# sanweiliti/RoHM

Measured on NVIDIA H100. Metric: denoised motion clips/sec (145-frame, 1000-step PoseNet p_sample_loop), higher is better.
Workload: dtype f32 (fp16 hi/lo error-compensated tensor-core GEMMs)

## Files before the change

include/rohm_b200.h:

```cpp
#ifndef ROHM_B200_H_
#define ROHM_B200_H_

#include <stdint.h>

#ifdef __cplusplus
extern "C" {
#endif

#if defined(__GNUC__)
#define ROHM_API __attribute__((visibility("default")))
#else
#define ROHM_API
#endif

typedef enum {
  ROHM_OK = 0,
  ROHM_ERR_INVALID = -1,
  ROHM_ERR_CUDA = -2,
  ROHM_ERR_NO_DEVICE = -3,
  ROHM_ERR_STATE = -4
} rohm_status;

typedef enum {
  ROHM_PRECISION_TF32X3 = 3,
  ROHM_PRECISION_F16X2 = 2,
  ROHM_PRECISION_TF32 = 1
} rohm_precision;

typedef struct rohm_ctx rohm_ctx;
typedef struct rohm_posenet rohm_posenet;
typedef struct rohm_trajnet rohm_trajnet;
typedef struct rohm_body rohm_body;

ROHM_API int rohm_version(void);
ROHM_API int rohm_ctx_create(int device, rohm_ctx** out);
ROHM_API void rohm_ctx_destroy(rohm_ctx* ctx);
ROHM_API const char* rohm_last_error(const rohm_ctx* ctx);


#define ROHM_DDPM_COEFS 8
ROHM_API int rohm_ddpm_step(rohm_ctx* ctx, const float* x0, const float* x_t, const float* noise, const float* grad0,
                            const float* grad1, int n_grads, float* out, int64_t n_clips, int64_t clip_elems,
                            const float* coef, int64_t coef_clip_stride, void* stream);

ROHM_API int rohm_ddpm_step_philox(rohm_ctx* ctx, const float* x0, const float* x_t, const float* grad0, const float* grad1,
                                   int n_grads, float* out, int64_t n_clips, int64_t clip_elems, const float* coef,
                                   int64_t coef_clip_stride, uint64_t seed, uint64_t offset, uint64_t* offset_increment,
                                   void* stream);

ROHM_API int rohm_q_sample(rohm_ctx* ctx, const float* x_start, const float* noise, float* out, int64_t n, float sqrt_ac,
                  float sqrt_one_minus_ac, void* stream);

ROHM_API int rohm_ddim_step(rohm_ctx* ctx, const float* x0, const float* x_t, const float* noise, float* out, int64_t n,
                   float sqrt_recip_ac, float sqrt_recipm1_ac, float sqrt_ac_prev, float dir_coef, float sigma,
                   void* stream);

typedef struct {
  const float* in_proj_w;
  const float* in_proj_b;
  const float* out_proj_w;
  const float* out_proj_b;
  const float* lin1_w;
  const float* lin1_b;
  const float* lin2_w;
  const float* lin2_b;
  const float* norm1_w;
  const float* norm1_b;
  const float* norm2_w;
  const float* norm2_b;
} rohm_posenet_layer;

typedef struct {
  int d_model;
  int ff_size;
  int num_layers;
  int num_heads;
  int in_feats;
  int out_feats;
  int traj_feats;
  int pe_len;
  const float* in_w;
  const float* in_b;
  const float* cond_w;
  const float* cond_b;
  const float* pe;
  const float* t0_w;
  const float* t0_b;
  const float* t2_w;
  const float* t2_b;
  const float* out_w;
  const float* out_b;
  const rohm_posenet_layer* layers;
} rohm_posenet_weights;

ROHM_API int rohm_posenet_create(rohm_ctx* ctx, const rohm_posenet_weights* w, int max_batch, int max_frames, int precision,
                        rohm_posenet** out);
ROHM_API void rohm_posenet_destroy(rohm_posenet* pn);

ROHM_API int rohm_posenet_set_cond(rohm_posenet* pn, const float* cond, int B, int T, void* stream);

ROHM_API int rohm_posenet_set_lengths(rohm_posenet* pn, const int* lengths_host, int B);

ROHM_API int rohm_posenet_forward(rohm_posenet* pn, const float* x_t, const int64_t* timesteps, float* out, int B, int T,
                         void* stream);

ROHM_API int rohm_posenet_sample_step(rohm_posenet* pn, const float* x_t, const int64_t* timesteps, float* x0_out,
                                      float* x_next, const float* coef_row, uint64_t seed, uint64_t offset,
                                      uint64_t* offset_increment, int B, int T, void* stream);

ROHM_API int rohm_posenet_profile(rohm_posenet* pn, const float* x_t, const int64_t* timesteps, float* out, int B, int T,
                         void* stream, float* ms_by_category, int* launches_by_category);

ROHM_API int rohm_posenet_set_option(rohm_posenet* pn, int option, int value);

ROHM_API int rohm_posenet_launches_per_forward(const rohm_posenet* pn);


ROHM_API int rohm_trajnet_create(rohm_ctx* ctx, int n_params, const char* const* names, const float* const* ptrs,
                                 const int64_t* numels, int time_dim, int cond_dim, int traj_feat_dim, int mid_dim,
                                 int trajcontrol, int control_cond_dim, int max_batch, int frames, int precision,
                                 rohm_trajnet** out);
ROHM_API void rohm_trajnet_destroy(rohm_trajnet* tn);

ROHM_API int rohm_trajnet_set_cond(rohm_trajnet* tn, const float* cond, const float* control_cond, int B, void* stream);

ROHM_API int rohm_trajnet_set_lengths(rohm_trajnet* tn, const int* lengths_host, int B);

ROHM_API int rohm_trajnet_forward(rohm_trajnet* tn, const float* x_t, const int64_t* time, float* out, int B,
                                  void* stream);
ROHM_API int rohm_trajnet_sample_step(rohm_trajnet* tn, const float* x_t, const int64_t* time, float* x0_out, float* x_next,
                                      const float* coef_row, uint64_t seed, uint64_t offset, uint64_t* offset_increment, int B,
                                      void* stream);
ROHM_API int rohm_trajnet_set_option(rohm_trajnet* tn, int option, int value);
ROHM_API int rohm_trajnet_launches_per_forward(const rohm_trajnet* tn);


ROHM_API int rohm_body_create(rohm_ctx* ctx, const float* v_template, const float* shapedirs, int shape_comps,
                              const float* posedirs, const float* J_regressor, const float* lbs_weights,
                              const int* parents_host, int num_verts, int64_t max_frames, int with_vertices,
                              int precision, rohm_body** out);
ROHM_API void rohm_body_destroy(rohm_body* bd);
ROHM_API int rohm_body_uses_fused_lbs(const rohm_body* bd);

ROHM_API int rohm_body_set_vertex_pitch(rohm_body* bd, int64_t pitch_floats);

ROHM_API int rohm_body_forward(rohm_body* bd, const float* global_orient, const float* body_pose, const float* betas,
                               const float* transl, int64_t N, float* joints, int num_joints, float* vertices,
                               void* stream);

ROHM_API int rohm_body_from_repr(rohm_body* bd, const float* x, const float* mean, const float* stdv, int B, int T,
                                 float* joints, int num_joints, float* vertices, void* stream);

ROHM_API int rohm_body_from_repr_layout(rohm_body* bd, const float* x, int channels_last, const float* mean,
                                        const float* stdv, int B, int T, float* joints, int num_joints, float* vertices,
                                        void* stream);


ROHM_API int rohm_body_from_repr_lengths(rohm_body* bd, const float* x, int channels_last, const float* mean,
                                         const float* stdv, int B, int T, const int* lengths, const int* clip_off,
                                         int64_t total_frames, float* joints, int num_joints, float* vertices,
                                         void* stream);

ROHM_API int rohm_skating_guidance(rohm_body* bd, const float* x0, const float* mean, const float* stdv, int B, int T,
                                   float* grad, float* loss_out, void* stream);

ROHM_API int rohm_skating_guidance_lengths(rohm_body* bd, const float* x0, const float* mean, const float* stdv,
                                           const int* lengths, int B, int T, float* grad, float* loss_out, void* stream);

ROHM_API int rohm_skating_guidance_sums(rohm_body* bd, const float* x0, const float* mean, const float* stdv, int B, int T,
                                        float* sums_out, void* stream);
ROHM_API int rohm_skating_guidance_backward(rohm_body* bd, const float* x0, const float* mean, const float* stdv, int B, int T,
                                            const float* sums, float* grad, void* stream);

ROHM_API int rohm_projection_guidance(rohm_body* bd, const float* x0, const float* mean, const float* stdv, int B, int T,
                                      const float* cam_affine, const float* focal, const float* center,
                                      const float* keypoints_2d, int kp_frames, float* grad, float* loss_out,
                                      void* stream);


ROHM_API int rohm_traj_glue(rohm_body* bd, const float* traj_out, int traj_dim, const float* repr_clean,
                            const float* traj_mean, const float* traj_std, const float* pose_mean, const float* pose_std,
                            int B, int T, float* composite_out, float* traj_full_out, void* stream);

ROHM_API int rohm_traj_glue_lengths(rohm_body* bd, const float* traj_out, int traj_dim, const float* repr_clean,
                                    const float* traj_mean, const float* traj_std, const float* pose_mean,
                                    const float* pose_std, int B, int T, const int* lengths, const int* clip_off,
                                    int64_t total_frames, float* composite_out, float* traj_full_out, void* stream);

ROHM_API int rohm_traj_repr_from_joints(rohm_ctx* ctx, const float* joints, const float* global_orient_aa,
                                        const float* transl, const float* mean, const float* stdv, int B, int T,
                                        float* traj_full_out, void* stream);

ROHM_API int rohm_traj_repr_from_joints_lengths(rohm_ctx* ctx, const float* joints, const float* global_orient_aa,
                                                const float* transl, const float* mean, const float* stdv, int B, int T,
                                                const int* lengths, const int* clip_off, float* traj_full_out,
                                                void* stream);

ROHM_API int rohm_pose_to_control_cond(rohm_ctx* ctx, const float* pose_out, int B, int Tp, int T, int traj_feats,
                                       int cond_feats, float* control_cond, void* stream);

ROHM_API int rohm_pose_to_control_cond_lengths(rohm_ctx* ctx, const float* pose_out, int B, int Tp, int T, int traj_feats,
                                               int cond_feats, const int* lengths, float* control_cond, void* stream);

ROHM_API int rohm_build_pose_cond(rohm_ctx* ctx, const float* src, int src_channel_major, int src_T, const float* traj_full,
                                  const unsigned char* chan_keep, const int* frame_lo, const int* frame_hi,
                                  int zero_contact, int B, int Tp, float* cond_out, void* stream);

ROHM_API int rohm_build_pose_cond_lengths(rohm_ctx* ctx, const float* src, int src_channel_major, int src_T,
                                          const float* traj_full, const unsigned char* chan_keep, const int* frame_lo,
                                          const int* frame_hi, int zero_contact, int B, int Tp, const int* lengths,
                                          float* cond_out, void* stream);

ROHM_API int rohm_rot6d_to_aa(rohm_ctx* ctx, const float* rot6d, int64_t n, float* aa, float* rotmat, void* stream);

ROHM_API int rohm_joints_from_traj(rohm_ctx* ctx, const float* x, int channels_last, const float* mean, const float* stdv,
                                   int B, int T, int relative, float* joints, void* stream);

ROHM_API int rohm_joints_from_traj_lengths(rohm_ctx* ctx, const float* x, int channels_last, const float* mean,
                                           const float* stdv, int B, int T, const int* lengths, const int* clip_off,
                                           int64_t total_frames, int relative, float* joints, void* stream);

#ifdef __cplusplus
}
#endif
#endif
```

rohm_b200/_lib.py:

```python
import ctypes as C
import os
import threading

_HERE = os.path.dirname(os.path.abspath(__file__))
LIB_PATH = os.path.join(_HERE, "librohm_b200.so")

ROHM_OK = 0
PRECISION_TF32X3 = 3
PRECISION_F16X2 = 2
PRECISION_TF32 = 1
DDPM_COEFS = 8


class RohmB200Error(RuntimeError):
    pass


class PoseNetLayerW(C.Structure):
    _fields_ = [(n, C.c_void_p) for n in (
        "in_proj_w", "in_proj_b", "out_proj_w", "out_proj_b", "lin1_w", "lin1_b", "lin2_w", "lin2_b",
        "norm1_w", "norm1_b", "norm2_w", "norm2_b")]


class PoseNetW(C.Structure):
    _fields_ = [("d_model", C.c_int), ("ff_size", C.c_int), ("num_layers", C.c_int), ("num_heads", C.c_int),
                ("in_feats", C.c_int), ("out_feats", C.c_int), ("traj_feats", C.c_int), ("pe_len", C.c_int)] + \
               [(n, C.c_void_p) for n in ("in_w", "in_b", "cond_w", "cond_b", "pe", "t0_w", "t0_b", "t2_w", "t2_b",
                                          "out_w", "out_b")] + [("layers", C.POINTER(PoseNetLayerW))]


_p, _i, _i64, _f = C.c_void_p, C.c_int, C.c_int64, C.c_float
SIGNATURES = {
    "rohm_version": (_i, []),
    "rohm_ctx_create": (_i, [_i, C.POINTER(_p)]),
    "rohm_ctx_destroy": (None, [_p]),
    "rohm_last_error": (C.c_char_p, [_p]),
    "rohm_ddpm_step": (_i, [_p, _p, _p, _p, _p, _p, _i, _p, _i64, _i64, _p, _i64, _p]),
    "rohm_ddpm_step_philox": (_i, [_p, _p, _p, _p, _p, _i, _p, _i64, _i64, _p, _i64, C.c_uint64, C.c_uint64,
                                    C.POINTER(C.c_uint64), _p]),
    "rohm_q_sample": (_i, [_p, _p, _p, _p, _i64, _f, _f, _p]),
    "rohm_ddim_step": (_i, [_p, _p, _p, _p, _p, _i64, _f, _f, _f, _f, _f, _p]),
    "rohm_posenet_create": (_i, [_p, C.POINTER(PoseNetW), _i, _i, _i, C.POINTER(_p)]),
    "rohm_posenet_destroy": (None, [_p]),
    "rohm_posenet_set_cond": (_i, [_p, _p, _i, _i, _p]),
    "rohm_posenet_set_lengths": (_i, [_p, C.POINTER(_i), _i]),
    "rohm_posenet_forward": (_i, [_p, _p, _p, _p, _i, _i, _p]),
    "rohm_posenet_sample_step": (_i, [_p, _p, _p, _p, _p, _p, C.c_uint64, C.c_uint64, C.POINTER(C.c_uint64), _i, _i, _p]),
    "rohm_posenet_profile": (_i, [_p, _p, _p, _p, _i, _i, _p, C.POINTER(C.c_float), C.POINTER(C.c_int)]),
    "rohm_posenet_set_option": (_i, [_p, _i, _i]),
    "rohm_posenet_launches_per_forward": (_i, [_p]),
    "rohm_trajnet_create": (_i, [_p, _i, C.POINTER(C.c_char_p), C.POINTER(_p), C.POINTER(_i64), _i, _i, _i, _i, _i, _i,
                                 _i, _i, _i, C.POINTER(_p)]),
    "rohm_trajnet_destroy": (None, [_p]),
    "rohm_trajnet_set_cond": (_i, [_p, _p, _p, _i, _p]),
    "rohm_trajnet_set_lengths": (_i, [_p, C.POINTER(_i), _i]),
    "rohm_trajnet_forward": (_i, [_p, _p, _p, _p, _i, _p]),
    "rohm_trajnet_sample_step": (_i, [_p, _p, _p, _p, _p, _p, C.c_uint64, C.c_uint64, C.POINTER(C.c_uint64), _i, _p]),
    "rohm_trajnet_set_option": (_i, [_p, _i, _i]),
    "rohm_trajnet_launches_per_forward": (_i, [_p]),
    "rohm_body_create": (_i, [_p, _p, _p, _i, _p, _p, _p, C.POINTER(C.c_int), _i, _i64, _i, _i, C.POINTER(_p)]),
    "rohm_body_destroy": (None, [_p]),
    "rohm_body_uses_fused_lbs": (_i, [_p]),
    "rohm_body_set_vertex_pitch": (_i, [_p, _i64]),
    "rohm_body_forward": (_i, [_p, _p, _p, _p, _p, _i64, _p, _i, _p, _p]),
    "rohm_body_from_repr": (_i, [_p, _p, _p, _p, _i, _i, _p, _i, _p, _p]),
    "rohm_body_from_repr_layout": (_i, [_p, _p, _i, _p, _p, _i, _i, _p, _i, _p, _p]),
    "rohm_body_from_repr_lengths": (_i, [_p, _p, _i, _p, _p, _i, _i, _p, _p, _i64, _p, _i, _p, _p]),
    "rohm_skating_guidance": (_i, [_p, _p, _p, _p, _i, _i, _p, _p, _p]),
    "rohm_skating_guidance_lengths": (_i, [_p, _p, _p, _p, _p, _i, _i, _p, _p, _p]),
    "rohm_skating_guidance_sums": (_i, [_p, _p, _p, _p, _i, _i, _p, _p]),
    "rohm_skating_guidance_backward": (_i, [_p, _p, _p, _p, _i, _i, _p, _p, _p]),
    "rohm_projection_guidance": (_i, [_p, _p, _p, _p, _i, _i, _p, _p, _p, _p, _i, _p, _p, _p]),
    "rohm_traj_glue": (_i, [_p, _p, _i, _p, _p, _p, _p, _p, _i, _i, _p, _p, _p]),
    "rohm_traj_glue_lengths": (_i, [_p, _p, _i, _p, _p, _p, _p, _p, _i, _i, _p, _p, _i64, _p, _p, _p]),
    "rohm_traj_repr_from_joints": (_i, [_p, _p, _p, _p, _p, _p, _i, _i, _p, _p]),
    "rohm_traj_repr_from_joints_lengths": (_i, [_p, _p, _p, _p, _p, _p, _i, _i, _p, _p, _p, _p]),
    "rohm_pose_to_control_cond": (_i, [_p, _p, _i, _i, _i, _i, _i, _p, _p]),
    "rohm_pose_to_control_cond_lengths": (_i, [_p, _p, _i, _i, _i, _i, _i, _p, _p, _p]),
    "rohm_build_pose_cond": (_i, [_p, _p, _i, _i, _p, _p, _p, _p, _i, _i, _i, _p, _p]),
    "rohm_build_pose_cond_lengths": (_i, [_p, _p, _i, _i, _p, _p, _p, _p, _i, _i, _i, _p, _p, _p]),
    "rohm_rot6d_to_aa": (_i, [_p, _p, _i64, _p, _p, _p]),
    "rohm_joints_from_traj": (_i, [_p, _p, _i, _p, _p, _i, _i, _i, _p, _p]),
    "rohm_joints_from_traj_lengths": (_i, [_p, _p, _i, _p, _p, _i, _i, _p, _p, _i64, _i, _p, _p]),
}

_lock = threading.Lock()
_lib = None
_ctx = {}


def load():
    global _lib
    if _lib is not None:
        return _lib
    with _lock:
        if _lib is not None:
            return _lib
        if not os.path.exists(LIB_PATH):
            raise RohmB200Error(
                f"{LIB_PATH} not found: build it with `python -c 'import __graft_entry__ as g; g.build()'` "
                "or `make -C rohm_b200/csrc`.  rohm_b200 has no CPU fallback.")
        try:
            lib = C.CDLL(LIB_PATH)
        except OSError as e:
            raise RohmB200Error(f"cannot load {LIB_PATH}: {e}") from e
        for name, (res, args) in SIGNATURES.items():
            fn = getattr(lib, name)
            fn.restype = res
            fn.argtypes = args
        _lib = lib
    return _lib


def ctx(device_index):
    lib = load()
    if device_index in _ctx:
        return _ctx[device_index]
    with _lock:
        if device_index in _ctx:
            return _ctx[device_index]
        out = C.c_void_p()
        rc = lib.rohm_ctx_create(int(device_index), C.byref(out))
        if rc != ROHM_OK:
            raise RohmB200Error(f"rohm_ctx_create(device={device_index}) failed with status {rc}: "
                                "an sm_90 (H100) device is required; there is no CPU fallback")
        _ctx[device_index] = out
    return _ctx[device_index]


def check(rc, c):
    if rc != ROHM_OK:
        msg = load().rohm_last_error(c)
        raise RohmB200Error(f"status {rc}: {msg.decode() if msg else '?'}")
```

rohm_b200/csrc/gemm.cu:

```cuda
#include "gemm.cuh"
#include "ptx.cuh"

#include <cudaTypedefs.h>
#include <cmath>
#include <cstdio>
#include <cstring>
#include <mutex>

namespace rohm {

namespace {

constexpr int kFirstMmaWarp = 4;
constexpr int kMmaWarps = 8;
constexpr int kFirstEpiWarp = kFirstMmaWarp + kMmaWarps;
__host__ __device__ constexpr bool epi_role(int epi) { return epi == 0 || epi == 1 || epi == 3; }
__host__ __device__ constexpr int kernel_threads(int epi) { return 32 * (kFirstEpiWarp + (epi_role(epi) ? 4 : 0)); }
constexpr int kProducerRegs = 40, kEpiRoleRegs = 152, kMmaRegs = 160;
static_assert(kProducerRegs + kEpiRoleRegs + 2 * kMmaRegs <= 512, "register file of one SM");
static_assert(kProducerRegs <= 128 && kEpiRoleRegs >= 128 && kMmaRegs >= 128, "setmaxnreg.dec / .inc direction");
constexpr int kSmemLimit = 227 * 1024;
constexpr int kStaticSmemReserve = 8 * 1024;
constexpr int kEpiTileFloats = 32 * 32;
constexpr int kSkinPitch = 100;
constexpr int kSkinStageBytes = kGemmBlockM * kSkinPitch * 4;

template <int BLOCK_N, int PASSES, bool EPI_ROLE>
struct TileCfg {
  static constexpr int kEpiWarps = EPI_ROLE ? 4 : 8;
  static constexpr int kABytes = kGemmBlockM * kGemmBlockK * 4;
  static constexpr int kBBytes = BLOCK_N * kGemmBlockK * 4;
  static constexpr int kSplit = (PASSES == 3) ? 2 : 1;
  static constexpr int kStageBytes = kSplit * (kABytes + kBBytes);
  static constexpr int kAccPitch = BLOCK_N + 4;
  static constexpr int kAccBytes = kGemmBlockM * kAccPitch * 4;
  static constexpr int kEpiBytes = !EPI_ROLE && BLOCK_N == 96 && kSkinStageBytes > kEpiWarps * kEpiTileFloats * 4
                                       ? kSkinStageBytes
                                       : kEpiWarps * kEpiTileFloats * 4;
  static constexpr int kStagesRaw = (kSmemLimit - kStaticSmemReserve - 1024 - kAccBytes - kEpiBytes) / kStageBytes;
  static constexpr int kStages = kStagesRaw > 10 ? 10 : kStagesRaw;
  static constexpr int kSmemBytes = kStages * kStageBytes + 1024 + kAccBytes + kEpiWarps * kEpiTileFloats * 4;
  static constexpr int kAccRegs = BLOCK_N / 2;
  static_assert(kStages >= 2, "need at least a double buffer");
  static_assert(BLOCK_N % 32 == 0 && BLOCK_N >= 32 && BLOCK_N <= 128, "wgmma N and the epilogue's 32-column chunks");
};

template <int KIND, int R>
__device__ __forceinline__ void mma_step(float (&d)[R], uint64_t a, uint64_t b) {
  if constexpr (KIND == kKindF16) ptx::wgmma_f16(d, a, b);
  else ptx::wgmma_tf32(d, a, b);
}

template <int PITCH, int N>
__device__ __forceinline__ void acc_load(const float* acc, int row, int col, float (&v)[N]) {
  const float4* src = reinterpret_cast<const float4*>(acc + row * PITCH + col);
#pragma unroll
  for (int j = 0; j < N / 4; ++j) {
    const float4 t = src[j];
    v[4 * j] = t.x, v[4 * j + 1] = t.y, v[4 * j + 2] = t.z, v[4 * j + 3] = t.w;
  }
}

__device__ __forceinline__ float apply_act(float x, int act) {
  if (act == kActGelu) {
    return 0.5f * x * (1.0f + erff(x * 0.70710678118654752440f));
  } else if (act == kActSilu) {
    return x / (1.0f + expf(-x));
  } else if (act == kActMish) {
    float sp = x > 20.0f ? x : log1pf(expf(x));
    return x * tanhf(sp);
  }
  return x;
}

__device__ __forceinline__ float gelu_erf(float x) {
  const float u = fminf(fabsf(x), 6.5f);
  float q = -1.657032612e-06f;
  q = fmaf(q, u, 2.461445729e-05f);
  q = fmaf(q, u, -1.118122309e-04f);
  q = fmaf(q, u, -3.311361652e-04f);
  q = fmaf(q, u, 7.346248254e-03f);
  q = fmaf(q, u, -5.272617936e-02f);
  q = fmaf(q, u, -4.591094553e-01f);
  q = fmaf(q, u, -1.151124716e+00f);
  q = fmaf(q, u, -9.999987483e-01f);
  float p;
  asm("ex2.approx.ftz.f32 %0, %1;" : "=f"(p) : "f"(q));
  return fmaf(-fabsf(x), p, fmaxf(x, 0.0f));
}

__device__ __forceinline__ void load_bone_transform(const float* frame_col, int64_t lda, int bone, float4& r0, float4& r1,
                                                    float4& r2) {
  const float* a = frame_col + static_cast<int64_t>(bone) * 12 * lda;
  r0 = make_float4(__ldg(a), __ldg(a + lda), __ldg(a + 2 * lda), __ldg(a + 3 * lda));
  r1 = make_float4(__ldg(a + 4 * lda), __ldg(a + 5 * lda), __ldg(a + 6 * lda), __ldg(a + 7 * lda));
  r2 = make_float4(__ldg(a + 8 * lda), __ldg(a + 9 * lda), __ldg(a + 10 * lda), __ldg(a + 11 * lda));
}

struct EpiParams {
  const float* bias;
  const float* residual;
  const float2* a_stats;
  const float* a_corr;
  const float2* res_stats;
  const float* res_gamma;
  const float* res_beta;
  float2* stats_out;
  float ln_eps;
  float* out;
  void* out_hi;
  void* out_lo;
  float acc_scale;
  int tma_store;
  int bias_per_row;
  int ldr, ldo, lds, act, M, N, out_row_mul, out_row_add, clip_rows, clip_valid;
};

__device__ __forceinline__ float2 combine_row_stats(const float2* row8, float eps) {
  const float4* q4 = reinterpret_cast<const float4*>(row8);
  float4 t[4];
#pragma unroll
  for (int i = 0; i < 4; ++i) t[i] = __ldcg(q4 + i);
  const float mean = ((t[0].x + t[0].z) + (t[1].x + t[1].z) + (t[2].x + t[2].z) + (t[3].x + t[3].z)) * 0.125f;
  float m2 = 0.0f;
#pragma unroll
  for (int i = 0; i < 4; ++i) {
    const float d0 = t[i].x - mean, d1 = t[i].z - mean;
    m2 += fmaf(64.0f * d0, d0, t[i].y) + fmaf(64.0f * d1, d1, t[i].w);
  }
  return make_float2(mean, rsqrtf(m2 * (1.0f / 512.0f) + eps));
}

__device__ __forceinline__ void stage_pair_chunk(const float (&v)[32], uint8_t* tb, int lane, const CUtensorMap* st_hi,
                                                 const CUtensorMap* st_lo, int col0, int row0) {
  if (lane == 0) ptx::bulk_wait_read_all();
  __syncwarp();
#pragma unroll
  for (int c = 0; c < 4; ++c) {
    uint2 h0, l0, h1, l1;
    ptx::split_f16x4(make_float4(v[8 * c], v[8 * c + 1], v[8 * c + 2], v[8 * c + 3]), h0, l0);
    ptx::split_f16x4(make_float4(v[8 * c + 4], v[8 * c + 5], v[8 * c + 6], v[8 * c + 7]), h1, l1);
    const int off = lane * 64 + ((c ^ ((lane >> 1) & 3)) << 4);
    *reinterpret_cast<uint4*>(tb + off) = make_uint4(h0.x, h0.y, h1.x, h1.y);
    *reinterpret_cast<uint4*>(tb + 2048 + off) = make_uint4(l0.x, l0.y, l1.x, l1.y);
  }
  ptx::fence_proxy_async();
  __syncwarp();
  if (lane == 0) {
    ptx::tma_store_2d(st_hi, tb, col0, row0);
    ptx::tma_store_2d(st_lo, tb + 2048, col0, row0);
    ptx::bulk_commit();
  }
}

template <int BLOCK_N, int PASSES, int EPI, int KIND>
__global__ void __launch_bounds__(kernel_threads(EPI), 1) gemm_tile_kernel(const __grid_constant__ GemmParams p) {
  constexpr bool LEAN = EPI != 2 && EPI != 5;
  constexpr bool EPI_ROLE = epi_role(EPI);
  constexpr int kElemK = gemm_block_k(KIND);
  using Cfg = TileCfg<BLOCK_N, PASSES, EPI_ROLE>;
  constexpr int kEpiWarps = Cfg::kEpiWarps;
  extern __shared__ uint8_t smem_raw[];
  __shared__ uint64_t full_bar[Cfg::kStages];
  __shared__ uint64_t empty_bar[Cfg::kStages];
  __shared__ EpiParams epi_s;
  __shared__ __align__(16) float bias_s[BLOCK_N];
  __shared__ __align__(16) float corr_s[BLOCK_N];
  __shared__ __align__(16) float beta_s[EPI == 3 ? BLOCK_N : 4];
  __shared__ uint64_t res_bar[EPI == 3 ? kEpiWarps : 1];
  __shared__ uint64_t acc_full, acc_empty;
  __shared__ __align__(16) float skin_w_s[EPI == 4 ? 2 : 1][EPI == 4 ? kSkinTileBones * 32 : 4];
  __shared__ int skin_bone_s[EPI == 4 ? 2 : 1][EPI == 4 ? kSkinTileBones : 1];
  __shared__ int skin_nb_s[2];

  const uint32_t raw_addr = ptx::smem_u32(smem_raw);
  uint8_t* smem = smem_raw + ((1024u - (raw_addr & 1023u)) & 1023u);
  float* const acc_s = reinterpret_cast<float*>(smem + Cfg::kStages * Cfg::kStageBytes);
  uint8_t* const epi_smem = smem + Cfg::kStages * Cfg::kStageBytes + Cfg::kAccBytes;

  const int warp_idx = threadIdx.x >> 5;
  const int lane = threadIdx.x & 31;
  const int tiles_n = (p.grid_n_cols + BLOCK_N - 1) / BLOCK_N;
  const int tiles_m = (p.grid_m_rows + kGemmBlockM - 1) / kGemmBlockM;
  const int num_tiles = tiles_m * tiles_n;

  int total_iters = 0;
  for (int s = 0; s < p.num_segs; ++s) total_iters += p.seg_kblocks[s];
  const int S = (!LEAN && p.k_splits > 1) ? p.k_splits : 1;
  const int per_split = (total_iters + S - 1) / S;
  const int num_work = num_tiles * S;

  if (warp_idx == 0 && lane == 0) {
    ptx::prefetch_tmap(&p.b_hi);
    if (PASSES == 3) ptx::prefetch_tmap(&p.b_lo);
    for (int s = 0; s < p.num_segs; ++s) {
      ptx::prefetch_tmap(&p.a_hi[s]);
      if (PASSES == 3) ptx::prefetch_tmap(&p.a_lo[s]);
    }
    for (int i = 0; i < Cfg::kStages; ++i) {
      ptx::mbar_init(&full_bar[i], 1);
      ptx::mbar_init(&empty_bar[i], 2);
    }
    if (EPI == 3)
      for (int i = 0; i < kEpiWarps; ++i) ptx::mbar_init(&res_bar[i], 1);
    if (EPI_ROLE) {
      ptx::mbar_init(&acc_full, kMmaWarps);
      ptx::mbar_init(&acc_empty, kEpiWarps);
    }
    ptx::fence_barrier_init();
  }
  int prefetched = 0;
  if (warp_idx == 0 && lane == 0 && static_cast<int>(blockIdx.x) < num_work) {
    const int tile0 = static_cast<int>(blockIdx.x) / S;
    const int it_b = (static_cast<int>(blockIdx.x) - tile0 * S) * per_split;
    const int cnt = (total_iters < it_b + per_split ? total_iters : it_b + per_split) - it_b;
    const int n0 = (tile0 % tiles_n) * BLOCK_N;
    prefetched = cnt < Cfg::kStages ? cnt : Cfg::kStages;
    for (int i = 0; i < prefetched; ++i) {
      uint8_t* st = smem + i * Cfg::kStageBytes;
      ptx::mbar_expect_tx(&full_bar[i], Cfg::kStageBytes);
      ptx::tma_load_2d(st + Cfg::kSplit * Cfg::kABytes, &p.b_hi, &full_bar[i], (it_b + i) * kElemK, n0);
      if (PASSES == 3)
        ptx::tma_load_2d(st + 2 * Cfg::kABytes + Cfg::kBBytes, &p.b_lo, &full_bar[i], (it_b + i) * kElemK, n0);
    }
  }
  if (warp_idx == kFirstMmaWarp && lane == 0) {
    epi_s.bias = p.bias, epi_s.residual = p.residual, epi_s.ldr = p.ldr, epi_s.out = p.out, epi_s.ldo = p.ldo;
    epi_s.out_hi = p.out_hi, epi_s.out_lo = p.out_lo, epi_s.lds = p.lds, epi_s.act = p.act, epi_s.M = p.M, epi_s.N = p.N;
    epi_s.out_row_mul = p.out_row_mul, epi_s.out_row_add = p.out_row_add, epi_s.clip_rows = p.clip_rows;
    epi_s.clip_valid = p.clip_valid;
    epi_s.acc_scale = p.acc_scale == 0.0f ? 1.0f : p.acc_scale;
    epi_s.tma_store = p.tma_store;
    epi_s.bias_per_row = p.bias_per_row;
    epi_s.a_stats = p.a_stats, epi_s.a_corr = p.a_corr, epi_s.res_stats = p.res_stats, epi_s.res_gamma = p.res_gamma;
    epi_s.res_beta = p.res_beta, epi_s.stats_out = p.stats_out, epi_s.ln_eps = p.ln_eps;
    if (p.tma_store) {
      ptx::prefetch_tmap(&p.st_out);
      ptx::prefetch_tmap(&p.st_hi);
      ptx::prefetch_tmap(&p.st_lo);
    }
  }
  __syncthreads();

  ptx::pdl_launch_dependents();
  ptx::pdl_wait_prior_grid();

  if (warp_idx < kFirstMmaWarp) {
    ptx::setmaxnreg_dec<kProducerRegs>();
    if (warp_idx == 0 && lane == 0) {
      int it = 0, stage = 0;
      uint32_t phase = 0;
      for (int w = blockIdx.x; w < num_work; w += gridDim.x) {
        const int tile = w / S;
        const int m0 = (tile / tiles_n) * kGemmBlockM;
        const int n0 = (tile % tiles_n) * BLOCK_N;
        const int it_b = (w - tile * S) * per_split;
        const int it_e = total_iters < it_b + per_split ? total_iters : it_b + per_split;
        int s = 0, kb = it_b;
        while (s + 1 < p.num_segs && kb >= p.seg_kblocks[s]) kb -= p.seg_kblocks[s], ++s;
        int kcol = it_b * kElemK;
        for (int i = it_b; i < it_e; ++i, ++it, kcol += kElemK) {
          {
            const int row = m0 * p.seg_row_mul[s] + p.seg_row_shift[s];
            uint8_t* st = smem + stage * Cfg::kStageBytes;
            if (it < prefetched) {
              ptx::tma_load_2d(st, &p.a_hi[s], &full_bar[stage], kb * kElemK, row);
              if (PASSES == 3) ptx::tma_load_2d(st + Cfg::kABytes, &p.a_lo[s], &full_bar[stage], kb * kElemK, row);
              if (++stage == Cfg::kStages) stage = 0, phase ^= 1;
              if (++kb == p.seg_kblocks[s]) kb = 0, ++s;
              continue;
            }
            ptx::mbar_wait(&empty_bar[stage], phase ^ 1);
            ptx::mbar_expect_tx(&full_bar[stage], Cfg::kStageBytes);
            ptx::tma_load_2d(st, &p.a_hi[s], &full_bar[stage], kb * kElemK, row);
            ptx::tma_load_2d(st + Cfg::kSplit * Cfg::kABytes, &p.b_hi, &full_bar[stage], kcol, n0);
            if (PASSES == 3) {
              ptx::tma_load_2d(st + Cfg::kABytes, &p.a_lo[s], &full_bar[stage], kb * kElemK, row);
              ptx::tma_load_2d(st + 2 * Cfg::kABytes + Cfg::kBBytes, &p.b_lo, &full_bar[stage], kcol, n0);
            }
            if (++stage == Cfg::kStages) stage = 0, phase ^= 1;
            if (++kb == p.seg_kblocks[s]) kb = 0, ++s;
          }
        }
      }
    }
  } else {
    const bool mma_warp = warp_idx < kFirstEpiWarp;
    if constexpr (!EPI_ROLE) ptx::setmaxnreg_inc<232>();
    const int mq = (warp_idx - kFirstMmaWarp) & 3;
    const int mhalf = (warp_idx - kFirstMmaWarp) >> 2;
    const int ew = warp_idx - (EPI_ROLE ? kFirstEpiWarp : kFirstMmaWarp);
    const int q = ew & 3;
    const int half = EPI_ROLE ? 0 : ew >> 2;
    constexpr int kChunkStep = EPI_ROLE ? 32 : 64;
    int mma_stage = 0;
    uint32_t mma_phase = 0;
    auto mma_tile = [&](int w, int tc) {
      float dm[Cfg::kAccRegs];
      float dc[PASSES == 3 ? Cfg::kAccRegs : 1];
#pragma unroll
      for (int i = 0; i < Cfg::kAccRegs; ++i) dm[i] = 0.0f;
#pragma unroll
      for (int i = 0; i < (PASSES == 3 ? Cfg::kAccRegs : 1); ++i) dc[i] = 0.0f;
      const int it_b = (w % S) * per_split;
      const int n_it = (total_iters < it_b + per_split ? total_iters : it_b + per_split) - it_b;
      const bool signaller = (threadIdx.x & 127) == 0;
      auto release = [&](int stg) {
        if (signaller) ptx::mbar_arrive(&empty_bar[stg]);
      };
      int prev = -1;
      for (int ki = 0; ki < n_it; ++ki) {
        ptx::mbar_wait(&full_bar[mma_stage], mma_phase);
        const uint32_t st = ptx::smem_u32(smem + mma_stage * Cfg::kStageBytes);
        const uint32_t a_off = static_cast<uint32_t>(mhalf * (Cfg::kABytes / 2));
        const uint64_t a_hi = ptx::make_desc_kmajor<kGemmBlockK * 4>(st + a_off);
        const uint64_t b_hi = ptx::make_desc_kmajor<kGemmBlockK * 4>(st + Cfg::kSplit * Cfg::kABytes);
        const uint64_t a_lo = ptx::make_desc_kmajor<kGemmBlockK * 4>(st + Cfg::kABytes + a_off);
        const uint64_t b_lo = ptx::make_desc_kmajor<kGemmBlockK * 4>(st + 2 * Cfg::kABytes + Cfg::kBBytes);
        ptx::wgmma_fence_regs(dm);
        if (PASSES == 3) ptx::wgmma_fence_regs(dc);
        ptx::wgmma_fence();
#pragma unroll
        for (int k = 0; k < kGemmBlockK / 8; ++k) {
          const uint64_t koff = static_cast<uint64_t>(k * 2);
          mma_step<KIND>(dm, a_hi + koff, b_hi + koff);
          if constexpr (PASSES == 3) {
            mma_step<KIND>(dc, a_lo + koff, b_hi + koff);
            mma_step<KIND>(dc, a_hi + koff, b_lo + koff);
          }
        }
        ptx::wgmma_commit();
        ptx::wgmma_fence_regs(dm);
        if (PASSES == 3) ptx::wgmma_fence_regs(dc);
        ptx::wgmma_wait<1>();
        if (prev >= 0) release(prev);
        prev = mma_stage;
        if (++mma_stage == Cfg::kStages) mma_stage = 0, mma_phase ^= 1;
      }
      ptx::wgmma_wait<0>();
      ptx::wgmma_fence_regs(dm);
      if (PASSES == 3) ptx::wgmma_fence_regs(dc);
      if (prev >= 0) release(prev);
      if constexpr (EPI_ROLE) ptx::mbar_wait(&acc_empty, static_cast<uint32_t>((tc & 1) ^ 1));
      const int r0 = mhalf * 64 + mq * 16 + (lane >> 2);
      const int cc = 2 * (lane & 3);
#pragma unroll
      for (int j = 0; j < BLOCK_N / 8; ++j) {
        float v0 = dm[4 * j], v1 = dm[4 * j + 1], v2 = dm[4 * j + 2], v3 = dm[4 * j + 3];
        if (PASSES == 3) v0 += dc[4 * j], v1 += dc[4 * j + 1], v2 += dc[4 * j + 2], v3 += dc[4 * j + 3];
        *reinterpret_cast<float2*>(acc_s + r0 * Cfg::kAccPitch + 8 * j + cc) = make_float2(v0, v1);
        *reinterpret_cast<float2*>(acc_s + (r0 + 8) * Cfg::kAccPitch + 8 * j + cc) = make_float2(v2, v3);
      }
      if constexpr (EPI_ROLE) {
        __syncwarp();
        if (lane == 0) ptx::mbar_arrive(&acc_full);
      } else {
        asm volatile("bar.sync 3, %0;" ::"n"(kMmaWarps * 32));
      }
    };
    const bool epi_warp = !EPI_ROLE || !mma_warp;
    if (!epi_warp) {
      ptx::setmaxnreg_inc<kMmaRegs>();
      int tc = 0;
      for (int wi = blockIdx.x; wi < num_work; wi += gridDim.x, ++tc) mma_tile(wi, tc);
    } else if constexpr (EPI_ROLE) {
      ptx::setmaxnreg_inc<kEpiRoleRegs>();
    }
    EpiParams e_regs;
    if constexpr (!EPI_ROLE) e_regs = epi_s;
    const EpiParams& e = EPI_ROLE ? epi_s : e_regs;
    const bool vec_ok = ((e.N & 3) == 0);
    float* tile = reinterpret_cast<float*>(epi_smem) + ew * kEpiTileFloats;
    const int tr = lane >> 3, tc = (lane & 7) * 4;
    int tcount = 0;
    uint32_t res_phase = 0;
    if constexpr (EPI == 4) {
      static_assert(BLOCK_N == 96 && PASSES == 3 && KIND == kKindF16, "skinning epilogue: 32 vertices x 3 per tile, fp16 pairs");
      constexpr int kSkinRegBones = 4;
      const int i = ew * 32 + lane;
      float4 sk[kSkinRegBones][3];
      float* const stg = reinterpret_cast<float*>(epi_smem);
      auto fetch_tables = [&](int tile_n, float& w0, float& w1, int& bone, int& nbv) {
        const float* wsrc = p.skin_w + static_cast<int64_t>(tile_n) * (kSkinTileBones * 32);
        w0 = __ldg(wsrc + i), w1 = __ldg(wsrc + i + 256);
        bone = i < kSkinTileBones ? __ldg(p.skin_bone + tile_n * kSkinTileBones + i) : 0;
        nbv = i == 0 ? __ldg(p.skin_nb + tile_n) : 0;
      };
      auto publish_tables = [&](int buf, float w0, float w1, int bone, int nbv) {
        skin_w_s[buf][i] = w0, skin_w_s[buf][i + 256] = w1;
        if (i < kSkinTileBones) skin_bone_s[buf][i] = bone;
        if (i == 0) skin_nb_s[buf] = nbv;
      };
      auto request_transforms = [&](int buf, int m_first) {
        const int mm = m_first + q * 32 + lane;
        const float* col = p.skin_A + (mm < e.M ? mm : 0);
        const int nbv = skin_nb_s[buf];
#pragma unroll
        for (int b = 0; b < kSkinRegBones; ++b)
          if (b < nbv) load_bone_transform(col, p.skin_lda, skin_bone_s[buf][b], sk[b][0], sk[b][1], sk[b][2]);
      };
      int buf = 0;
      if (static_cast<int>(blockIdx.x) < num_tiles) {
        float w0, w1;
        int bone, nbv;
        fetch_tables(static_cast<int>(blockIdx.x) % tiles_n, w0, w1, bone, nbv);
        publish_tables(0, w0, w1, bone, nbv);
        asm volatile("bar.sync 1, %0;" ::"n"(kEpiWarps * 32));
        request_transforms(0, (static_cast<int>(blockIdx.x) / tiles_n) * kGemmBlockM);
      }
      for (int tile_idx = blockIdx.x; tile_idx < num_tiles; tile_idx += gridDim.x, ++tcount, buf ^= 1) {
        const int m0 = (tile_idx / tiles_n) * kGemmBlockM;
        const int n0 = (tile_idx % tiles_n) * BLOCK_N;
        const int m = m0 + q * 32 + lane;
        const int next = tile_idx + static_cast<int>(gridDim.x);
        const bool has_next = next < num_tiles;
        float nw0 = 0.f, nw1 = 0.f;
        int nbone = 0, nnb = 0;
        if (has_next) fetch_tables(next % tiles_n, nw0, nw1, nbone, nnb);

        mma_tile(tile_idx, tcount);
        float o[48];
#pragma unroll
        for (int j = 0; j < 48; ++j) o[j] = 0.0f;
        const int nb = skin_nb_s[buf];
        const float* col = p.skin_A + (m < e.M ? m : 0);
#pragma unroll
        for (int h2 = 0; h2 < 2; ++h2) {
          float vp[24];
          {
            acc_load<Cfg::kAccPitch>(acc_s, q * 32 + lane, 48 * half + 24 * h2, vp);
#pragma unroll
            for (int j = 0; j < 24; ++j) vp[j] *= e.acc_scale;
          }
          auto apply_bone = [&](const float4& r0, const float4& r1, const float4& r2, const float* wrow) {
#pragma unroll
            for (int g = 0; g < 2; ++g) {
              const float4 w4 = *reinterpret_cast<const float4*>(wrow + 8 * h2 + 4 * g);
              const float wv[4] = {w4.x, w4.y, w4.z, w4.w};
#pragma unroll
              for (int u = 0; u < 4; ++u) {
                const int j = 4 * g + u;
                const float x = vp[3 * j], y = vp[3 * j + 1], z = vp[3 * j + 2];
                float& ox = o[24 * h2 + 3 * j];
                float& oy = o[24 * h2 + 3 * j + 1];
                float& oz = o[24 * h2 + 3 * j + 2];
                ox = fmaf(wv[u], fmaf(r0.x, x, fmaf(r0.y, y, fmaf(r0.z, z, r0.w))), ox);
                oy = fmaf(wv[u], fmaf(r1.x, x, fmaf(r1.y, y, fmaf(r1.z, z, r1.w))), oy);
                oz = fmaf(wv[u], fmaf(r2.x, x, fmaf(r2.y, y, fmaf(r2.z, z, r2.w))), oz);
              }
            }
          };
#pragma unroll
          for (int b = 0; b < kSkinRegBones; ++b)
            if (b < nb) apply_bone(sk[b][0], sk[b][1], sk[b][2], &skin_w_s[buf][b * 32 + 16 * half]);
          if (nb > kSkinRegBones) {
            float4 c0, c1, c2;
            load_bone_transform(col, p.skin_lda, skin_bone_s[buf][kSkinRegBones], c0, c1, c2);
            for (int b = kSkinRegBones; b < nb; ++b) {
              const float4 r0 = c0, r1 = c1, r2 = c2;
              if (b + 1 < nb) load_bone_transform(col, p.skin_lda, skin_bone_s[buf][b + 1], c0, c1, c2);
              apply_bone(r0, r1, r2, &skin_w_s[buf][b * 32 + 16 * half]);
            }
          }
        }
        if (has_next) publish_tables(buf ^ 1, nw0, nw1, nbone, nnb);
        if (e.tma_store && ew == 0 && lane == 0) ptx::bulk_wait_read_all();
        asm volatile("bar.sync 1, %0;" ::"n"(kEpiWarps * 32));
        if (has_next) request_transforms(buf ^ 1, (next / tiles_n) * kGemmBlockM);
        if (e.tma_store) {
          uint8_t* const sb = reinterpret_cast<uint8_t*>(stg);
          const int r = q * 32 + lane;
#pragma unroll
          for (int j = 0; j < 12; ++j) {
            const int cc = 12 * half + j;
            *reinterpret_cast<float4*>(sb + (cc >> 3) * (kGemmBlockM * 128) + r * 128 + (((cc & 7) ^ (r & 7)) << 4)) =
                make_float4(o[4 * j], o[4 * j + 1], o[4 * j + 2], o[4 * j + 3]);
          }
          ptx::fence_proxy_async();
          asm volatile("bar.sync 2, %0;" ::"n"(kEpiWarps * 32));
          if (ew == 0 && lane == 0) {
#pragma unroll
            for (int j = 0; j < 3; ++j)
              if (n0 + 32 * j < e.N) ptx::tma_store_2d(&p.st_out, sb + j * (kGemmBlockM * 128), n0 + 32 * j, m0);
            ptx::bulk_commit();
          }
          continue;
        }
        {
          float4* srow = reinterpret_cast<float4*>(stg + (q * 32 + lane) * kSkinPitch + 48 * half);
#pragma unroll
          for (int j = 0; j < 12; ++j) srow[j] = make_float4(o[4 * j], o[4 * j + 1], o[4 * j + 2], o[4 * j + 3]);
        }
        asm volatile("bar.sync 2, %0;" ::"n"(kEpiWarps * 32));
        {
          const int w8 = ew;
#pragma unroll 4
          for (int rr = 0; rr < kGemmBlockM / kEpiWarps; ++rr) {
            const int r = w8 * (kGemmBlockM / kEpiWarps) + rr;
            const int mr = m0 + r;
            if (mr >= e.M) break;
            float* dst = e.out + static_cast<int64_t>(mr) * e.ldo + n0;
            const float* src = stg + r * kSkinPitch;
#pragma unroll
            for (int c = 0; c < 3; ++c) {
              const int col = lane + 32 * c;
              if (n0 + col < e.N) __stcs(dst + col, src[col]);
            }
          }
        }
      }
    }
    for (int wi = blockIdx.x; EPI != 4 && epi_warp && wi < num_work; wi += gridDim.x, ++tcount) {
      const int tile_idx = wi / S;
      const int split_rows = (wi - tile_idx * S) * (!LEAN ? p.split_row_stride : 0);
      const int m0 = (tile_idx / tiles_n) * kGemmBlockM;
      const int n0 = (tile_idx % tiles_n) * BLOCK_N;
      const int m = m0 + q * 32 + lane;
      const bool row_ok = m < e.M;
      bool row_real = true;
      if constexpr (EPI == 5) row_real = row_ok && __ldg(p.row_mask + m) != 0;
      else if (!LEAN && e.clip_rows > 0) row_real = (m % e.clip_rows) < e.clip_valid;
      const int64_t orow = static_cast<int64_t>(m) * e.out_row_mul + e.out_row_add + split_rows;
      const float bias_row = (e.bias != nullptr && e.bias_per_row && row_ok) ? __ldg(e.bias + m) : 0.0f;

      {
        const int i = ew * 32 + lane;
        asm volatile("bar.sync 1, %0;" ::"n"(kEpiWarps * 32));
        if (i < BLOCK_N) {
          const bool col_ok = n0 + i < e.N;
          bias_s[i] = (e.bias != nullptr && !e.bias_per_row && col_ok) ? __ldg(e.bias + n0 + i) : 0.0f;
          if (EPI == 3) {
            corr_s[i] = e.res_stats != nullptr ? __ldg(e.res_gamma + n0 + i) : 1.0f;
            beta_s[i] = e.res_stats != nullptr ? __ldg(e.res_beta + n0 + i) : 0.0f;
          } else {
            corr_s[i] = (e.a_stats != nullptr && col_ok) ? __ldg(e.a_corr + n0 + i) : 0.0f;
          }
        }
        if (e.residual != nullptr && row_ok) {
          const float* r = e.residual + orow * e.ldr + n0 + half * 32;
#pragma unroll
          for (int c = 0; c < (EPI_ROLE ? BLOCK_N : (BLOCK_N > 64 ? 128 : 64)); c += kChunkStep)
            asm volatile("prefetch.global.L2 [%0];" ::"l"(r + c));
        }
        asm volatile("bar.sync 1, %0;" ::"n"(kEpiWarps * 32));
      }
      float a_mean = 0.0f, a_rstd = 1.0f;
      if (EPI != 3 && LEAN && e.a_stats != nullptr && row_ok) {
        const float2 mr = combine_row_stats(e.a_stats + static_cast<int64_t>(m) * 8, e.ln_eps);
        a_mean = mr.x, a_rstd = mr.y;
      }
      float lnv[EPI == 3 ? 2 : 1][EPI == 3 ? 32 : 1];
      float r_mean = 0.0f, r_rstd = 1.0f;
      auto load_residual = [&](int g) {
        uint8_t* tb = reinterpret_cast<uint8_t*>(tile);
        uint64_t* rb = &res_bar[ew];
#pragma unroll
        for (int h2 = 0; h2 < 2; ++h2) {
          const int c0 = g * 32 + 64 * h2;
          if (lane == 0) {
            ptx::bulk_wait_read_all();
            ptx::mbar_expect_tx(rb, 4096);
            ptx::tma_load_2d(tb, &p.st_hi, rb, n0 + c0, m0 + q * 32);
            ptx::tma_load_2d(tb + 2048, &p.st_lo, rb, n0 + c0, m0 + q * 32);
          }
          ptx::mbar_wait(rb, res_phase);
          res_phase ^= 1;
#pragma unroll
          for (int c = 0; c < 4; ++c) {
            const int off = lane * 64 + ((c ^ ((lane >> 1) & 3)) << 4);
            const uint4 hq = *reinterpret_cast<const uint4*>(tb + off);
            const uint4 lq = *reinterpret_cast<const uint4*>(tb + 2048 + off);
            const uint32_t hw[4] = {hq.x, hq.y, hq.z, hq.w};
            const uint32_t lw[4] = {lq.x, lq.y, lq.z, lq.w};
#pragma unroll
            for (int k = 0; k < 4; ++k) {
              const float2 fh = __half22float2(*reinterpret_cast<const __half2*>(&hw[k]));
              const float2 fl = __half22float2(*reinterpret_cast<const __half2*>(&lw[k]));
              const int j = 8 * c + 2 * k;
              lnv[h2][j] = fmaf(((fh.x + fl.x) - r_mean) * r_rstd, corr_s[c0 + j], beta_s[c0 + j]);
              lnv[h2][j + 1] = fmaf(((fh.y + fl.y) - r_mean) * r_rstd, corr_s[c0 + j + 1], beta_s[c0 + j + 1]);
            }
          }
          ptx::fence_proxy_async();
          __syncwarp();
        }
      };
      if constexpr (EPI == 3) {
        if (e.res_stats != nullptr && row_ok) {
          const float2 mr = combine_row_stats(e.res_stats + static_cast<int64_t>(m) * 8, e.ln_eps);
          r_mean = mr.x, r_rstd = mr.y;
        }
        load_residual(0);
      }
      if constexpr (EPI_ROLE) {
        ptx::mbar_wait(&acc_full, static_cast<uint32_t>(tcount & 1));
      } else {
        mma_tile(wi, tcount);
      }

      if constexpr (EPI == 3) {
        static_assert(BLOCK_N == 128 && PASSES == 3 && KIND == kKindF16, "LayerNorm-folding producer: fp16 pairs, 128-wide tiles");
        static_assert(EPI_ROLE, "one thread per row: both 64-column statistics groups");
        const int tile_n = tile_idx % tiles_n;
        float (&v)[2][32] = lnv;
        uint8_t* tb = reinterpret_cast<uint8_t*>(tile);
        const bool group_full = (m0 + q * 32 + 32 <= e.M);
#pragma unroll 1
        for (int g = 0; g < 2; ++g) {
          if (g == 1) load_residual(1);
#pragma unroll
          for (int h2 = 0; h2 < 2; ++h2) {
            const int c0 = g * 32 + 64 * h2;
            float raw[32];
            acc_load<Cfg::kAccPitch>(acc_s, q * 32 + lane, c0, raw);
#pragma unroll
            for (int j = 0; j < 32; j += 4) {
              const float4 b4 = *reinterpret_cast<const float4*>(&bias_s[c0 + j]);
              v[h2][j] += fmaf(raw[j], e.acc_scale, b4.x);
              v[h2][j + 1] += fmaf(raw[j + 1], e.acc_scale, b4.y);
              v[h2][j + 2] += fmaf(raw[j + 2], e.acc_scale, b4.z);
              v[h2][j + 3] += fmaf(raw[j + 3], e.acc_scale, b4.w);
            }
          }
          if (g == 1) {
            __syncwarp();
            if (lane == 0) ptx::mbar_arrive(&acc_empty);
          }
          auto store_chunk = [&](int h2) {
            const int nb = n0 + g * 32 + 64 * h2;
            if (group_full) {
              stage_pair_chunk(v[h2], tb, lane, &p.st_hi, &p.st_lo, nb, m0 + q * 32);
            } else if (row_ok) {
              __half* oh = static_cast<__half*>(e.out_hi) + static_cast<int64_t>(m) * e.lds + nb;
              __half* ol = static_cast<__half*>(e.out_lo) + static_cast<int64_t>(m) * e.lds + nb;
#pragma unroll
              for (int j = 0; j < 32; ++j) ptx::split_f16(v[h2][j], oh[j], ol[j]);
            }
          };
          store_chunk(0);
          float s1 = 0.0f;
#pragma unroll
          for (int j = 0; j < 32; ++j) s1 += v[0][j] + v[1][j];
          const float mean_i = s1 * (1.0f / 64.0f);
          float m2_i = 0.0f;
#pragma unroll
          for (int j = 0; j < 32; ++j) {
            const float d0 = v[0][j] - mean_i, d1 = v[1][j] - mean_i;
            m2_i = fmaf(d0, d0, fmaf(d1, d1, m2_i));
          }
          if (row_ok) e.stats_out[static_cast<int64_t>(m) * 8 + tile_n * 2 + g] = make_float2(mean_i, m2_i);
          store_chunk(1);
        }
        continue;
      }

#pragma unroll 1
      for (int c0 = half * 32; c0 < BLOCK_N; c0 += kChunkStep) {
        const int nb = n0 + c0;
        const bool full = vec_ok && (nb + 32 <= e.N);
        if (e.tma_store && full && (m0 + q * 32 + 32 <= e.M)) {
          float v[32];
          acc_load<Cfg::kAccPitch>(acc_s, q * 32 + lane, c0, v);
          if (KIND == kKindF16) {
#pragma unroll
            for (int j = 0; j < 32; ++j) v[j] *= e.acc_scale;
          }
          if (LEAN && e.a_stats != nullptr) {
#pragma unroll
            for (int j = 0; j < 32; j += 4) {
              const float4 c4 = *reinterpret_cast<const float4*>(&corr_s[c0 + j]);
              v[j] = a_rstd * fmaf(-a_mean, c4.x, v[j]), v[j + 1] = a_rstd * fmaf(-a_mean, c4.y, v[j + 1]);
              v[j + 2] = a_rstd * fmaf(-a_mean, c4.z, v[j + 2]), v[j + 3] = a_rstd * fmaf(-a_mean, c4.w, v[j + 3]);
            }
          }
          if (e.bias != nullptr) {
#pragma unroll
            for (int j = 0; j < 32; j += 4) {
              const float4 b4 = *reinterpret_cast<const float4*>(&bias_s[c0 + j]);
              v[j] += b4.x, v[j + 1] += b4.y, v[j + 2] += b4.z, v[j + 3] += b4.w;
            }
            if (e.bias_per_row) {
#pragma unroll
              for (int j = 0; j < 32; ++j) v[j] += bias_row;
            }
          }
          if (EPI == 1) {
#pragma unroll
            for (int j = 0; j < 32; ++j) v[j] = gelu_erf(v[j]);
          }
          if (!LEAN) {
            if (e.act == kActGelu) {
#pragma unroll
              for (int j = 0; j < 32; ++j) v[j] = gelu_erf(v[j]);
            } else if (e.act == kActSilu) {
#pragma unroll
              for (int j = 0; j < 32; ++j) v[j] = v[j] / (1.0f + expf(-v[j]));
            } else if (e.act == kActMish) {
#pragma unroll
              for (int j = 0; j < 32; ++j) v[j] = apply_act(v[j], kActMish);
            }
            if (!row_real) {
#pragma unroll
              for (int j = 0; j < 32; ++j) v[j] = 0.0f;
            }
          }
          if (lane == 0) ptx::bulk_wait_read_all();
          __syncwarp();
          uint8_t* tb = reinterpret_cast<uint8_t*>(tile);
          if (e.out != nullptr) {
#pragma unroll
            for (int c = 0; c < 8; ++c)
              *reinterpret_cast<float4*>(tb + lane * 128 + ((c ^ (lane & 7)) << 4)) =
                  make_float4(v[4 * c], v[4 * c + 1], v[4 * c + 2], v[4 * c + 3]);
          } else {
#pragma unroll
            for (int c = 0; c < 4; ++c) {
              uint2 h0, l0, h1, l1;
              ptx::split_f16x4(make_float4(v[8 * c], v[8 * c + 1], v[8 * c + 2], v[8 * c + 3]), h0, l0);
              ptx::split_f16x4(make_float4(v[8 * c + 4], v[8 * c + 5], v[8 * c + 6], v[8 * c + 7]), h1, l1);
              const int off = lane * 64 + ((c ^ ((lane >> 1) & 3)) << 4);
              *reinterpret_cast<uint4*>(tb + off) = make_uint4(h0.x, h0.y, h1.x, h1.y);
              *reinterpret_cast<uint4*>(tb + 2048 + off) = make_uint4(l0.x, l0.y, l1.x, l1.y);
            }
          }
          ptx::fence_proxy_async();
          __syncwarp();
          if (lane == 0) {
            if (e.out != nullptr) {
              ptx::tma_store_2d(&p.st_out, tb, nb, m0 + q * 32 + split_rows);
            } else {
              ptx::tma_store_2d(&p.st_hi, tb, nb, m0 + q * 32 + split_rows);
              ptx::tma_store_2d(&p.st_lo, tb + 2048, nb, m0 + q * 32 + split_rows);
            }
            ptx::bulk_commit();
          }
          continue;
        }
        float4 res[8];
        const bool use_res = e.residual != nullptr && full;
        if (use_res) {
#pragma unroll
          for (int rr = 0; rr < 8; ++rr) {
            const int mr = m0 + q * 32 + rr * 4 + tr;
            res[rr] = make_float4(0.f, 0.f, 0.f, 0.f);
            if (mr < e.M)
              res[rr] = *reinterpret_cast<const float4*>(
                  e.residual + (static_cast<int64_t>(mr) * e.out_row_mul + e.out_row_add) * e.ldr + nb + tc);
          }
        }
        float v[32];
        acc_load<Cfg::kAccPitch>(acc_s, q * 32 + lane, c0, v);
        if (KIND == kKindF16) {
#pragma unroll
          for (int j = 0; j < 32; ++j) v[j] *= e.acc_scale;
        }
        if (nb >= e.N) continue;

        if (row_ok) {
          if (LEAN && e.a_stats != nullptr) {
#pragma unroll
            for (int j = 0; j < 32; ++j) v[j] = a_rstd * fmaf(-a_mean, corr_s[c0 + j], v[j]);
          }
          if (e.bias != nullptr) {
#pragma unroll
            for (int j = 0; j < 32; ++j) v[j] += bias_s[c0 + j];
            if (e.bias_per_row) {
#pragma unroll
              for (int j = 0; j < 32; ++j) v[j] += bias_row;
            }
          }
          if (EPI == 0) {
          } else if (EPI == 1 || e.act == kActGelu) {
#pragma unroll
            for (int j = 0; j < 32; ++j) v[j] = gelu_erf(v[j]);
          } else if (e.act == kActSilu) {
#pragma unroll
            for (int j = 0; j < 32; ++j) v[j] = v[j] / (1.0f + expf(-v[j]));
          } else if (e.act == kActMish) {
#pragma unroll
            for (int j = 0; j < 32; ++j) v[j] = apply_act(v[j], kActMish);
          }
          if (e.residual != nullptr && !full) {
            const float* r = e.residual + orow * e.ldr + nb;
#pragma unroll
            for (int j = 0; j < 32; ++j)
              if (nb + j < e.N) v[j] += r[j];
          }
          if (!LEAN && !row_real) {
#pragma unroll
            for (int j = 0; j < 32; ++j) v[j] = 0.0f;
          }
        }

        if (full) {
          if (e.tma_store) {
            if (lane == 0) ptx::bulk_wait_read_all();
            __syncwarp();
          }
#pragma unroll
          for (int j = 0; j < 32; ++j) tile[lane * 32 + (j ^ lane)] = v[j];
          __syncwarp();
#pragma unroll
          for (int rr = 0; rr < 8; ++rr) {
            const int r = rr * 4 + tr;
            const int mr = m0 + q * 32 + r;
            float4 w;
            w.x = tile[r * 32 + (tc ^ r)], w.y = tile[r * 32 + ((tc + 1) ^ r)];
            w.z = tile[r * 32 + ((tc + 2) ^ r)], w.w = tile[r * 32 + ((tc + 3) ^ r)];
            if (mr < e.M) {
              if (use_res) {
                bool real = true;
                if constexpr (EPI == 5) real = __ldg(p.row_mask + mr) != 0;
                else if (!LEAN && e.clip_rows > 0) real = (mr % e.clip_rows) < e.clip_valid;
                if (real) w.x += res[rr].x, w.y += res[rr].y, w.z += res[rr].z, w.w += res[rr].w;
              }
              const int64_t orr = static_cast<int64_t>(mr) * e.out_row_mul + e.out_row_add + split_rows;
              if (e.out != nullptr) *reinterpret_cast<float4*>(e.out + orr * e.ldo + nb + tc) = w;
              if (e.out_hi != nullptr) {
                if (KIND == kKindF16) {
                  uint2 h, l;
                  ptx::split_f16x4(w, h, l);
                  *reinterpret_cast<uint2*>(static_cast<__half*>(e.out_hi) + orr * e.lds + nb + tc) = h;
                  *reinterpret_cast<uint2*>(static_cast<__half*>(e.out_lo) + orr * e.lds + nb + tc) = l;
                } else {
                  float4 h, l;
                  h.x = ptx::to_tf32(w.x), h.y = ptx::to_tf32(w.y), h.z = ptx::to_tf32(w.z), h.w = ptx::to_tf32(w.w);
                  l.x = w.x - h.x, l.y = w.y - h.y, l.z = w.z - h.z, l.w = w.w - h.w;
                  *reinterpret_cast<float4*>(static_cast<float*>(e.out_hi) + orr * e.lds + nb + tc) = h;
                  *reinterpret_cast<float4*>(static_cast<float*>(e.out_lo) + orr * e.lds + nb + tc) = l;
                }
              }
            }
          }
          __syncwarp();
        } else if (row_ok) {
          if (e.out != nullptr) {
            float* o = e.out + orow * e.ldo + nb;
#pragma unroll
            for (int j = 0; j < 32; ++j)
              if (nb + j < e.N) o[j] = v[j];
          }
          if (e.out_hi != nullptr && KIND == kKindF16) {
            __half* oh = static_cast<__half*>(e.out_hi) + orow * e.lds + nb;
            __half* ol = static_cast<__half*>(e.out_lo) + orow * e.lds + nb;
#pragma unroll
            for (int j = 0; j < 32; ++j)
              if (nb + j < e.N) ptx::split_f16(v[j], oh[j], ol[j]);
          } else if (e.out_hi != nullptr) {
            float* oh = static_cast<float*>(e.out_hi) + orow * e.lds + nb;
            float* ol = static_cast<float*>(e.out_lo) + orow * e.lds + nb;
#pragma unroll
            for (int j = 0; j < 32; ++j)
              if (nb + j < e.N) {
                const float h = ptx::to_tf32(v[j]);
                oh[j] = h;
                ol[j] = v[j] - h;
              }
          }
        }
      }
      if constexpr (EPI_ROLE) {
        __syncwarp();
        if (lane == 0) ptx::mbar_arrive(&acc_empty);
      }
    }
    if (lane == 0) ptx::bulk_wait_read_all();
  }

  __syncthreads();
}

__global__ void split_tf32_kernel(const float* __restrict__ x, float* __restrict__ hi, float* __restrict__ lo,
                                  int64_t n) {
  int64_t i = static_cast<int64_t>(blockIdx.x) * blockDim.x + threadIdx.x;
  const int64_t stride = static_cast<int64_t>(gridDim.x) * blockDim.x;
  for (; i < n; i += stride) {
    const float v = x[i];
    const float h = ptx::to_tf32(v);
    hi[i] = h;
    lo[i] = v - h;
  }
}

__global__ void split_f16_kernel(const float* __restrict__ x, __half* __restrict__ hi, __half* __restrict__ lo, int64_t n,
                                 float scale) {
  int64_t i = static_cast<int64_t>(blockIdx.x) * blockDim.x + threadIdx.x;
  const int64_t stride = static_cast<int64_t>(gridDim.x) * blockDim.x;
  for (; i < n; i += stride) ptx::split_f16(x[i] * scale, hi[i], lo[i]);
}

__global__ void absmax_kernel(const float* __restrict__ w, int64_t n, unsigned int* __restrict__ out) {
  float m = 0.0f;
  for (int64_t i = static_cast<int64_t>(blockIdx.x) * blockDim.x + threadIdx.x; i < n;
       i += static_cast<int64_t>(gridDim.x) * blockDim.x) {
    const float a = fabsf(w[i]);
    m = (a <= 3.0e38f && a > m) ? a : m;
  }
#pragma unroll
  for (int off = 16; off > 0; off >>= 1) m = fmaxf(m, __shfl_xor_sync(0xffffffffu, m, off));
  if ((threadIdx.x & 31) == 0) atomicMax(out, __float_as_uint(m));
}

PFN_cuTensorMapEncodeTiled_v12000 get_encode_fn() {
  static PFN_cuTensorMapEncodeTiled_v12000 fn = nullptr;
  static std::once_flag once;
  std::call_once(once, [] {
    void* ptr = nullptr;
    cudaDriverEntryPointQueryResult qres;
    cudaError_t e = cudaGetDriverEntryPoint("cuTensorMapEncodeTiled", &ptr, cudaEnableDefault, &qres);
    if (e == cudaSuccess && qres == cudaDriverEntryPointSuccess) fn = reinterpret_cast<PFN_cuTensorMapEncodeTiled_v12000>(ptr);
  });
  return fn;
}

template <int BLOCK_N, int PASSES, int KIND>
static cudaError_t set_attr() {
  constexpr int kRoleSmem = TileCfg<BLOCK_N, PASSES, true>::kSmemBytes;
  cudaError_t e = cudaFuncSetAttribute(gemm_tile_kernel<BLOCK_N, PASSES, 0, KIND>,
                                       cudaFuncAttributeMaxDynamicSharedMemorySize, kRoleSmem);
  if (e != cudaSuccess) return e;
  e = cudaFuncSetAttribute(gemm_tile_kernel<BLOCK_N, PASSES, 1, KIND>, cudaFuncAttributeMaxDynamicSharedMemorySize, kRoleSmem);
  if (e != cudaSuccess) return e;
  e = cudaFuncSetAttribute(gemm_tile_kernel<BLOCK_N, PASSES, 2, KIND>, cudaFuncAttributeMaxDynamicSharedMemorySize,
                           TileCfg<BLOCK_N, PASSES, false>::kSmemBytes);
  if (e != cudaSuccess) return e;
  e = cudaFuncSetAttribute(gemm_tile_kernel<BLOCK_N, PASSES, 5, KIND>, cudaFuncAttributeMaxDynamicSharedMemorySize,
                           TileCfg<BLOCK_N, PASSES, false>::kSmemBytes);
  if (e != cudaSuccess) return e;
  if constexpr (BLOCK_N == 128 && PASSES == 3 && KIND == kKindF16)
    e = cudaFuncSetAttribute(gemm_tile_kernel<BLOCK_N, PASSES, 3, KIND>, cudaFuncAttributeMaxDynamicSharedMemorySize, kRoleSmem);
  return e;
}

template <int BLOCK_N, int PASSES, int KIND>
cudaError_t launch_cfg(const GemmParams& p, int m_rows, int n_cols, cudaStream_t stream, bool pdl) {
  using Cfg = TileCfg<BLOCK_N, PASSES, false>;
  const bool plain = p.clip_rows == 0;
  const int epi = (plain && p.act == kActNone) ? 0 : (plain && p.act == kActGelu) ? 1 : p.row_mask != nullptr ? 5 : 2;
  auto kern = epi == 0   ? gemm_tile_kernel<BLOCK_N, PASSES, 0, KIND>
              : epi == 1 ? gemm_tile_kernel<BLOCK_N, PASSES, 1, KIND>
              : epi == 2 ? gemm_tile_kernel<BLOCK_N, PASSES, 2, KIND>
                         : gemm_tile_kernel<BLOCK_N, PASSES, 5, KIND>;
  int threads = kernel_threads(epi);
  int smem_bytes = epi_role(epi) ? TileCfg<BLOCK_N, PASSES, true>::kSmemBytes : Cfg::kSmemBytes;
  if (p.a_stats != nullptr && (!plain || p.a_corr == nullptr)) return cudaErrorInvalidValue;
  if (p.row_mask != nullptr && plain) return cudaErrorInvalidValue;
  if (p.stats_out != nullptr) {
    if constexpr (BLOCK_N == 128 && PASSES == 3 && KIND == kKindF16) {
      if (!plain || p.act != kActNone || n_cols != 4 * BLOCK_N || p.N != n_cols || !p.tma_store || p.out != nullptr ||
          p.out_hi == nullptr || p.a_stats != nullptr || (p.res_stats != nullptr && (p.res_gamma == nullptr || p.res_beta == nullptr)))
        return cudaErrorInvalidValue;
      kern = gemm_tile_kernel<BLOCK_N, PASSES, 3, KIND>;
      threads = kernel_threads(3);
      smem_bytes = TileCfg<BLOCK_N, PASSES, true>::kSmemBytes;
    } else {
      return cudaErrorInvalidValue;
    }
  }
  if (p.skin_A != nullptr) {
    if constexpr (BLOCK_N == 96 && PASSES == 3 && KIND == kKindF16) {
      if (!plain || p.act != kActNone || p.out == nullptr || p.skin_nb == nullptr || p.skin_bone == nullptr || p.skin_w == nullptr ||
          p.bias != nullptr || p.residual != nullptr || p.a_stats != nullptr || p.stats_out != nullptr)
        return cudaErrorInvalidValue;
      kern = gemm_tile_kernel<BLOCK_N, PASSES, 4, KIND>;
      threads = kernel_threads(4);
      smem_bytes = Cfg::kStages * Cfg::kStageBytes + 1024 + Cfg::kAccBytes + kSkinStageBytes;
      static bool skin_attr_set = false;
      if (!skin_attr_set) {
        cudaError_t e = cudaFuncSetAttribute(kern, cudaFuncAttributeMaxDynamicSharedMemorySize, smem_bytes);
        if (e != cudaSuccess) return e;
        skin_attr_set = true;
      }
    } else {
      return cudaErrorInvalidValue;
    }
  }
  static bool attr_set = false;
  if (!attr_set) {
    cudaError_t e = set_attr<BLOCK_N, PASSES, KIND>();
    if (e != cudaSuccess) return e;
    attr_set = true;
  }
  static int num_sms = 0;
  if (num_sms == 0) {
    int dev = 0;
    cudaGetDevice(&dev);
    if (cudaDeviceGetAttribute(&num_sms, cudaDevAttrMultiProcessorCount, dev) != cudaSuccess || num_sms <= 0) num_sms = 132;
  }
  GemmParams q = p;
  q.grid_m_rows = m_rows;
  q.grid_n_cols = n_cols;
  int tiles = ((n_cols + BLOCK_N - 1) / BLOCK_N) * ((m_rows + kGemmBlockM - 1) / kGemmBlockM);
  if (q.k_splits > 1) {
    int iters = 0;
    for (int s = 0; s < q.num_segs; ++s) iters += q.seg_kblocks[s];
    const int per = (iters + q.k_splits - 1) / q.k_splits;
    if (plain || q.out == nullptr || q.out_hi != nullptr || q.bias != nullptr || q.residual != nullptr ||
        q.act != kActNone || q.out_row_mul != 1 || q.out_row_add != 0 || (q.k_splits - 1) * per >= iters ||
        q.split_row_stride < m_rows)
      return cudaErrorInvalidValue;
    tiles *= q.k_splits;
  }
  cudaLaunchConfig_t cfg{};
  int grid = tiles < num_sms ? tiles : num_sms;
  if (p.stats_out != nullptr) grid -= grid % 4;
  cfg.gridDim = dim3(grid, 1, 1);
  cfg.blockDim = dim3(threads, 1, 1);
  cfg.dynamicSmemBytes = smem_bytes;
  cfg.stream = stream;
  cudaLaunchAttribute attr[1];
  int na = 0;
  if (pdl) {
    attr[na].id = cudaLaunchAttributeProgrammaticStreamSerialization;
    attr[na].val.programmaticStreamSerializationAllowed = 1;
    ++na;
  }
  cfg.attrs = attr;
  cfg.numAttrs = na;
  return cudaLaunchKernelEx(&cfg, kern, q);
}

}

int make_tmap_2d(CUtensorMap* map, const void* base, int64_t rows, int64_t cols, int64_t ld, int box_rows,
                 int row_elem_stride, int kind) {
  auto fn = get_encode_fn();
  if (fn == nullptr) return -1;
  cuuint64_t gdim[2] = {static_cast<cuuint64_t>(cols), static_cast<cuuint64_t>(rows)};
  cuuint64_t gstride[1] = {static_cast<cuuint64_t>(ld) * gemm_elem_bytes(kind)};
  cuuint32_t box[2] = {static_cast<cuuint32_t>(gemm_block_k(kind)), static_cast<cuuint32_t>(box_rows * row_elem_stride)};
  cuuint32_t estride[2] = {1u, static_cast<cuuint32_t>(row_elem_stride)};
  CUresult r = fn(map, kind == kKindF16 ? CU_TENSOR_MAP_DATA_TYPE_FLOAT16 : CU_TENSOR_MAP_DATA_TYPE_FLOAT32, 2,
                  const_cast<void*>(base), gdim, gstride, box, estride,
                  CU_TENSOR_MAP_INTERLEAVE_NONE, CU_TENSOR_MAP_SWIZZLE_64B, CU_TENSOR_MAP_L2_PROMOTION_L2_256B,
                  CU_TENSOR_MAP_FLOAT_OOB_FILL_NONE);
  return static_cast<int>(r);
}

static int encode_store_map(CUtensorMap* map, const void* base, int64_t rows, int64_t cols, int64_t ld, bool half,
                            int box_rows = 32) {
  auto fn = get_encode_fn();
  if (fn == nullptr) return -1;
  const int eb = half ? 2 : 4;
  cuuint64_t gdim[2] = {static_cast<cuuint64_t>(cols), static_cast<cuuint64_t>(rows)};
  cuuint64_t gstride[1] = {static_cast<cuuint64_t>(ld) * eb};
  cuuint32_t box[2] = {32u, static_cast<cuuint32_t>(box_rows)};
  cuuint32_t estride[2] = {1u, 1u};
  return static_cast<int>(fn(map, half ? CU_TENSOR_MAP_DATA_TYPE_FLOAT16 : CU_TENSOR_MAP_DATA_TYPE_FLOAT32, 2,
                             const_cast<void*>(base), gdim, gstride, box, estride, CU_TENSOR_MAP_INTERLEAVE_NONE,
                             half ? CU_TENSOR_MAP_SWIZZLE_64B : CU_TENSOR_MAP_SWIZZLE_128B, CU_TENSOR_MAP_L2_PROMOTION_NONE,
                             CU_TENSOR_MAP_FLOAT_OOB_FILL_NONE));
}

int make_store_tmap(CUtensorMap* map, const void* base, int64_t rows, int64_t cols, int64_t ld, bool half, int box_rows) {
  return encode_store_map(map, base, rows, cols, ld, half, box_rows);
}

int make_tile_tmap_f16_sw128(CUtensorMap* map, const void* base, int64_t rows, int64_t cols, int64_t ld, int box_rows) {
  auto fn = get_encode_fn();
  if (fn == nullptr) return -1;
  cuuint64_t gdim[2] = {static_cast<cuuint64_t>(cols), static_cast<cuuint64_t>(rows)};
  cuuint64_t gstride[1] = {static_cast<cuuint64_t>(ld) * 2};
  cuuint32_t box[2] = {64u, static_cast<cuuint32_t>(box_rows)};
  cuuint32_t estride[2] = {1u, 1u};
  return static_cast<int>(fn(map, CU_TENSOR_MAP_DATA_TYPE_FLOAT16, 2, const_cast<void*>(base), gdim, gstride, box, estride,
                             CU_TENSOR_MAP_INTERLEAVE_NONE, CU_TENSOR_MAP_SWIZZLE_128B, CU_TENSOR_MAP_L2_PROMOTION_L2_256B,
                             CU_TENSOR_MAP_FLOAT_OOB_FILL_NONE));
}

int gemm_enable_tma_store(GemmParams* p, int64_t rows_total, int kind) {
  p->tma_store = 0;
  const bool plain = p->residual == nullptr && p->out_row_mul == 1 && p->out_row_add == 0;
  const bool only_out = p->out != nullptr && p->out_hi == nullptr;
  const bool only_pair = p->out == nullptr && p->out_hi != nullptr && kind == kKindF16;
  if (!plain || !(only_out || only_pair)) return 0;
  int rc = 0;
  if (only_out) {
    if ((p->ldo * 4) % 16 != 0 || (reinterpret_cast<uintptr_t>(p->out) & 15) != 0) return 0;
    rc = encode_store_map(&p->st_out, p->out, rows_total, p->N, p->ldo, false);
    p->st_hi = p->st_out, p->st_lo = p->st_out;
  } else {
    if ((p->lds * 2) % 16 != 0 || (reinterpret_cast<uintptr_t>(p->out_hi) & 15) != 0 ||
        (reinterpret_cast<uintptr_t>(p->out_lo) & 15) != 0)
      return 0;
    rc = encode_store_map(&p->st_hi, p->out_hi, rows_total, p->N, p->lds, true);
    if (rc == 0) rc = encode_store_map(&p->st_lo, p->out_lo, rows_total, p->N, p->lds, true);
    p->st_out = p->st_hi;
  }
  if (rc != 0) return rc;
  p->tma_store = 1;
  return 0;
}

cudaError_t launch_gemm(const GemmParams& p, int m_rows, int n_cols, int block_n, int passes, cudaStream_t stream,
                        bool pdl, int kind) {
  if (kind == kKindF16 && passes != 3) return cudaErrorInvalidValue;
#define ROHM_GEMM_CASE(BN)                                                                       \
  case BN:                                                                                       \
    if (kind == kKindF16) return launch_cfg<BN, 3, kKindF16>(p, m_rows, n_cols, stream, pdl);    \
    return passes == 3 ? launch_cfg<BN, 3, kKindTf32>(p, m_rows, n_cols, stream, pdl)            \
                       : launch_cfg<BN, 1, kKindTf32>(p, m_rows, n_cols, stream, pdl);
  switch (block_n) {
    ROHM_GEMM_CASE(32)
    ROHM_GEMM_CASE(64)
    ROHM_GEMM_CASE(96)
    ROHM_GEMM_CASE(128)
    default:
      return cudaErrorInvalidValue;
  }
#undef ROHM_GEMM_CASE
}

cudaError_t gemm_init_attributes() {
  cudaError_t e;
  if ((e = set_attr<32, 1, kKindTf32>()) != cudaSuccess) return e;
  if ((e = set_attr<32, 3, kKindTf32>()) != cudaSuccess) return e;
  if ((e = set_attr<64, 1, kKindTf32>()) != cudaSuccess) return e;
  if ((e = set_attr<64, 3, kKindTf32>()) != cudaSuccess) return e;
  if ((e = set_attr<96, 1, kKindTf32>()) != cudaSuccess) return e;
  if ((e = set_attr<96, 3, kKindTf32>()) != cudaSuccess) return e;
  if ((e = set_attr<128, 1, kKindTf32>()) != cudaSuccess) return e;
  if ((e = set_attr<128, 3, kKindTf32>()) != cudaSuccess) return e;
  if ((e = set_attr<32, 3, kKindF16>()) != cudaSuccess) return e;
  if ((e = set_attr<64, 3, kKindF16>()) != cudaSuccess) return e;
  if ((e = set_attr<96, 3, kKindF16>()) != cudaSuccess) return e;
  if ((e = set_attr<128, 3, kKindF16>()) != cudaSuccess) return e;
  return cudaSuccess;
}

cudaError_t f16_weight_scale(const float* w_dev, int64_t n, float* scale_out) {
  *scale_out = 1.0f;
  if (n <= 0) return cudaSuccess;
  unsigned int* d_max = nullptr;
  cudaError_t e = cudaMalloc(&d_max, sizeof(unsigned int));
  if (e != cudaSuccess) return e;
  unsigned int bits = 0;
  e = cudaMemset(d_max, 0, sizeof(unsigned int));
  if (e == cudaSuccess) {
    absmax_kernel<<<132, 256>>>(w_dev, n, d_max);
    e = cudaGetLastError();
  }
  if (e == cudaSuccess) e = cudaMemcpy(&bits, d_max, sizeof bits, cudaMemcpyDeviceToHost);
  cudaFree(d_max);
  if (e != cudaSuccess) return e;
  float wmax;
  memcpy(&wmax, &bits, sizeof wmax);
  if (wmax > 0.0f) {
    int e2 = 0;
    frexpf(wmax, &e2);
    int sh = 14 - e2;
    sh = sh > 100 ? 100 : (sh < -100 ? -100 : sh);
    *scale_out = ldexpf(1.0f, sh);
  }
  return cudaSuccess;
}

cudaError_t launch_split_f16(const float* x, void* hi, void* lo, int64_t n, float scale, cudaStream_t stream) {
  if (n <= 0) return cudaSuccess;
  const int threads = 256;
  int64_t blocks = (n + threads - 1) / threads;
  if (blocks > 132 * 16) blocks = 132 * 16;
  split_f16_kernel<<<static_cast<unsigned>(blocks), threads, 0, stream>>>(x, static_cast<__half*>(hi), static_cast<__half*>(lo),
                                                                          n, scale);
  return cudaGetLastError();
}

cudaError_t launch_split_tf32(const float* x, float* hi, float* lo, int64_t n, cudaStream_t stream) {
  if (n <= 0) return cudaSuccess;
  const int threads = 256;
  int64_t blocks = (n + threads - 1) / threads;
  if (blocks > 132 * 16) blocks = 132 * 16;
  split_tf32_kernel<<<static_cast<unsigned>(blocks), threads, 0, stream>>>(x, hi, lo, n);
  return cudaGetLastError();
}

}
```

rohm_b200/csrc/gemm.cuh:

```cuda
#pragma once
#include <cstdint>
#include <cuda.h>
#include <cuda_runtime.h>

namespace rohm {

constexpr int kSkinTileBones = 16;
constexpr int kGemmBlockM = 128;
constexpr int kGemmBlockK = 16;
constexpr int kMaxSegs = 10;

enum GemmKind : int { kKindTf32 = 0, kKindF16 = 1 };
__host__ __device__ constexpr int gemm_block_k(int kind) { return kind == kKindF16 ? 2 * kGemmBlockK : kGemmBlockK; }
__host__ __device__ constexpr int gemm_elem_bytes(int kind) { return kind == kKindF16 ? 2 : 4; }

enum GemmAct : int { kActNone = 0, kActGelu = 1, kActSilu = 2, kActMish = 3 };

struct alignas(64) GemmParams {
  CUtensorMap a_hi[kMaxSegs];
  CUtensorMap a_lo[kMaxSegs];
  CUtensorMap b_hi;
  CUtensorMap b_lo;
  int seg_kblocks[kMaxSegs];
  int seg_row_shift[kMaxSegs];
  int seg_row_mul[kMaxSegs];
  int num_segs;
  const float* bias;
  int bias_per_row;
  const float* residual;
  int ldr;
  float* out;
  int ldo;
  void* out_hi;
  void* out_lo;
  int lds;
  float acc_scale;
  int act;
  int M;
  int N;
  int out_row_mul;
  int out_row_add;
  int clip_rows;
  int clip_valid;
  const unsigned char* row_mask;
  CUtensorMap st_out;
  CUtensorMap st_hi;
  CUtensorMap st_lo;
  int tma_store;
  const float2* a_stats;
  const float* a_corr;
  const float2* res_stats;
  const float* res_gamma;
  const float* res_beta;
  float2* stats_out;
  float ln_eps;
  const float* skin_A;
  int64_t skin_lda;
  const int* skin_nb;
  const int* skin_bone;
  const float* skin_w;
  int k_splits;
  int split_row_stride;
  int grid_m_rows;
  int grid_n_cols;
};

int make_tmap_2d(CUtensorMap* map, const void* base, int64_t rows, int64_t cols, int64_t ld, int box_rows,
                 int row_elem_stride = 1, int kind = kKindTf32);

int gemm_enable_tma_store(GemmParams* p, int64_t rows_total, int kind);

int make_store_tmap(CUtensorMap* map, const void* base, int64_t rows, int64_t cols, int64_t ld, bool half, int box_rows = 32);

int make_tile_tmap_f16_sw128(CUtensorMap* map, const void* base, int64_t rows, int64_t cols, int64_t ld, int box_rows);

cudaError_t launch_gemm(const GemmParams& p, int m_rows, int n_cols, int block_n, int passes, cudaStream_t stream,
                        bool pdl = false, int kind = kKindTf32);

cudaError_t gemm_init_attributes();

cudaError_t launch_split_tf32(const float* x, float* hi, float* lo, int64_t n, cudaStream_t stream);
cudaError_t f16_weight_scale(const float* w_dev, int64_t n, float* scale_out);

cudaError_t launch_split_f16(const float* x, void* hi, void* lo, int64_t n, float scale, cudaStream_t stream);

}
```

rohm_b200/csrc/posenet.cu:

```cuda
#include <cmath>
#include <cstdlib>
#include <cstring>
#include <new>

#include "attention.cuh"
#include "common.h"
#include "gemm.cuh"
#include "graph.cuh"
#include "ptx.cuh"

namespace rohm {
namespace {


__device__ __forceinline__ void clip_rows(const int* clip_off, int b, int S, int T, int64_t& row0, int& frames) {
  if (clip_off != nullptr) {
    row0 = clip_off[b];
    frames = clip_off[b + 1] - clip_off[b] - 1;
  } else {
    row0 = static_cast<int64_t>(b) * S;
    frames = T;
  }
}

__global__ void pack_tokens_kernel(const float* __restrict__ x, float* __restrict__ hi, float* __restrict__ lo, int C,
                                   int T, int S, int ld, int f16, const int* __restrict__ clip_off) {
  __shared__ float tile[32][33];
  ptx::pdl_launch_dependents();
  ptx::pdl_wait_prior_grid();
  const int b = blockIdx.z;
  const int t0 = blockIdx.x * 32, c0 = blockIdx.y * 32;
  const int tx = threadIdx.x, ty = threadIdx.y;
  int64_t row0;
  int len;
  clip_rows(clip_off, b, S, T, row0, len);
  for (int j = ty; j < 32; j += 8) {
    const int c = c0 + j, t = t0 + tx;
    tile[j][tx] = (c < C && t < len) ? x[(static_cast<int64_t>(b) * C + c) * T + t] : 0.0f;
  }
  __syncthreads();
  for (int j = ty; j < 32; j += 8) {
    const int t = t0 + j, c = c0 + tx;
    if (t < len && c < C) {
      const float v = tile[tx][j];
      const int64_t o = (row0 + 1 + t) * ld + c;
      if (f16) {
        ptx::split_f16(v, reinterpret_cast<__half*>(hi)[o], reinterpret_cast<__half*>(lo)[o]);
      } else {
        const float h = ptx::to_tf32(v);
        hi[o] = h;
        lo[o] = v - h;
      }
    }
  }
}
constexpr size_t kPackTokensX = 0;

__global__ void unpack_tokens_kernel(const float* __restrict__ tok, const float* __restrict__ cond_traj,
                                     float* __restrict__ out, int C, int Cout, int traj, int T, int S, int ldt,
                                     const int* __restrict__ clip_off) {
  __shared__ float tile[32][33];
  ptx::pdl_launch_dependents();
  ptx::pdl_wait_prior_grid();
  const int b = blockIdx.z;
  const int t0 = blockIdx.x * 32, c0 = blockIdx.y * 32;
  const int tx = threadIdx.x, ty = threadIdx.y;
  int64_t row0;
  int len;
  clip_rows(clip_off, b, S, T, row0, len);
  for (int j = ty; j < 32; j += 8) {
    const int t = t0 + j, c = c0 + tx;
    tile[j][tx] = (t < len && c < Cout) ? tok[(row0 + 1 + t) * ldt + c] : 0.0f;
  }
  __syncthreads();
  for (int j = ty; j < 32; j += 8) {
    const int c = c0 + j, t = t0 + tx;
    if (c < Cout && t < T) out[(static_cast<int64_t>(b) * C + traj + c) * T + t] = tile[tx][j];
  }
  if (blockIdx.y == 0) {
    for (int c = ty; c < traj; c += 8) {
      const int t = t0 + tx;
      if (t < T) out[(static_cast<int64_t>(b) * C + c) * T + t] = t < len ? cond_traj[(static_cast<int64_t>(b) * traj + c) * T + t] : 0.0f;
    }
  }
}
constexpr size_t kUnpackTokensOut = 2;

__global__ void pe_rows_kernel(const float* __restrict__ pe, float* __restrict__ rows, int T, int S, int D,
                               const int* __restrict__ clip_off) {
  int64_t row0;
  int len;
  clip_rows(clip_off, blockIdx.y, S, T, row0, len);
  const int d4 = D / 4;
  const int64_t i = static_cast<int64_t>(blockIdx.x) * blockDim.x + threadIdx.x;
  if (i >= static_cast<int64_t>(len + 1) * d4) return;
  const int s = static_cast<int>(i / d4);
  const int c = static_cast<int>(i - static_cast<int64_t>(s) * d4);
  reinterpret_cast<float4*>(rows)[row0 * d4 + i] = reinterpret_cast<const float4*>(pe)[static_cast<int64_t>(s) * d4 + c];
}

__global__ void time_token_gather_kernel(const int64_t* __restrict__ timesteps, const float* __restrict__ table,
                                         int table_rows, float* __restrict__ X, float* __restrict__ Xh,
                                         float* __restrict__ Xl, int S, int D, int f16, const int* __restrict__ clip_off) {
  ptx::pdl_launch_dependents();
  ptx::pdl_wait_prior_grid();
  const int b = blockIdx.x;
  int64_t t = timesteps[b];
  const bool bad = t < 0 || t >= table_rows;
  t = bad ? 0 : t;
  const float4* src = reinterpret_cast<const float4*>(table + t * D);
  const int64_t o = (clip_off != nullptr ? static_cast<int64_t>(clip_off[b]) : static_cast<int64_t>(b) * S) * D;
  const float nan = __int_as_float(0x7fc00000);
  for (int i = threadIdx.x; i < D / 4; i += blockDim.x) {
    const float4 v = bad ? make_float4(nan, nan, nan, nan) : src[i];
    reinterpret_cast<float4*>(X + o)[i] = v;
    if (f16) {
      uint2 h, l;
      ptx::split_f16x4(v, h, l);
      reinterpret_cast<uint2*>(reinterpret_cast<__half*>(Xh) + o)[i] = h;
      reinterpret_cast<uint2*>(reinterpret_cast<__half*>(Xl) + o)[i] = l;
    } else {
      float4 h, l;
      h.x = ptx::to_tf32(v.x), h.y = ptx::to_tf32(v.y), h.z = ptx::to_tf32(v.z), h.w = ptx::to_tf32(v.w);
      l.x = v.x - h.x, l.y = v.y - h.y, l.z = v.z - h.z, l.w = v.w - h.w;
      reinterpret_cast<float4*>(Xh + o)[i] = h;
      reinterpret_cast<float4*>(Xl + o)[i] = l;
    }
  }
}
constexpr size_t kTimeTokenTimesteps = 0;

__global__ void add_vec_kernel(const float* __restrict__ a, const float* __restrict__ b, float* __restrict__ out, int n) {
  const int i = blockIdx.x * blockDim.x + threadIdx.x;
  if (i < n) out[i] = a[i] + b[i];
}

template <int D>
__global__ void __launch_bounds__(256) layernorm_kernel(const float* __restrict__ in, const float* res,
                                                        const float* __restrict__ gamma,
                                                        const float* __restrict__ beta, float* out,
                                                        float* __restrict__ out_hi, float* __restrict__ out_lo,
                                                        int rows, int f16) {
  static_assert(D % 128 == 0, "row must be a multiple of 32 lanes x float4");
  ptx::pdl_launch_dependents();
  ptx::pdl_wait_prior_grid();
  constexpr int V = D / 128;
  const int row = blockIdx.x * (blockDim.x >> 5) + (threadIdx.x >> 5);
  const int lane = threadIdx.x & 31;
  if (row >= rows) return;
  const float4* src = reinterpret_cast<const float4*>(in + static_cast<int64_t>(row) * D);
  float4 x[V];
#pragma unroll
  for (int i = 0; i < V; ++i) x[i] = src[lane + 32 * i];
  if (res != nullptr) {
    const float4* rs = reinterpret_cast<const float4*>(res + static_cast<int64_t>(row) * D);
#pragma unroll
    for (int i = 0; i < V; ++i) {
      const float4 r = rs[lane + 32 * i];
      x[i].x += r.x, x[i].y += r.y, x[i].z += r.z, x[i].w += r.w;
    }
  }
  float sum = 0.0f;
#pragma unroll
  for (int i = 0; i < V; ++i) sum += (x[i].x + x[i].y) + (x[i].z + x[i].w);
#pragma unroll
  for (int off = 16; off > 0; off >>= 1) sum += __shfl_xor_sync(0xffffffffu, sum, off);
  const float mean = sum * (1.0f / D);
  float sq = 0.0f;
#pragma unroll
  for (int i = 0; i < V; ++i) {
    const float a = x[i].x - mean, b = x[i].y - mean, c = x[i].z - mean, d = x[i].w - mean;
    sq += (a * a + b * b) + (c * c + d * d);
  }
#pragma unroll
  for (int off = 16; off > 0; off >>= 1) sq += __shfl_xor_sync(0xffffffffu, sq, off);
  const float rstd = rsqrtf(sq * (1.0f / D) + 1e-5f);
  const float4* g4 = reinterpret_cast<const float4*>(gamma);
  const float4* b4 = reinterpret_cast<const float4*>(beta);
  float4* o = reinterpret_cast<float4*>(out + static_cast<int64_t>(row) * D);
  float4* oh = reinterpret_cast<float4*>(out_hi + static_cast<int64_t>(row) * D);
  float4* ol = reinterpret_cast<float4*>(out_lo + static_cast<int64_t>(row) * D);
  uint2* oh16 = reinterpret_cast<uint2*>(reinterpret_cast<__half*>(out_hi) + static_cast<int64_t>(row) * D);
  uint2* ol16 = reinterpret_cast<uint2*>(reinterpret_cast<__half*>(out_lo) + static_cast<int64_t>(row) * D);
#pragma unroll
  for (int i = 0; i < V; ++i) {
    const float4 g = g4[lane + 32 * i], bb = b4[lane + 32 * i];
    float4 y;
    y.x = (x[i].x - mean) * rstd * g.x + bb.x;
    y.y = (x[i].y - mean) * rstd * g.y + bb.y;
    y.z = (x[i].z - mean) * rstd * g.z + bb.z;
    y.w = (x[i].w - mean) * rstd * g.w + bb.w;
    o[lane + 32 * i] = y;
    if (f16) {
      uint2 h, l;
      ptx::split_f16x4(y, h, l);
      oh16[lane + 32 * i] = h;
      ol16[lane + 32 * i] = l;
    } else {
      float4 h, l;
      h.x = ptx::to_tf32(y.x), h.y = ptx::to_tf32(y.y), h.z = ptx::to_tf32(y.z), h.w = ptx::to_tf32(y.w);
      l.x = y.x - h.x, l.y = y.y - h.y, l.z = y.z - h.z, l.w = y.w - h.w;
      oh[lane + 32 * i] = h;
      ol[lane + 32 * i] = l;
    }
  }
}

}

struct PoseNetLayerDev {
  PackedWeight qkv, proj, ff1, ff2;
  float *qkv_b, *proj_b, *ff1_b, *ff2_b, *n1_w, *n1_b, *n2_w, *n2_b;
  float *qkv_c = nullptr, *qkv_d = nullptr, *ff1_c = nullptr, *ff1_d = nullptr;
};

}

using namespace rohm;

struct rohm_posenet {
  rohm_ctx* ctx = nullptr;
  DevicePool pool;
  int D = 0, F = 0, L = 0, H = 0, C = 0, Cout = 0, traj = 0, pe_len = 0, passes = 3;
  int kind = kKindTf32;
  int max_batch = 0, max_frames = 0;
  int64_t max_rows = 0;
  int Kin_p = 0;
  PackedWeight w_in, w_cond, w_out;
  float *in_b = nullptr, *cond_b = nullptr, *out_b = nullptr, *pe = nullptr;
  float* time_table = nullptr;
  std::vector<PoseNetLayerDev> layers;
  float *Ain_h = nullptr, *Ain_l = nullptr;
  float *X = nullptr, *Xh = nullptr, *Xl = nullptr, *Y = nullptr, *QKV = nullptr, *CTXh = nullptr, *CTXl = nullptr;
  float *Hh = nullptr, *Hl = nullptr, *condpe = nullptr, *OUT = nullptr;
  float* cond_traj = nullptr;
  int cond_B = -1, cond_T = -1;
  std::vector<int> lengths;
  std::vector<int> cond_lengths;
  int* clip_off = nullptr;
  int* clip_ids = nullptr;
  int packed_rows = 0, n_short = 0, short_tokens = 0, long_tokens = 0;
  int launches = 0;
  ForwardGraphs graphs;
  bool use_pdl = true;
  bool tc_attention = false;
  bool attn_maps = false;
  AttnWgmmaMaps attn_wg{};
  AttnArgs attn{};
  bool fused_ln = false;
  float2* stats1 = nullptr;
  float2* stats2 = nullptr;
  float *out_c = nullptr, *out_d = nullptr;
  bool profiling = false;
  std::vector<cudaEvent_t> prof_events;
  std::vector<int> prof_cat;
  GemmParams g_in{}, g_cond{}, g_out{};
  std::vector<GemmParams> g_qkv, g_proj, g_ff1, g_ff2;
};

enum ProfCat { kCatGemm = 0, kCatAttention = 1, kCatLayerNorm = 2, kCatOther = 3, kNumCats = 4 };

static void prof_begin(rohm_posenet* pn, int cat, cudaStream_t st) {
  if (!pn->profiling) return;
  cudaEvent_t a, b;
  cudaEventCreate(&a);
  cudaEventCreate(&b);
  pn->prof_events.push_back(a);
  pn->prof_events.push_back(b);
  pn->prof_cat.push_back(cat);
  cudaEventRecord(a, st);
}
static void prof_end(rohm_posenet* pn, cudaStream_t st) {
  if (!pn->profiling) return;
  cudaEventRecord(pn->prof_events.back(), st);
}

static int pick_block_n(int N) {
  if (N % 128 == 0) return 128;
  if (N % 96 == 0) return 96;
  if (N % 64 == 0) return 64;
  if (N <= 32) return 32;
  int best = 128, waste = static_cast<int>(round_up(N, 128)) - N;
  for (int bn : {96, 64}) {
    const int w = static_cast<int>(round_up(N, bn)) - N;
    if (w < waste) best = bn, waste = w;
  }
  return best;
}

static __global__ void pack_weight_kernel(const float* __restrict__ w, float* __restrict__ hi, float* __restrict__ lo, int N,
                                   int K, int Kp, int f16, float scale) {
  const int64_t i = static_cast<int64_t>(blockIdx.x) * blockDim.x + threadIdx.x;
  if (i >= static_cast<int64_t>(N) * K) return;
  const int n = static_cast<int>(i / K), k = static_cast<int>(i % K);
  const float v = w[i];
  const int64_t o = static_cast<int64_t>(n) * Kp + k;
  if (f16) {
    ptx::split_f16(v * scale, reinterpret_cast<__half*>(hi)[o], reinterpret_cast<__half*>(lo)[o]);
  } else {
    const float h = ptx::to_tf32(v);
    hi[o] = h;
    lo[o] = v - h;
  }
}

static __global__ void fold_ln_kernel(const float* __restrict__ W, const float* __restrict__ gamma,
                                      const float* __restrict__ beta, const float* __restrict__ bias, int K,
                                      float* __restrict__ Wf, float* __restrict__ c, float* __restrict__ d) {
  const int n = blockIdx.x;
  double sc = 0.0, sd = 0.0;
  for (int k = threadIdx.x; k < K; k += blockDim.x) {
    const float w = W[static_cast<int64_t>(n) * K + k];
    const float wf = gamma[k] * w;
    Wf[static_cast<int64_t>(n) * K + k] = wf;
    sc += static_cast<double>(wf);
    sd += static_cast<double>(beta[k]) * static_cast<double>(w);
  }
  __shared__ double rc[256], rd[256];
  rc[threadIdx.x] = sc, rd[threadIdx.x] = sd;
  __syncthreads();
  for (int s = blockDim.x / 2; s > 0; s >>= 1) {
    if (threadIdx.x < s) rc[threadIdx.x] += rc[threadIdx.x + s], rd[threadIdx.x] += rd[threadIdx.x + s];
    __syncthreads();
  }
  if (threadIdx.x == 0) {
    c[n] = static_cast<float>(rc[0]);
    d[n] = static_cast<float>(static_cast<double>(bias[n]) + rd[0]);
  }
}

static int pack_weight(rohm_posenet* pn, const float* w, int N, int K, PackedWeight* out, int kind);

static int pack_folded(rohm_posenet* pn, const float* w, const float* bias, const float* gamma, const float* beta, int N, int K,
                       PackedWeight* out, float** c, float** d) {
  float* wf = nullptr;
  if (cudaMalloc(&wf, static_cast<size_t>(N) * K * sizeof(float)) != cudaSuccess)
    return fail(pn->ctx, ROHM_ERR_CUDA, "folded weight scratch alloc failed");
  *c = pn->pool.floats(N), *d = pn->pool.floats(N);
  int rc = ROHM_OK;
  if (*c == nullptr || *d == nullptr) {
    rc = fail(pn->ctx, ROHM_ERR_CUDA, "alloc failed: %s", cudaGetErrorString(pn->pool.last_error()));
  } else {
    fold_ln_kernel<<<N, 256>>>(w, gamma, beta, bias, K, wf, *c, *d);
    if (cudaGetLastError() != cudaSuccess) rc = fail(pn->ctx, ROHM_ERR_CUDA, "fold_ln_kernel launch failed");
    if (rc == ROHM_OK) rc = pack_weight(pn, wf, N, K, out, pn->kind);
    if (rc == ROHM_OK && cudaDeviceSynchronize() != cudaSuccess) rc = fail(pn->ctx, ROHM_ERR_CUDA, "weight folding failed");
  }
  cudaFree(wf);
  return rc;
}

static int pack_weight(rohm_posenet* pn, const float* w, int N, int K, PackedWeight* out, int kind) {
  out->N = N, out->K = K;
  out->block_n = pick_block_n(N);
  out->Np = static_cast<int>(round_up(N, out->block_n));
  out->Kp = static_cast<int>(round_up(K, gemm_block_k(kind)));
  out->kind = kind;
  out->scale = 1.0f;
  const int64_t bytes = static_cast<int64_t>(out->Np) * out->Kp * gemm_elem_bytes(kind);
  out->hi = static_cast<float*>(pn->pool.bytes(bytes));
  out->lo = static_cast<float*>(pn->pool.bytes(bytes));
  if (out->hi == nullptr || out->lo == nullptr)
    return fail(pn->ctx, ROHM_ERR_CUDA, "weight alloc failed: %s", cudaGetErrorString(pn->pool.last_error()));
  const int64_t n = static_cast<int64_t>(N) * K;
  if (kind == kKindF16) ROHM_CUDA(pn->ctx, f16_weight_scale(w, n, &out->scale));
  pack_weight_kernel<<<static_cast<unsigned>((n + 255) / 256), 256>>>(w, out->hi, out->lo, N, K, out->Kp,
                                                                     kind == kKindF16 ? 1 : 0, out->scale);
  ROHM_CUDA(pn->ctx, cudaGetLastError());
  return ROHM_OK;
}

static int copy_vec(rohm_posenet* pn, const float* src, int64_t n, float** dst) {
  *dst = pn->pool.floats(n);
  if (*dst == nullptr) return fail(pn->ctx, ROHM_ERR_CUDA, "alloc failed: %s", cudaGetErrorString(pn->pool.last_error()));
  ROHM_CUDA(pn->ctx, cudaMemcpy(*dst, src, static_cast<size_t>(n) * sizeof(float), cudaMemcpyDeviceToDevice));
  return ROHM_OK;
}

static int setup_linear(rohm_posenet* pn, GemmParams* g, const float* a_hi, const float* a_lo, int64_t rows, int K, int lda,
                 const PackedWeight& w, const float* bias) {
  *g = GemmParams{};
  int rc = make_tmap_2d(&g->a_hi[0], a_hi, rows, K, lda, kGemmBlockM, 1, w.kind);
  rc |= make_tmap_2d(&g->a_lo[0], a_lo, rows, K, lda, kGemmBlockM, 1, w.kind);
  rc |= make_tmap_2d(&g->b_hi, w.hi, w.Np, w.Kp, w.Kp, w.block_n, 1, w.kind);
  rc |= make_tmap_2d(&g->b_lo, w.lo, w.Np, w.Kp, w.Kp, w.block_n, 1, w.kind);
  if (rc != 0) return fail(pn->ctx, ROHM_ERR_CUDA, "cuTensorMapEncodeTiled failed (%d)", rc);
  g->num_segs = 1;
  g->seg_kblocks[0] = w.Kp / gemm_block_k(w.kind);
  g->acc_scale = 1.0f / w.scale;
  g->seg_row_shift[0] = 0;
  g->seg_row_mul[0] = 1;
  g->bias = bias;
  g->N = w.N;
  g->out_row_mul = 1;
  g->out_row_add = 0;
  return ROHM_OK;
}

static int run_gemm(rohm_posenet* pn, GemmParams& g, const PackedWeight& w, int rows, cudaStream_t st) {
  g.M = rows;
  prof_begin(pn, kCatGemm, st);
  ROHM_CUDA(pn->ctx, launch_gemm(g, rows, w.N, w.block_n, pn->passes, st, pn->use_pdl && !pn->profiling, w.kind));
  prof_end(pn, st);
  pn->launches++;
  return ROHM_OK;
}

template <int D>
static void launch_ln(const float* in, const float* res, const float* g, const float* b, float* out, float* oh, float* ol,
               int rows, cudaStream_t st, int f16, bool pdl) {
  launch_chain(layernorm_kernel<D>, dim3((rows + 7) / 8), dim3(256), 0, st, pdl, in, res, g, b, out, oh, ol, rows, f16);
}

static int run_ln(rohm_posenet* pn, const float* in, const float* res, const float* g, const float* b, float* out, float* oh,
           float* ol, int rows, cudaStream_t st) {
  prof_begin(pn, kCatLayerNorm, st);
  const int f16 = pn->kind == kKindF16 ? 1 : 0;
  const bool pdl = pn->use_pdl && !pn->profiling;
  switch (pn->D) {
    case 128: launch_ln<128>(in, res, g, b, out, oh, ol, rows, st, f16, pdl); break;
    case 256: launch_ln<256>(in, res, g, b, out, oh, ol, rows, st, f16, pdl); break;
    case 512: launch_ln<512>(in, res, g, b, out, oh, ol, rows, st, f16, pdl); break;
    case 1024: launch_ln<1024>(in, res, g, b, out, oh, ol, rows, st, f16, pdl); break;
    default: return fail(pn->ctx, ROHM_ERR_INVALID, "unsupported d_model %d for LayerNorm", pn->D);
  }
  prof_end(pn, st);
  ROHM_CUDA(pn->ctx, cudaGetLastError());
  pn->launches++;
  return ROHM_OK;
}

static int run_attention(rohm_posenet* pn, int B, int S, cudaStream_t st) {
  if (!pn->lengths.empty()) {
    const int n_long = B - pn->n_short;
    for (int k = 0; k < 2; ++k) {
      AttnArgs a = pn->attn;
      a.clip_off = pn->clip_off;
      a.clip_ids = pn->clip_ids + (k == 0 ? 0 : pn->n_short);
      a.B = k == 0 ? pn->n_short : n_long;
      a.S = k == 0 ? pn->short_tokens : pn->long_tokens;
      if (a.B == 0) continue;
      prof_begin(pn, kCatAttention, st);
      const cudaError_t e = launch_attention(a, k == 0 ? kAttnWgmma : kAttnWgmmaStream, &pn->attn_wg, st,
                                             pn->use_pdl && !pn->profiling);
      prof_end(pn, st);
      ROHM_CUDA(pn->ctx, e);
      pn->launches++;
    }
    return ROHM_OK;
  }
  AttnArgs a = pn->attn;
  a.B = B, a.S = S;
  const bool maps = pn->attn_maps && (pn->tc_attention || S > kAttnWgmmaMaxTokens);
  prof_begin(pn, kCatAttention, st);
  const cudaError_t e = launch_attention(a, kAttnAuto, maps ? &pn->attn_wg : nullptr, st, pn->use_pdl && !pn->profiling);
  prof_end(pn, st);
  ROHM_CUDA(pn->ctx, e);
  pn->launches++;
  return ROHM_OK;
}

static int build_time_table(rohm_posenet* pn, const rohm_posenet_weights* w) {
  const int D = pn->D, R = pn->pe_len;
  const int64_t n = static_cast<int64_t>(R) * D;
  pn->time_table = pn->pool.floats(n);
  if (pn->time_table == nullptr) return fail(pn->ctx, ROHM_ERR_CUDA, "time table alloc failed");
  DevicePool tmp;
  PackedWeight w0, w2;
  float* pe_h = tmp.floats(n);
  float* pe_l = tmp.floats(n);
  float* h_h = tmp.floats(n);
  float* h_l = tmp.floats(n);
  float* bias2 = tmp.floats(D);
  if (!pe_h || !pe_l || !h_h || !h_l || !bias2) return fail(pn->ctx, ROHM_ERR_CUDA, "time table scratch alloc failed");
  int rc;
  if ((rc = pack_weight(pn, w->t0_w, D, D, &w0, kKindTf32)) != ROHM_OK) return rc;
  if ((rc = pack_weight(pn, w->t2_w, D, D, &w2, kKindTf32)) != ROHM_OK) return rc;
  ROHM_CUDA(pn->ctx, launch_split_tf32(pn->pe, pe_h, pe_l, n, 0));
  add_vec_kernel<<<(D + 255) / 256, 256>>>(w->t2_b, pn->pe, bias2, D);
  ROHM_CUDA(pn->ctx, cudaGetLastError());
  GemmParams g1{}, g2{};
  if ((rc = setup_linear(pn, &g1, pe_h, pe_l, R, D, D, w0, w->t0_b)) != ROHM_OK) return rc;
  g1.act = kActSilu;
  g1.out_hi = h_h, g1.out_lo = h_l, g1.lds = D;
  g1.M = R;
  ROHM_CUDA(pn->ctx, launch_gemm(g1, R, D, w0.block_n, 3, 0));
  if ((rc = setup_linear(pn, &g2, h_h, h_l, R, D, D, w2, bias2)) != ROHM_OK) return rc;
  g2.out = pn->time_table, g2.ldo = D;
  g2.M = R;
  ROHM_CUDA(pn->ctx, launch_gemm(g2, R, D, w2.block_n, 3, 0));
  ROHM_CUDA(pn->ctx, cudaDeviceSynchronize());
  return ROHM_OK;
}

extern "C" int rohm_posenet_create(rohm_ctx* ctx, const rohm_posenet_weights* w, int max_batch, int max_frames,
                                   int precision, rohm_posenet** out) {
  if (ctx == nullptr) return ROHM_ERR_INVALID;
  rohm::DeviceGuard device_guard__(ctx);
  if (w == nullptr || out == nullptr || max_batch <= 0 || max_frames <= 0)
    return fail(ctx, ROHM_ERR_INVALID, "rohm_posenet_create: bad arguments");
  if (precision != ROHM_PRECISION_TF32X3 && precision != ROHM_PRECISION_TF32 && precision != ROHM_PRECISION_F16X2)
    return fail(ctx, ROHM_ERR_INVALID, "rohm_posenet_create: precision must be 3 (TF32x3), 2 (F16x2) or 1 (TF32)");
  if (w->d_model % 128 != 0 || w->d_model % w->num_heads != 0 || w->ff_size % 64 != 0)
    return fail(ctx, ROHM_ERR_INVALID, "rohm_posenet_create: d_model must be a multiple of 128, ff_size of 64");
  const int dh = w->d_model / w->num_heads;
  if (dh != 64 && dh != 128) return fail(ctx, ROHM_ERR_INVALID, "rohm_posenet_create: head dim must be 64 or 128");
  if (max_frames + 1 > w->pe_len)
    return fail(ctx, ROHM_ERR_INVALID, "rohm_posenet_create: %d frames need %d rows of the positional table, which has %d",
                max_frames, max_frames + 1, w->pe_len);
  if (!(precision == ROHM_PRECISION_F16X2 && dh == 128)) {
    int simt_frames = kAttnSimtMaxTokens - 1;
    while (attention_smem_bytes(simt_frames + 1, dh) > kAttnSmemLimit) --simt_frames;
    if (max_frames > simt_frames)
      return fail(ctx, ROHM_ERR_INVALID,
                  "rohm_posenet_create: %d frames per clip: precision f16x2 with head dim 128 reaches pe_len - 1 = %d "
                  "frames; the tf32x3 / tf32 precisions and head dim 64 reach %d frames at head dim %d",
                  max_frames, w->pe_len - 1, simt_frames, dh);
  }

  rohm_posenet* pn = new (std::nothrow) rohm_posenet();
  if (pn == nullptr) return fail(ctx, ROHM_ERR_INVALID, "out of host memory");
  pn->ctx = ctx;
  pn->D = w->d_model, pn->F = w->ff_size, pn->L = w->num_layers, pn->H = w->num_heads;
  pn->C = w->in_feats, pn->Cout = w->out_feats, pn->traj = w->traj_feats, pn->pe_len = w->pe_len;
  pn->kind = precision == ROHM_PRECISION_F16X2 ? kKindF16 : kKindTf32;
  pn->passes = precision == ROHM_PRECISION_TF32 ? 1 : 3;
  pn->max_batch = max_batch, pn->max_frames = max_frames;
  pn->max_rows = static_cast<int64_t>(max_batch) * (max_frames + 1);
  pn->Kin_p = static_cast<int>(round_up(pn->C, gemm_block_k(pn->kind)));
  {
    const char* env = getenv("ROHM_B200_TC_ATTENTION");
    pn->tc_attention = pn->kind == kKindF16 && dh == 128 && (env == nullptr || env[0] != '0');
  }
  const int D = pn->D, F = pn->F;
  const int64_t R = pn->max_rows;
  {
    const char* env = getenv("ROHM_B200_FUSED_LN");
    pn->fused_ln = pn->kind == kKindF16 && D == 512 && (env == nullptr || env[0] != '0');
    if (pn->fused_ln) {
      pn->stats1 = static_cast<float2*>(pn->pool.bytes(R * 8 * static_cast<int64_t>(sizeof(float2))));
      pn->stats2 = static_cast<float2*>(pn->pool.bytes(R * 8 * static_cast<int64_t>(sizeof(float2))));
      if (pn->stats1 == nullptr || pn->stats2 == nullptr) {
        const int rc = fail(ctx, ROHM_ERR_CUDA, "LayerNorm statistics buffers: %s", cudaGetErrorString(pn->pool.last_error()));
        delete pn;
        return rc;
      }
    }
  }

#define TRY(expr)            \
  do {                       \
    int rc__ = (expr);       \
    if (rc__ != ROHM_OK) {   \
      delete pn;             \
      return rc__;           \
    }                        \
  } while (0)

  TRY(pack_weight(pn, w->in_w, D, pn->C, &pn->w_in, pn->kind));
  TRY(pack_weight(pn, w->cond_w, D, pn->C, &pn->w_cond, pn->kind));
  if (pn->fused_ln && pn->L > 0) {
    const rohm_posenet_layer& last = w->layers[pn->L - 1];
    TRY(pack_folded(pn, w->out_w, w->out_b, last.norm2_w, last.norm2_b, pn->Cout, D, &pn->w_out, &pn->out_c, &pn->out_d));
  } else {
    TRY(pack_weight(pn, w->out_w, pn->Cout, D, &pn->w_out, pn->kind));
  }
  TRY(copy_vec(pn, w->in_b, D, &pn->in_b));
  TRY(copy_vec(pn, w->cond_b, D, &pn->cond_b));
  TRY(copy_vec(pn, w->out_b, pn->Cout, &pn->out_b));
  TRY(copy_vec(pn, w->pe, static_cast<int64_t>(pn->pe_len) * D, &pn->pe));
  TRY(build_time_table(pn, w));
  pn->layers.resize(pn->L);
  for (int l = 0; l < pn->L; ++l) {
    const rohm_posenet_layer& s = w->layers[l];
    PoseNetLayerDev& d = pn->layers[l];
    if (pn->fused_ln && l > 0) {
      const rohm_posenet_layer& prev = w->layers[l - 1];
      TRY(pack_folded(pn, s.in_proj_w, s.in_proj_b, prev.norm2_w, prev.norm2_b, 3 * D, D, &d.qkv, &d.qkv_c, &d.qkv_d));
    } else {
      TRY(pack_weight(pn, s.in_proj_w, 3 * D, D, &d.qkv, pn->kind));
    }
    TRY(pack_weight(pn, s.out_proj_w, D, D, &d.proj, pn->kind));
    if (pn->fused_ln) {
      TRY(pack_folded(pn, s.lin1_w, s.lin1_b, s.norm1_w, s.norm1_b, F, D, &d.ff1, &d.ff1_c, &d.ff1_d));
    } else {
      TRY(pack_weight(pn, s.lin1_w, F, D, &d.ff1, pn->kind));
    }
    TRY(pack_weight(pn, s.lin2_w, D, F, &d.ff2, pn->kind));
    TRY(copy_vec(pn, s.in_proj_b, 3 * D, &d.qkv_b));
    TRY(copy_vec(pn, s.out_proj_b, D, &d.proj_b));
    TRY(copy_vec(pn, s.lin1_b, F, &d.ff1_b));
    TRY(copy_vec(pn, s.lin2_b, D, &d.ff2_b));
    TRY(copy_vec(pn, s.norm1_w, D, &d.n1_w));
    TRY(copy_vec(pn, s.norm1_b, D, &d.n1_b));
    TRY(copy_vec(pn, s.norm2_w, D, &d.n2_w));
    TRY(copy_vec(pn, s.norm2_b, D, &d.n2_b));
  }

  struct {
    float** p;
    int64_t n;
  } bufs[] = {{&pn->Ain_h, R * pn->Kin_p}, {&pn->Ain_l, R * pn->Kin_p}, {&pn->X, R * D},     {&pn->Xh, R * D},
              {&pn->Xl, R * D},           {&pn->Y, R * D},             {&pn->QKV, R * 3 * D}, {&pn->CTXh, R * D},
              {&pn->CTXl, R * D},         {&pn->Hh, R * F},            {&pn->Hl, R * F},      {&pn->condpe, R * D},
              {&pn->OUT, R * pn->Cout},
              {&pn->cond_traj, static_cast<int64_t>(max_batch) * (pn->traj > 0 ? pn->traj : 1) * max_frames}};
  for (auto& b : bufs) {
    *b.p = pn->pool.floats(b.n);
    if (*b.p == nullptr) {
      const int rc = fail(ctx, ROHM_ERR_CUDA, "workspace alloc failed: %s", cudaGetErrorString(pn->pool.last_error()));
      delete pn;
      return rc;
    }
  }

  pn->clip_off = static_cast<int*>(pn->pool.bytes(static_cast<int64_t>(max_batch + 1) * sizeof(int)));
  pn->clip_ids = static_cast<int*>(pn->pool.bytes(static_cast<int64_t>(max_batch) * sizeof(int)));
  if (pn->clip_off == nullptr || pn->clip_ids == nullptr) {
    const int rc = fail(ctx, ROHM_ERR_CUDA, "clip table alloc failed: %s", cudaGetErrorString(pn->pool.last_error()));
    delete pn;
    return rc;
  }

  TRY(setup_linear(pn, &pn->g_in, pn->Ain_h, pn->Ain_l, R, pn->C, pn->Kin_p, pn->w_in, pn->in_b));
  pn->g_in.residual = pn->condpe, pn->g_in.ldr = D;
  pn->g_in.out = pn->X, pn->g_in.ldo = D;
  pn->g_in.out_hi = pn->Xh, pn->g_in.out_lo = pn->Xl, pn->g_in.lds = D;
  TRY(setup_linear(pn, &pn->g_cond, pn->Ain_h, pn->Ain_l, R, pn->C, pn->Kin_p, pn->w_cond, pn->cond_b));
  pn->g_cond.residual = pn->condpe, pn->g_cond.ldr = D;
  pn->g_cond.out = pn->condpe, pn->g_cond.ldo = D;
  TRY(setup_linear(pn, &pn->g_out, pn->Xh, pn->Xl, R, D, D, pn->w_out, pn->out_b));
  pn->g_out.out = pn->OUT, pn->g_out.ldo = pn->Cout;
  if (pn->fused_ln && pn->L > 0)
    pn->g_out.a_stats = pn->stats2, pn->g_out.a_corr = pn->out_c, pn->g_out.bias = pn->out_d, pn->g_out.ln_eps = 1e-5f;
  pn->g_qkv.resize(pn->L), pn->g_proj.resize(pn->L), pn->g_ff1.resize(pn->L), pn->g_ff2.resize(pn->L);
  for (int l = 0; l < pn->L; ++l) {
    PoseNetLayerDev& d = pn->layers[l];
    TRY(setup_linear(pn, &pn->g_qkv[l], pn->Xh, pn->Xl, R, D, D, d.qkv, d.qkv_b));
    if (pn->kind == kKindF16) {
      pn->g_qkv[l].out_hi = pn->QKV;
      pn->g_qkv[l].out_lo = reinterpret_cast<__half*>(pn->QKV) + R * 3 * D;
      pn->g_qkv[l].lds = 3 * D;
    } else {
      pn->g_qkv[l].out = pn->QKV, pn->g_qkv[l].ldo = 3 * D;
    }
    TRY(setup_linear(pn, &pn->g_proj[l], pn->CTXh, pn->CTXl, R, D, D, d.proj, d.proj_b));
    pn->g_proj[l].out = pn->Y, pn->g_proj[l].ldo = D;
    auto producer = [&](GemmParams& g, float2* stats_out, const float2* res_stats, const float* res_gamma, const float* res_beta) {
      g.out = nullptr, g.ldo = 0;
      g.out_hi = pn->Xh, g.out_lo = pn->Xl, g.lds = D;
      g.stats_out = stats_out, g.res_stats = res_stats, g.res_gamma = res_gamma, g.res_beta = res_beta, g.ln_eps = 1e-5f;
    };
    auto consumer = [&](GemmParams& g, const float2* a_stats, const float* c, const float* dvec) {
      g.a_stats = a_stats, g.a_corr = c, g.bias = dvec, g.ln_eps = 1e-5f;
    };
    if (pn->fused_ln) {
      if (l > 0) consumer(pn->g_qkv[l], pn->stats2, d.qkv_c, d.qkv_d);
      producer(pn->g_proj[l], pn->stats1, l > 0 ? pn->stats2 : nullptr, l > 0 ? pn->layers[l - 1].n2_w : nullptr,
               l > 0 ? pn->layers[l - 1].n2_b : nullptr);
    }
    TRY(setup_linear(pn, &pn->g_ff1[l], pn->Xh, pn->Xl, R, D, D, d.ff1, d.ff1_b));
    pn->g_ff1[l].act = kActGelu;
    pn->g_ff1[l].out_hi = pn->Hh, pn->g_ff1[l].out_lo = pn->Hl, pn->g_ff1[l].lds = F;
    TRY(setup_linear(pn, &pn->g_ff2[l], pn->Hh, pn->Hl, R, F, F, d.ff2, d.ff2_b));
    pn->g_ff2[l].out = pn->Y, pn->g_ff2[l].ldo = D;
    if (pn->fused_ln) {
      consumer(pn->g_ff1[l], pn->stats1, d.ff1_c, d.ff1_d);
      producer(pn->g_ff2[l], pn->stats2, pn->stats1, d.n1_w, d.n1_b);
    }
    for (GemmParams* g : {&pn->g_qkv[l], &pn->g_proj[l], &pn->g_ff1[l], &pn->g_ff2[l]}) {
      if (gemm_enable_tma_store(g, R, pn->kind) != 0) {
        const int rc__ = fail(ctx, ROHM_ERR_CUDA, "cuTensorMapEncodeTiled (store map) failed");
        delete pn;
        return rc__;
      }
    }
  }
  if (gemm_enable_tma_store(&pn->g_out, R, pn->kind) != 0) {
    const int rc__ = fail(ctx, ROHM_ERR_CUDA, "cuTensorMapEncodeTiled (store map) failed");
    delete pn;
    return rc__;
  }
#undef TRY

  {
    cudaError_t ea = gemm_init_attributes();
    if (ea == cudaSuccess) ea = attention_init_attributes(max_frames + 1, dh);
    if (ea != cudaSuccess) {
      delete pn;
      return fail(ctx, ROHM_ERR_CUDA, "kernel attribute setup failed: %s", cudaGetErrorString(ea));
    }
  }
  pn->attn.qkv_hi = pn->QKV;
  pn->attn.qkv_lo = reinterpret_cast<const __half*>(pn->QKV) + R * 3 * D;
  pn->attn.rows = R;
  pn->attn.ctx_hi = pn->CTXh, pn->attn.ctx_lo = pn->CTXl;
  pn->attn.D = D, pn->attn.H = pn->H;
  pn->attn.scale = 1.0f / sqrtf(static_cast<float>(dh));
  pn->attn.kind = pn->kind;
  pn->attn_maps = pn->kind == kKindF16 && dh == 128;
  if (pn->attn_maps) {
    const int rcm = attention_wgmma_maps(&pn->attn_wg, pn->attn);
    if (rcm != 0) {
      delete pn;
      return fail(ctx, ROHM_ERR_CUDA, "cuTensorMapEncodeTiled (attention tiles) failed (%d)", rcm);
    }
  }
  const cudaError_t e = cudaDeviceSynchronize();
  if (e != cudaSuccess) {
    delete pn;
    return fail(ctx, ROHM_ERR_CUDA, "weight packing failed: %s", cudaGetErrorString(e));
  }
  *out = pn;
  return ROHM_OK;
}

extern "C" void rohm_posenet_destroy(rohm_posenet* pn) { delete pn; }

extern "C" int rohm_posenet_launches_per_forward(const rohm_posenet* pn) { return pn ? pn->launches : 0; }

static int check_lengths(rohm_posenet* pn, int B, int T, const char* fn) {
  if (pn->lengths.empty()) return ROHM_OK;
  if (static_cast<int>(pn->lengths.size()) != B)
    return fail(pn->ctx, ROHM_ERR_INVALID, "%s: lengths were set for %d clips, the call has B=%d", fn,
                static_cast<int>(pn->lengths.size()), B);
  for (int b = 0; b < B; ++b)
    if (pn->lengths[b] > T)
      return fail(pn->ctx, ROHM_ERR_INVALID, "%s: lengths[%d] = %d exceeds T=%d", fn, b, pn->lengths[b], T);
  return ROHM_OK;
}

extern "C" int rohm_posenet_set_cond(rohm_posenet* pn, const float* cond, int B, int T, void* stream) {
  if (pn == nullptr) return ROHM_ERR_INVALID;
  rohm_ctx* ctx = pn->ctx;
  rohm::DeviceGuard device_guard__(ctx);
  if (cond == nullptr || B <= 0 || T <= 0 || B > pn->max_batch || T > pn->max_frames)
    return fail(ctx, ROHM_ERR_INVALID, "rohm_posenet_set_cond: B=%d T=%d outside the created capacity (%d, %d)", B, T,
                pn->max_batch, pn->max_frames);
  int rc = check_lengths(pn, B, T, "rohm_posenet_set_cond");
  if (rc != ROHM_OK) return rc;
  cudaStream_t st = static_cast<cudaStream_t>(stream);
  const int S = T + 1, D = pn->D;
  const bool packed = !pn->lengths.empty();
  const int* off = packed ? pn->clip_off : nullptr;
  const int rows = packed ? pn->packed_rows : B * S;
  dim3 grid((T + 31) / 32, (pn->C + 31) / 32, B);
  pack_tokens_kernel<<<grid, dim3(32, 8), 0, st>>>(cond, pn->Ain_h, pn->Ain_l, pn->C, T, S, pn->Kin_p,
                                                   pn->kind == kKindF16 ? 1 : 0, off);
  ROHM_CUDA(ctx, cudaGetLastError());
  const int64_t clip4 = static_cast<int64_t>(S) * D / 4;
  pe_rows_kernel<<<dim3(static_cast<unsigned>((clip4 + 255) / 256), B), 256, 0, st>>>(pn->pe, pn->condpe, T, S, D, off);
  ROHM_CUDA(ctx, cudaGetLastError());
  const int saved = pn->launches;
  rc = run_gemm(pn, pn->g_cond, pn->w_cond, rows, st);
  pn->launches = saved;
  if (rc != ROHM_OK) return rc;
  if (pn->traj > 0) {
    const size_t width = static_cast<size_t>(pn->traj) * T * sizeof(float);
    ROHM_CUDA(ctx, cudaMemcpy2DAsync(pn->cond_traj, width, cond, static_cast<size_t>(pn->C) * T * sizeof(float), width,
                                     B, cudaMemcpyDeviceToDevice, st));
  }
  pn->cond_B = B, pn->cond_T = T;
  pn->cond_lengths = pn->lengths;
  return ROHM_OK;
}

extern "C" int rohm_posenet_set_lengths(rohm_posenet* pn, const int* lengths, int B) {
  if (pn == nullptr) return ROHM_ERR_INVALID;
  rohm_ctx* ctx = pn->ctx;
  rohm::DeviceGuard device_guard__(ctx);
  if (lengths == nullptr) {
    pn->lengths.clear();
    return ROHM_OK;
  }
  if (!pn->attn_maps || !pn->tc_attention)
    return fail(ctx, ROHM_ERR_INVALID,
                "rohm_posenet_set_lengths: per-clip lengths run on the wgmma attention kernels: precision f16x2 with head "
                "dim 128 only (the tf32x3 / tf32 precisions, head dim 64 and ROHM_B200_TC_ATTENTION=0 are not supported)");
  if (B <= 0 || B > pn->max_batch)
    return fail(ctx, ROHM_ERR_INVALID, "rohm_posenet_set_lengths: B=%d outside the created capacity %d", B, pn->max_batch);
  for (int b = 0; b < B; ++b)
    if (lengths[b] < 1 || lengths[b] > pn->max_frames)
      return fail(ctx, ROHM_ERR_INVALID, "rohm_posenet_set_lengths: lengths[%d] = %d outside [1, %d]", b, lengths[b],
                  pn->max_frames);
  std::vector<int> v(lengths, lengths + B);
  if (v == pn->lengths) return ROHM_OK;
  std::vector<int> off(B + 1), ids;
  int n_short = 0, short_tokens = 0, long_tokens = 0;
  off[0] = 0;
  for (int b = 0; b < B; ++b) off[b + 1] = off[b] + v[b] + 1;
  for (int pass = 0; pass < 2; ++pass)
    for (int b = 0; b < B; ++b) {
      const int S = v[b] + 1;
      const bool is_short = S <= kAttnWgmmaMaxTokens;
      if (is_short != (pass == 0)) continue;
      ids.push_back(b);
      if (is_short) ++n_short, short_tokens = S > short_tokens ? S : short_tokens;
      else long_tokens = S > long_tokens ? S : long_tokens;
    }
  ROHM_CUDA(ctx, cudaDeviceSynchronize());
  ROHM_CUDA(ctx, cudaMemcpy(pn->clip_off, off.data(), (B + 1) * sizeof(int), cudaMemcpyHostToDevice));
  ROHM_CUDA(ctx, cudaMemcpy(pn->clip_ids, ids.data(), B * sizeof(int), cudaMemcpyHostToDevice));
  pn->lengths = std::move(v);
  pn->packed_rows = off[B];
  pn->n_short = n_short, pn->short_tokens = short_tokens, pn->long_tokens = long_tokens;
  return ROHM_OK;
}

static int forward_launches(rohm_posenet* pn, const float* x_t, const int64_t* timesteps, float* out, int B, int T,
                            cudaStream_t st) {
  rohm_ctx* ctx = pn->ctx;
  rohm::DeviceGuard device_guard__(ctx);
  const int S = T + 1, D = pn->D;
  const bool packed = !pn->lengths.empty();
  const int* off = packed ? pn->clip_off : nullptr;
  const int rows = packed ? pn->packed_rows : B * S;
  pn->launches = 0;
  int rc;

  dim3 grid((T + 31) / 32, (pn->C + 31) / 32, B);
  prof_begin(pn, kCatOther, st);
  const bool pdl = pn->use_pdl && !pn->profiling;
  ROHM_CUDA(ctx, launch_chain(pack_tokens_kernel, grid, dim3(32, 8), 0, st, pdl, x_t, pn->Ain_h, pn->Ain_l, pn->C, T, S, pn->Kin_p,
                              pn->kind == kKindF16 ? 1 : 0, off));
  prof_end(pn, st);
  ROHM_CUDA(ctx, cudaGetLastError());
  pn->launches++;
  if ((rc = run_gemm(pn, pn->g_in, pn->w_in, rows, st)) != ROHM_OK) return rc;
  prof_begin(pn, kCatOther, st);
  ROHM_CUDA(ctx, launch_chain(time_token_gather_kernel, dim3(B), dim3(128), 0, st, pdl, timesteps, pn->time_table, pn->pe_len,
                              pn->X, pn->Xh, pn->Xl, S, D, pn->kind == kKindF16 ? 1 : 0, off));
  prof_end(pn, st);
  ROHM_CUDA(ctx, cudaGetLastError());
  pn->launches++;

  for (int l = 0; l < pn->L; ++l) {
    PoseNetLayerDev& d = pn->layers[l];
    if ((rc = run_gemm(pn, pn->g_qkv[l], d.qkv, rows, st)) != ROHM_OK) return rc;
    if ((rc = run_attention(pn, B, S, st)) != ROHM_OK) return rc;
    if ((rc = run_gemm(pn, pn->g_proj[l], d.proj, rows, st)) != ROHM_OK) return rc;
    if (!pn->fused_ln && (rc = run_ln(pn, pn->Y, pn->X, d.n1_w, d.n1_b, pn->X, pn->Xh, pn->Xl, rows, st)) != ROHM_OK) return rc;
    if ((rc = run_gemm(pn, pn->g_ff1[l], d.ff1, rows, st)) != ROHM_OK) return rc;
    if ((rc = run_gemm(pn, pn->g_ff2[l], d.ff2, rows, st)) != ROHM_OK) return rc;
    if (!pn->fused_ln && (rc = run_ln(pn, pn->Y, pn->X, d.n2_w, d.n2_b, pn->X, pn->Xh, pn->Xl, rows, st)) != ROHM_OK) return rc;
  }
  if ((rc = run_gemm(pn, pn->g_out, pn->w_out, rows, st)) != ROHM_OK) return rc;
  dim3 grid_o((T + 31) / 32, (pn->Cout + 31) / 32, B);
  prof_begin(pn, kCatOther, st);
  ROHM_CUDA(ctx, launch_chain(unpack_tokens_kernel, grid_o, dim3(32, 8), 0, st, pdl, pn->OUT, pn->cond_traj, out, pn->C, pn->Cout,
                              pn->traj, T, S, pn->Cout, off));
  prof_end(pn, st);
  ROHM_CUDA(ctx, cudaGetLastError());
  pn->launches++;
  return ROHM_OK;
}

extern "C" int rohm_posenet_forward(rohm_posenet* pn, const float* x_t, const int64_t* timesteps, float* out, int B,
                                    int T, void* stream);

extern "C" int rohm_posenet_profile(rohm_posenet* pn, const float* x_t, const int64_t* timesteps, float* out, int B,
                                    int T, void* stream, float* ms_by_category, int* launches_by_category) {
  if (pn == nullptr) return ROHM_ERR_INVALID;
  if (ms_by_category == nullptr || launches_by_category == nullptr)
    return fail(pn->ctx, ROHM_ERR_INVALID, "rohm_posenet_profile: null output");
  pn->profiling = true;
  pn->prof_events.clear();
  pn->prof_cat.clear();
  int rc = rohm_posenet_forward(pn, x_t, timesteps, out, B, T, stream);
  pn->profiling = false;
  cudaError_t e = cudaStreamSynchronize(static_cast<cudaStream_t>(stream));
  for (int c = 0; c < kNumCats; ++c) ms_by_category[c] = 0.0f, launches_by_category[c] = 0;
  for (size_t i = 0; i < pn->prof_cat.size(); ++i) {
    float ms = 0.0f;
    if (rc == ROHM_OK && e == cudaSuccess) cudaEventElapsedTime(&ms, pn->prof_events[2 * i], pn->prof_events[2 * i + 1]);
    ms_by_category[pn->prof_cat[i]] += ms;
    launches_by_category[pn->prof_cat[i]]++;
  }
  for (cudaEvent_t ev : pn->prof_events) cudaEventDestroy(ev);
  pn->prof_events.clear();
  pn->prof_cat.clear();
  if (rc != ROHM_OK) return rc;
  ROHM_CUDA(pn->ctx, e);
  return ROHM_OK;
}

static int forward_or_step(rohm_posenet* pn, const float* x_t, const int64_t* timesteps, float* out, int B, int T,
                           void* stream, const DdpmStep* step) {
  if (pn == nullptr) return ROHM_ERR_INVALID;
  rohm_ctx* ctx = pn->ctx;
  rohm::DeviceGuard device_guard__(ctx);
  if (x_t == nullptr || timesteps == nullptr || out == nullptr)
    return fail(ctx, ROHM_ERR_INVALID, "rohm_posenet_forward: null pointer");
  if (B != pn->cond_B || T != pn->cond_T)
    return fail(ctx, ROHM_ERR_STATE, "rohm_posenet_forward: B=%d T=%d but set_cond was called with B=%d T=%d", B, T,
                pn->cond_B, pn->cond_T);
  if (pn->lengths != pn->cond_lengths)
    return fail(ctx, ROHM_ERR_STATE, "rohm_posenet_forward: the clip lengths differ from those set_cond was called with");
  auto launches = [&](cudaStream_t st) {
    const int rc = forward_launches(pn, x_t, timesteps, out, B, T, st);
    if (rc != ROHM_OK || step == nullptr) return rc;
    pn->launches++;
    return launch_ddpm_step(ctx, *step, st, pn->use_pdl && !pn->profiling);
  };
  std::vector<KernelPatch> patches = {{pack_tokens_kernel, arg<kPackTokensX>(x_t)},
                                      {time_token_gather_kernel, arg<kTimeTokenTimesteps>(timesteps)},
                                      {unpack_tokens_kernel, arg<kUnpackTokensOut>(out)}};
  if (step != nullptr) patches.push_back(ddpm_step_patch(*step));
  return pn->graphs.run(ctx, B, T, step != nullptr, pn->profiling, static_cast<cudaStream_t>(stream), launches, patches,
                        pn->lengths);
}

extern "C" int rohm_posenet_forward(rohm_posenet* pn, const float* x_t, const int64_t* timesteps, float* out, int B,
                                    int T, void* stream) {
  return forward_or_step(pn, x_t, timesteps, out, B, T, stream, nullptr);
}

extern "C" int rohm_posenet_sample_step(rohm_posenet* pn, const float* x_t, const int64_t* timesteps, float* x0_out,
                                        float* x_next, const float* coef_row, uint64_t seed, uint64_t offset,
                                        uint64_t* offset_increment, int B, int T, void* stream) {
  if (pn == nullptr) return ROHM_ERR_INVALID;
  if (x_next == nullptr || coef_row == nullptr)
    return fail(pn->ctx, ROHM_ERR_INVALID, "rohm_posenet_sample_step: null pointer");
  const int64_t clip_elems = static_cast<int64_t>(pn->C) * T;
  DdpmStep step{x0_out, x_t, x_next, clip_elems * B, clip_elems, coef_row, seed, offset};
  const int rc = ddpm_step_plan(pn->ctx, &step, offset_increment);
  if (rc != ROHM_OK) return rc;
  return forward_or_step(pn, x_t, timesteps, x0_out, B, T, stream, &step);
}

extern "C" int rohm_posenet_set_option(rohm_posenet* pn, int option, int value) {
  if (pn == nullptr) return ROHM_ERR_INVALID;
  if (option == 0) {
    pn->graphs.enabled = value != 0;
    return ROHM_OK;
  }
  if (option == 1) {
    if (pn->use_pdl != (value != 0)) pn->graphs.clear();
    pn->use_pdl = value != 0;
    return ROHM_OK;
  }
  return fail(pn->ctx, ROHM_ERR_INVALID, "rohm_posenet_set_option: unknown option %d", option);
}
```

rohm_b200/csrc/ptx.cuh:

```cuda
#pragma once
#include <cstdint>
#include <cuda.h>
#include <cuda_fp16.h>
#include <cuda_runtime.h>

namespace rohm {
namespace ptx {

__device__ __forceinline__ uint32_t smem_u32(const void* p) {
  return static_cast<uint32_t>(__cvta_generic_to_shared(p));
}

__device__ __forceinline__ bool elect_one() {
  uint32_t pred = 0;
  asm volatile(
      "{\n\t"
      ".reg .pred P;\n\t"
      "elect.sync _|P, 0xffffffff;\n\t"
      "selp.u32 %0, 1, 0, P;\n\t"
      "}\n"
      : "=r"(pred));
  return pred != 0;
}

__device__ __forceinline__ void mbar_init(uint64_t* bar, uint32_t count) {
  asm volatile("mbarrier.init.shared::cta.b64 [%0], %1;" ::"r"(smem_u32(bar)), "r"(count));
}
__device__ __forceinline__ void fence_barrier_init() {
  asm volatile("fence.mbarrier_init.release.cluster;" ::: "memory");
}
__device__ __forceinline__ void fence_proxy_async() {
  asm volatile("fence.proxy.async.shared::cta;" ::: "memory");
}
__device__ __forceinline__ void mbar_expect_tx(uint64_t* bar, uint32_t bytes) {
  asm volatile("mbarrier.arrive.expect_tx.shared::cta.b64 _, [%0], %1;" ::"r"(smem_u32(bar)), "r"(bytes)
               : "memory");
}
__device__ __forceinline__ void mbar_arrive(uint64_t* bar) {
  asm volatile("mbarrier.arrive.shared::cta.b64 _, [%0];" ::"r"(smem_u32(bar)) : "memory");
}
__device__ __forceinline__ bool mbar_try_wait(uint64_t* bar, uint32_t parity) {
  uint32_t ok;
  asm volatile(
      "{\n\t"
      ".reg .pred P;\n\t"
      "mbarrier.try_wait.parity.shared::cta.b64 P, [%1], %2;\n\t"
      "selp.u32 %0, 1, 0, P;\n\t"
      "}\n"
      : "=r"(ok)
      : "r"(smem_u32(bar)), "r"(parity)
      : "memory");
  return ok != 0;
}
__device__ __forceinline__ void mbar_wait(uint64_t* bar, uint32_t parity) {
  while (!mbar_try_wait(bar, parity)) {
  }
}

__device__ __forceinline__ void prefetch_tmap(const CUtensorMap* m) {
  asm volatile("prefetch.tensormap [%0];" ::"l"(reinterpret_cast<uint64_t>(m)) : "memory");
}
__device__ __forceinline__ void tma_load_2d(void* smem_dst, const CUtensorMap* m, uint64_t* bar, int32_t c0,
                                            int32_t c1) {
  asm volatile(
      "cp.async.bulk.tensor.2d.shared::cluster.global.tile.mbarrier::complete_tx::bytes [%0], [%1, {%3, %4}], [%2];"
      ::"r"(smem_u32(smem_dst)),
      "l"(reinterpret_cast<uint64_t>(m)), "r"(smem_u32(bar)), "r"(c0), "r"(c1)
      : "memory");
}
__device__ __forceinline__ void tma_load_3d(void* smem_dst, const CUtensorMap* m, uint64_t* bar, int32_t c0,
                                            int32_t c1, int32_t c2) {
  asm volatile(
      "cp.async.bulk.tensor.3d.shared::cluster.global.tile.mbarrier::complete_tx::bytes [%0], [%1, {%3, %4, %5}], "
      "[%2];" ::"r"(smem_u32(smem_dst)),
      "l"(reinterpret_cast<uint64_t>(m)), "r"(smem_u32(bar)), "r"(c0), "r"(c1), "r"(c2)
      : "memory");
}

__device__ __forceinline__ void tma_store_2d(const CUtensorMap* m, const void* smem_src, int32_t c0, int32_t c1) {
  asm volatile("cp.async.bulk.tensor.2d.global.shared::cta.bulk_group [%0, {%2, %3}], [%1];" ::"l"(
                   reinterpret_cast<uint64_t>(m)),
               "r"(smem_u32(smem_src)), "r"(c0), "r"(c1)
               : "memory");
}
__device__ __forceinline__ void bulk_load_1d(void* smem_dst, const void* gsrc, uint32_t bytes, uint64_t* bar) {
  asm volatile("cp.async.bulk.shared::cluster.global.mbarrier::complete_tx::bytes [%0], [%1], %2, [%3];" ::"r"(smem_u32(smem_dst)),
               "l"(gsrc), "r"(bytes), "r"(smem_u32(bar))
               : "memory");
}
__device__ __forceinline__ void bulk_commit() { asm volatile("cp.async.bulk.commit_group;" ::: "memory"); }
__device__ __forceinline__ void bulk_wait_read_all() { asm volatile("cp.async.bulk.wait_group.read 0;" ::: "memory"); }
__device__ __forceinline__ void bulk_wait_all() { asm volatile("cp.async.bulk.wait_group 0;" ::: "memory"); }

__device__ __forceinline__ void wgmma_fence() { asm volatile("wgmma.fence.sync.aligned;" ::: "memory"); }
__device__ __forceinline__ void wgmma_commit() { asm volatile("wgmma.commit_group.sync.aligned;" ::: "memory"); }
template <int N>
__device__ __forceinline__ void wgmma_wait() {
  asm volatile("wgmma.wait_group.sync.aligned %0;" ::"n"(N) : "memory");
}
template <int R>
__device__ __forceinline__ void wgmma_fence_regs(float (&d)[R]) {
#pragma unroll
  for (int i = 0; i < R; ++i) asm volatile("" : "+f"(d[i])::"memory");
}
template <int R>
__device__ __forceinline__ void setmaxnreg_dec() {
  asm volatile("setmaxnreg.dec.sync.aligned.u32 %0;" ::"n"(R));
}
template <int R>
__device__ __forceinline__ void setmaxnreg_inc() {
  asm volatile("setmaxnreg.inc.sync.aligned.u32 %0;" ::"n"(R));
}
template <int kRowBytes>
__device__ __forceinline__ uint64_t make_desc_kmajor(uint32_t smem_addr) {
  static_assert(kRowBytes == 128 || kRowBytes == 64, "row = one swizzle span");
  uint64_t d = 0;
  d |= static_cast<uint64_t>((smem_addr & 0x3FFFFu) >> 4);
  d |= static_cast<uint64_t>(1) << 16;
  d |= static_cast<uint64_t>((8 * kRowBytes) >> 4) << 32;
  d |= static_cast<uint64_t>(kRowBytes == 128 ? 1 : 2) << 62;
  return d;
}

__device__ __forceinline__ uint64_t make_desc_mnmajor_sw128(uint32_t smem_addr, uint32_t lbo_bytes, uint32_t sbo_bytes) {
  uint64_t d = 0;
  d |= static_cast<uint64_t>((smem_addr & 0x3FFFFu) >> 4);
  d |= static_cast<uint64_t>((lbo_bytes >> 4) & 0x3FFFu) << 16;
  d |= static_cast<uint64_t>((sbo_bytes >> 4) & 0x3FFFu) << 32;
  d |= static_cast<uint64_t>(1) << 62;
  return d;
}

#define ROHM_R16_0 "%0, %1, %2, %3, %4, %5, %6, %7, %8, %9, %10, %11, %12, %13, %14, %15"
#define ROHM_R16_1 "%16, %17, %18, %19, %20, %21, %22, %23, %24, %25, %26, %27, %28, %29, %30, %31"
#define ROHM_R16_2 "%32, %33, %34, %35, %36, %37, %38, %39, %40, %41, %42, %43, %44, %45, %46, %47"
#define ROHM_R16_3 "%48, %49, %50, %51, %52, %53, %54, %55, %56, %57, %58, %59, %60, %61, %62, %63"
#define ROHM_R16_4 "%64, %65, %66, %67, %68, %69, %70, %71, %72, %73, %74, %75, %76, %77, %78, %79"
#define ROHM_F4(i) "+f"(d[i]), "+f"(d[i + 1]), "+f"(d[i + 2]), "+f"(d[i + 3])
#define ROHM_F16(i) ROHM_F4(i), ROHM_F4(i + 4), ROHM_F4(i + 8), ROHM_F4(i + 12)
#define ROHM_PRED(n) "{\n\t.reg .pred p;\n\tsetp.ne.b32 p, %" #n ", 0;\n\t"

#define ROHM_WGMMA_SS(KIND, INSTR, R, REGS, A, B, P, IMM, ...)                                                       \
  __device__ __forceinline__ void wgmma_##KIND(float (&d)[R], uint64_t desc_a, uint64_t desc_b) {                 \
    asm volatile(ROHM_PRED(P) INSTR " {" REGS "}, %" #A ", %" #B ", p" IMM ";\n\t}\n"                           \
                 : __VA_ARGS__                                                                                    \
                 : "l"(desc_a), "l"(desc_b), "r"(1));                                                             \
  }
ROHM_WGMMA_SS(f16, "wgmma.mma_async.sync.aligned.m64n32k16.f32.f16.f16", 16, ROHM_R16_0, 16, 17, 18, ", 1, 1, 0, 0",
              ROHM_F16(0))
ROHM_WGMMA_SS(f16, "wgmma.mma_async.sync.aligned.m64n64k16.f32.f16.f16", 32, ROHM_R16_0 ", " ROHM_R16_1, 32, 33, 34,
              ", 1, 1, 0, 0", ROHM_F16(0), ROHM_F16(16))
ROHM_WGMMA_SS(f16, "wgmma.mma_async.sync.aligned.m64n96k16.f32.f16.f16", 48,
              ROHM_R16_0 ", " ROHM_R16_1 ", " ROHM_R16_2, 48, 49, 50, ", 1, 1, 0, 0", ROHM_F16(0), ROHM_F16(16), ROHM_F16(32))
ROHM_WGMMA_SS(f16, "wgmma.mma_async.sync.aligned.m64n128k16.f32.f16.f16", 64,
              ROHM_R16_0 ", " ROHM_R16_1 ", " ROHM_R16_2 ", " ROHM_R16_3, 64, 65, 66, ", 1, 1, 0, 0", ROHM_F16(0),
              ROHM_F16(16), ROHM_F16(32), ROHM_F16(48))
ROHM_WGMMA_SS(f16, "wgmma.mma_async.sync.aligned.m64n160k16.f32.f16.f16", 80,
              ROHM_R16_0 ", " ROHM_R16_1 ", " ROHM_R16_2 ", " ROHM_R16_3 ", " ROHM_R16_4, 80, 81, 82, ", 1, 1, 0, 0",
              ROHM_F16(0), ROHM_F16(16), ROHM_F16(32), ROHM_F16(48), ROHM_F16(64))
ROHM_WGMMA_SS(tf32, "wgmma.mma_async.sync.aligned.m64n32k8.f32.tf32.tf32", 16, ROHM_R16_0, 16, 17, 18, ", 1, 1", ROHM_F16(0))
ROHM_WGMMA_SS(tf32, "wgmma.mma_async.sync.aligned.m64n64k8.f32.tf32.tf32", 32, ROHM_R16_0 ", " ROHM_R16_1, 32, 33, 34,
              ", 1, 1", ROHM_F16(0), ROHM_F16(16))
ROHM_WGMMA_SS(tf32, "wgmma.mma_async.sync.aligned.m64n96k8.f32.tf32.tf32", 48, ROHM_R16_0 ", " ROHM_R16_1 ", " ROHM_R16_2,
              48, 49, 50, ", 1, 1", ROHM_F16(0), ROHM_F16(16), ROHM_F16(32))
ROHM_WGMMA_SS(tf32, "wgmma.mma_async.sync.aligned.m64n128k8.f32.tf32.tf32", 64,
              ROHM_R16_0 ", " ROHM_R16_1 ", " ROHM_R16_2 ", " ROHM_R16_3, 64, 65, 66, ", 1, 1", ROHM_F16(0), ROHM_F16(16),
              ROHM_F16(32), ROHM_F16(48))

__device__ __forceinline__ void wgmma_f16_rs_tb(float (&d)[64], const uint32_t (&a)[4], uint64_t desc_b) {
  asm volatile(ROHM_PRED(69) "wgmma.mma_async.sync.aligned.m64n128k16.f32.f16.f16 {" ROHM_R16_0 ", " ROHM_R16_1 ", " ROHM_R16_2
               ", " ROHM_R16_3 "}, {%64, %65, %66, %67}, %68, p, 1, 1, 1;\n\t}\n"
               : ROHM_F16(0), ROHM_F16(16), ROHM_F16(32), ROHM_F16(48)
               : "r"(a[0]), "r"(a[1]), "r"(a[2]), "r"(a[3]), "l"(desc_b), "r"(1));
}

__device__ __forceinline__ float to_tf32(float x) {
  uint32_t r;
  asm("cvt.rna.tf32.f32 %0, %1;" : "=r"(r) : "f"(x));
  return __uint_as_float(r);
}

__device__ __forceinline__ void split_f16(float x, __half& hi, __half& lo) {
  const float c = fminf(fmaxf(x, -65504.0f), 65504.0f);
  hi = __float2half_rn(c);
  lo = __float2half_rn(x - __half2float(hi));
}
__device__ __forceinline__ void split_f16x2(float x, float y, uint32_t& hi, uint32_t& lo) {
  asm("cvt.rn.satfinite.f16x2.f32 %0, %1, %2;" : "=r"(hi) : "f"(y), "f"(x));
  const float2 hf = __half22float2(*reinterpret_cast<const __half2*>(&hi));
  const float lx = x - hf.x, ly = y - hf.y;
  asm("cvt.rn.satfinite.f16x2.f32 %0, %1, %2;" : "=r"(lo) : "f"(ly), "f"(lx));
}
__device__ __forceinline__ void split_f16x4(const float4& v, uint2& hi, uint2& lo) {
  split_f16x2(v.x, v.y, hi.x, lo.x);
  split_f16x2(v.z, v.w, hi.y, lo.y);
}

__device__ __forceinline__ void pdl_wait_prior_grid() { asm volatile("griddepcontrol.wait;" ::: "memory"); }
__device__ __forceinline__ void pdl_launch_dependents() { asm volatile("griddepcontrol.launch_dependents;" ::: "memory"); }

}
}
```

Baseline: 19.97.

## Chain per-layer proj/FF1/FF2/next-QKV GEMMs into one persistent dataflow kernel

Adds a chained GEMM launch that runs up to four dependent GEMMs (attention projection, FF1, FF2, next layer's QKV) in a single persistent kernel. CTAs take work items from a global atomic counter, and each stage's row-block waits on per-row-block completion counters from the previous stage before issuing TMA loads. The aim is to cut kernel launch count and the tail gaps between dependent GEMMs so stages overlap across row blocks. In exchange it adds spin-wait synchronisation with a timeout status flag and a per-forward memset of the counters, and the chained stages cannot carry a residual input.

```diff
diff --git a/include/rohm_b200.h b/include/rohm_b200.h
--- a/include/rohm_b200.h
+++ b/include/rohm_b200.h
@@ -113,6 +113,8 @@
 
 ROHM_API int rohm_posenet_set_option(rohm_posenet* pn, int option, int value);
 
+ROHM_API int rohm_posenet_chain_status(const rohm_posenet* pn, int* status);
+
 ROHM_API int rohm_posenet_launches_per_forward(const rohm_posenet* pn);
 
 
diff --git a/rohm_b200/_lib.py b/rohm_b200/_lib.py
--- a/rohm_b200/_lib.py
+++ b/rohm_b200/_lib.py
@@ -49,6 +49,7 @@
     "rohm_posenet_profile": (_i, [_p, _p, _p, _p, _i, _i, _p, C.POINTER(C.c_float), C.POINTER(C.c_int)]),
     "rohm_posenet_set_option": (_i, [_p, _i, _i]),
     "rohm_posenet_launches_per_forward": (_i, [_p]),
+    "rohm_posenet_chain_status": (_i, [_p, _p]),
     "rohm_trajnet_create": (_i, [_p, _i, C.POINTER(C.c_char_p), C.POINTER(_p), C.POINTER(_i64), _i, _i, _i, _i, _i, _i,
                                  _i, _i, _i, C.POINTER(_p)]),
     "rohm_trajnet_destroy": (None, [_p]),
diff --git a/rohm_b200/csrc/gemm.cu b/rohm_b200/csrc/gemm.cu
--- a/rohm_b200/csrc/gemm.cu
+++ b/rohm_b200/csrc/gemm.cu
@@ -6,6 +6,7 @@
 #include <cstdio>
 #include <cstring>
 #include <mutex>
+#include <type_traits>
 
 namespace rohm {
 
@@ -116,6 +117,41 @@
   int ldr, ldo, lds, act, M, N, out_row_mul, out_row_add, clip_rows, clip_valid;
 };
 
+struct ChainStage {
+  CUtensorMap a_hi, a_lo, b_hi, b_lo, st_hi, st_lo;
+  EpiParams epi;
+  int kblocks, row_shift, row_mul;
+  int tiles_n;
+  int first_item;
+  int kind;
+};
+struct GemmChainParams {
+  ChainStage stage[kMaxChainStages];
+  unsigned int* words;
+  int* status;
+  int num_stages, num_items, tiles_m;
+};
+static_assert(sizeof(GemmChainParams) <= 4096, "lean kernel parameter block: 4 KB");
+template <int EPI>
+using KernelParams = std::conditional_t<epi_role(EPI), GemmChainParams, GemmParams>;
+
+__device__ __forceinline__ int chain_stage_of(const GemmChainParams& c, int t) {
+  int s = 0;
+  while (s + 1 < c.num_stages && t >= c.stage[s + 1].first_item) ++s;
+  return s;
+}
+
+constexpr unsigned int kChainSpinLimit = 1u << 20;
+__device__ __forceinline__ void chain_wait(const unsigned int* counter, unsigned int target, int* status) {
+  for (unsigned int i = 0; ptx::ld_acquire_gpu(counter) < target; ++i) {
+    if (i >= kChainSpinLimit || ((i & 255) == 255 && *reinterpret_cast<volatile int*>(status) != kChainOk)) {
+      atomicExch(status, kChainErrWaitExpired);
+      return;
+    }
+    __nanosleep(64);
+  }
+}
+
 __device__ __forceinline__ float2 combine_row_stats(const float2* row8, float eps) {
   const float4* q4 = reinterpret_cast<const float4*>(row8);
   float4 t[4];
@@ -154,21 +190,26 @@
 }
 
 template <int BLOCK_N, int PASSES, int EPI, int KIND>
-__global__ void __launch_bounds__(kernel_threads(EPI), 1) gemm_tile_kernel(const __grid_constant__ GemmParams p) {
+__global__ void __launch_bounds__(kernel_threads(EPI), 1) gemm_tile_kernel(const __grid_constant__ KernelParams<EPI> p) {
   constexpr bool LEAN = EPI != 2 && EPI != 5;
   constexpr bool EPI_ROLE = epi_role(EPI);
+  constexpr bool kLnEpi = EPI == 0 && BLOCK_N == 128 && PASSES == 3 && KIND == kKindF16;
+  constexpr bool kResidual = !EPI_ROLE || EPI == 1;
   constexpr int kElemK = gemm_block_k(KIND);
   using Cfg = TileCfg<BLOCK_N, PASSES, EPI_ROLE>;
   constexpr int kEpiWarps = Cfg::kEpiWarps;
+  constexpr int kItemQ = 4;
   extern __shared__ uint8_t smem_raw[];
   __shared__ uint64_t full_bar[Cfg::kStages];
   __shared__ uint64_t empty_bar[Cfg::kStages];
-  __shared__ EpiParams epi_s;
+  __shared__ EpiParams epi_s[EPI_ROLE ? kMaxChainStages : 1];
   __shared__ __align__(16) float bias_s[BLOCK_N];
   __shared__ __align__(16) float corr_s[BLOCK_N];
-  __shared__ __align__(16) float beta_s[EPI == 3 ? BLOCK_N : 4];
-  __shared__ uint64_t res_bar[EPI == 3 ? kEpiWarps : 1];
+  __shared__ __align__(16) float beta_s[kLnEpi ? BLOCK_N : 4];
+  __shared__ uint64_t res_bar[kLnEpi ? kEpiWarps : 1];
   __shared__ uint64_t acc_full, acc_empty;
+  __shared__ int item_q[EPI_ROLE ? kItemQ : 1];
+  __shared__ uint64_t q_full[EPI_ROLE ? kItemQ : 1], q_empty[EPI_ROLE ? kItemQ : 1];
   __shared__ __align__(16) float skin_w_s[EPI == 4 ? 2 : 1][EPI == 4 ? kSkinTileBones * 32 : 4];
   __shared__ int skin_bone_s[EPI == 4 ? 2 : 1][EPI == 4 ? kSkinTileBones : 1];
   __shared__ int skin_nb_s[2];
@@ -180,28 +221,47 @@
 
   const int warp_idx = threadIdx.x >> 5;
   const int lane = threadIdx.x & 31;
-  const int tiles_n = (p.grid_n_cols + BLOCK_N - 1) / BLOCK_N;
-  const int tiles_m = (p.grid_m_rows + kGemmBlockM - 1) / kGemmBlockM;
-  const int num_tiles = tiles_m * tiles_n;
-
-  int total_iters = 0;
-  for (int s = 0; s < p.num_segs; ++s) total_iters += p.seg_kblocks[s];
-  const int S = (!LEAN && p.k_splits > 1) ? p.k_splits : 1;
-  const int per_split = (total_iters + S - 1) / S;
-  const int num_work = num_tiles * S;
+  int tiles_n = 0, num_tiles = 0, total_iters = 0, S = 1, per_split = 0, num_work = 0;
+  if constexpr (EPI_ROLE) {
+    num_work = p.num_items;
+  } else {
+    tiles_n = (p.grid_n_cols + BLOCK_N - 1) / BLOCK_N;
+    num_tiles = ((p.grid_m_rows + kGemmBlockM - 1) / kGemmBlockM) * tiles_n;
+    for (int s = 0; s < p.num_segs; ++s) total_iters += p.seg_kblocks[s];
+    S = (!LEAN && p.k_splits > 1) ? p.k_splits : 1;
+    per_split = (total_iters + S - 1) / S;
+    num_work = num_tiles * S;
+  }
+  auto item_iters = [&](int w) {
+    const int it_b = (w % S) * per_split;
+    return (total_iters < it_b + per_split ? total_iters : it_b + per_split) - it_b;
+  };
 
   if (warp_idx == 0 && lane == 0) {
-    ptx::prefetch_tmap(&p.b_hi);
-    if (PASSES == 3) ptx::prefetch_tmap(&p.b_lo);
-    for (int s = 0; s < p.num_segs; ++s) {
-      ptx::prefetch_tmap(&p.a_hi[s]);
-      if (PASSES == 3) ptx::prefetch_tmap(&p.a_lo[s]);
+    if constexpr (EPI_ROLE) {
+      for (int s = 0; s < p.num_stages; ++s) {
+        ptx::prefetch_tmap(&p.stage[s].b_hi);
+        if (PASSES == 3) ptx::prefetch_tmap(&p.stage[s].b_lo);
+        ptx::prefetch_tmap(&p.stage[s].a_hi);
+        if (PASSES == 3) ptx::prefetch_tmap(&p.stage[s].a_lo);
+      }
+      for (int i = 0; i < kItemQ; ++i) {
+        ptx::mbar_init(&q_full[i], 1);
+        ptx::mbar_init(&q_empty[i], kMmaWarps + kEpiWarps);
+      }
+    } else {
+      ptx::prefetch_tmap(&p.b_hi);
+      if (PASSES == 3) ptx::prefetch_tmap(&p.b_lo);
+      for (int s = 0; s < p.num_segs; ++s) {
+        ptx::prefetch_tmap(&p.a_hi[s]);
+        if (PASSES == 3) ptx::prefetch_tmap(&p.a_lo[s]);
+      }
     }
     for (int i = 0; i < Cfg::kStages; ++i) {
       ptx::mbar_init(&full_bar[i], 1);
       ptx::mbar_init(&empty_bar[i], 2);
     }
-    if (EPI == 3)
+    if (kLnEpi)
       for (int i = 0; i < kEpiWarps; ++i) ptx::mbar_init(&res_bar[i], 1);
     if (EPI_ROLE) {
       ptx::mbar_init(&acc_full, kMmaWarps);
@@ -210,10 +270,26 @@
     ptx::fence_barrier_init();
   }
   int prefetched = 0;
-  if (warp_idx == 0 && lane == 0 && static_cast<int>(blockIdx.x) < num_work) {
+  int first_item = static_cast<int>(blockIdx.x);
+  if constexpr (EPI_ROLE) {
+    if (warp_idx == 0 && lane == 0) {
+      if (p.words != nullptr) first_item = static_cast<int>(atomicAdd(p.words, 1u));
+      if (first_item < num_work) {
+        const ChainStage& cs = p.stage[chain_stage_of(p, first_item)];
+        const int n0 = ((first_item - cs.first_item) % cs.tiles_n) * BLOCK_N;
+        prefetched = cs.kblocks < Cfg::kStages ? cs.kblocks : Cfg::kStages;
+        for (int i = 0; i < prefetched; ++i) {
+          uint8_t* st = smem + i * Cfg::kStageBytes;
+          ptx::mbar_expect_tx(&full_bar[i], Cfg::kStageBytes);
+          ptx::tma_load_2d(st + Cfg::kSplit * Cfg::kABytes, &cs.b_hi, &full_bar[i], i * kElemK, n0);
+          if (PASSES == 3) ptx::tma_load_2d(st + 2 * Cfg::kABytes + Cfg::kBBytes, &cs.b_lo, &full_bar[i], i * kElemK, n0);
+        }
+      }
+    }
+  } else if (warp_idx == 0 && lane == 0 && static_cast<int>(blockIdx.x) < num_work) {
     const int tile0 = static_cast<int>(blockIdx.x) / S;
     const int it_b = (static_cast<int>(blockIdx.x) - tile0 * S) * per_split;
-    const int cnt = (total_iters < it_b + per_split ? total_iters : it_b + per_split) - it_b;
+    const int cnt = item_iters(static_cast<int>(blockIdx.x));
     const int n0 = (tile0 % tiles_n) * BLOCK_N;
     prefetched = cnt < Cfg::kStages ? cnt : Cfg::kStages;
     for (int i = 0; i < prefetched; ++i) {
@@ -225,19 +301,30 @@
     }
   }
   if (warp_idx == kFirstMmaWarp && lane == 0) {
-    epi_s.bias = p.bias, epi_s.residual = p.residual, epi_s.ldr = p.ldr, epi_s.out = p.out, epi_s.ldo = p.ldo;
-    epi_s.out_hi = p.out_hi, epi_s.out_lo = p.out_lo, epi_s.lds = p.lds, epi_s.act = p.act, epi_s.M = p.M, epi_s.N = p.N;
-    epi_s.out_row_mul = p.out_row_mul, epi_s.out_row_add = p.out_row_add, epi_s.clip_rows = p.clip_rows;
-    epi_s.clip_valid = p.clip_valid;
-    epi_s.acc_scale = p.acc_scale == 0.0f ? 1.0f : p.acc_scale;
-    epi_s.tma_store = p.tma_store;
-    epi_s.bias_per_row = p.bias_per_row;
-    epi_s.a_stats = p.a_stats, epi_s.a_corr = p.a_corr, epi_s.res_stats = p.res_stats, epi_s.res_gamma = p.res_gamma;
-    epi_s.res_beta = p.res_beta, epi_s.stats_out = p.stats_out, epi_s.ln_eps = p.ln_eps;
-    if (p.tma_store) {
-      ptx::prefetch_tmap(&p.st_out);
-      ptx::prefetch_tmap(&p.st_hi);
-      ptx::prefetch_tmap(&p.st_lo);
+    if constexpr (EPI_ROLE) {
+      for (int s = 0; s < p.num_stages; ++s) {
+        epi_s[s] = p.stage[s].epi;
+        if (p.stage[s].epi.tma_store) {
+          ptx::prefetch_tmap(&p.stage[s].st_hi);
+          ptx::prefetch_tmap(&p.stage[s].st_lo);
+        }
+      }
+    } else {
+      EpiParams& es = epi_s[0];
+      es.bias = p.bias, es.residual = p.residual, es.ldr = p.ldr, es.out = p.out, es.ldo = p.ldo;
+      es.out_hi = p.out_hi, es.out_lo = p.out_lo, es.lds = p.lds, es.act = p.act, es.M = p.M, es.N = p.N;
+      es.out_row_mul = p.out_row_mul, es.out_row_add = p.out_row_add, es.clip_rows = p.clip_rows;
+      es.clip_valid = p.clip_valid;
+      es.acc_scale = p.acc_scale == 0.0f ? 1.0f : p.acc_scale;
+      es.tma_store = p.tma_store;
+      es.bias_per_row = p.bias_per_row;
+      es.a_stats = p.a_stats, es.a_corr = p.a_corr, es.res_stats = p.res_stats, es.res_gamma = p.res_gamma;
+      es.res_beta = p.res_beta, es.stats_out = p.stats_out, es.ln_eps = p.ln_eps;
+      if (p.tma_store) {
+        ptx::prefetch_tmap(&p.st_out);
+        ptx::prefetch_tmap(&p.st_hi);
+        ptx::prefetch_tmap(&p.st_lo);
+      }
     }
   }
   __syncthreads();
@@ -247,7 +334,45 @@
 
   if (warp_idx < kFirstMmaWarp) {
     ptx::setmaxnreg_dec<kProducerRegs>();
-    if (warp_idx == 0 && lane == 0) {
+    if constexpr (EPI_ROLE) {
+      if (warp_idx == 0 && lane == 0) {
+        int it = 0, stage = 0;
+        uint32_t phase = 0;
+        for (int k = 0;; ++k) {
+          int t = first_item;
+          if (k > 0)
+            t = p.words != nullptr ? static_cast<int>(atomicAdd(p.words, 1u)) : static_cast<int>(blockIdx.x + k * gridDim.x);
+          const int slot = k % kItemQ;
+          ptx::mbar_wait(&q_empty[slot], static_cast<uint32_t>(((k / kItemQ) & 1) ^ 1));
+          item_q[slot] = t;
+          ptx::mbar_arrive(&q_full[slot]);
+          if (t >= num_work) break;
+          const int s = chain_stage_of(p, t);
+          const ChainStage& cs = p.stage[s];
+          const int tile = t - cs.first_item;
+          const int m0 = (tile / cs.tiles_n) * kGemmBlockM;
+          const int n0 = (tile % cs.tiles_n) * BLOCK_N;
+          if (s > 0) {
+            chain_wait(p.words + 1 + (s - 1) * p.tiles_m + m0 / kGemmBlockM, static_cast<unsigned int>(p.stage[s - 1].tiles_n),
+                       p.status);
+            ptx::fence_proxy_async_global();
+          }
+          const int row = m0 * cs.row_mul + cs.row_shift;
+          for (int kb = 0; kb < cs.kblocks; ++kb, ++it) {
+            uint8_t* st = smem + stage * Cfg::kStageBytes;
+            if (it >= prefetched) {
+              ptx::mbar_wait(&empty_bar[stage], phase ^ 1);
+              ptx::mbar_expect_tx(&full_bar[stage], Cfg::kStageBytes);
+              ptx::tma_load_2d(st + Cfg::kSplit * Cfg::kABytes, &cs.b_hi, &full_bar[stage], kb * kElemK, n0);
+              if (PASSES == 3) ptx::tma_load_2d(st + 2 * Cfg::kABytes + Cfg::kBBytes, &cs.b_lo, &full_bar[stage], kb * kElemK, n0);
+            }
+            ptx::tma_load_2d(st, &cs.a_hi, &full_bar[stage], kb * kElemK, row);
+            if (PASSES == 3) ptx::tma_load_2d(st + Cfg::kABytes, &cs.a_lo, &full_bar[stage], kb * kElemK, row);
+            if (++stage == Cfg::kStages) stage = 0, phase ^= 1;
+          }
+        }
+      }
+    } else if (warp_idx == 0 && lane == 0) {
       int it = 0, stage = 0;
       uint32_t phase = 0;
       for (int w = blockIdx.x; w < num_work; w += gridDim.x) {
@@ -295,15 +420,13 @@
     constexpr int kChunkStep = EPI_ROLE ? 32 : 64;
     int mma_stage = 0;
     uint32_t mma_phase = 0;
-    auto mma_tile = [&](int w, int tc) {
+    auto mma_tile = [&](int n_it, int tc) {
       float dm[Cfg::kAccRegs];
       float dc[PASSES == 3 ? Cfg::kAccRegs : 1];
 #pragma unroll
       for (int i = 0; i < Cfg::kAccRegs; ++i) dm[i] = 0.0f;
 #pragma unroll
       for (int i = 0; i < (PASSES == 3 ? Cfg::kAccRegs : 1); ++i) dc[i] = 0.0f;
-      const int it_b = (w % S) * per_split;
-      const int n_it = (total_iters < it_b + per_split ? total_iters : it_b + per_split) - it_b;
       const bool signaller = (threadIdx.x & 127) == 0;
       auto release = [&](int stg) {
         if (signaller) ptx::mbar_arrive(&empty_bar[stg]);
@@ -358,24 +481,36 @@
         asm volatile("bar.sync 3, %0;" ::"n"(kMmaWarps * 32));
       }
     };
+    auto pop_item = [&](int k) {
+      const int slot = k % kItemQ;
+      ptx::mbar_wait(&q_full[slot], static_cast<uint32_t>((k / kItemQ) & 1));
+      const int t = item_q[slot];
+      __syncwarp();
+      if (lane == 0) ptx::mbar_arrive(&q_empty[slot]);
+      return t;
+    };
     const bool epi_warp = !EPI_ROLE || !mma_warp;
     if (!epi_warp) {
       ptx::setmaxnreg_inc<kMmaRegs>();
-      int tc = 0;
-      for (int wi = blockIdx.x; wi < num_work; wi += gridDim.x, ++tc) mma_tile(wi, tc);
+      if constexpr (EPI_ROLE) {
+        for (int k = 0;; ++k) {
+          const int t = pop_item(k);
+          if (t >= num_work) break;
+          mma_tile(p.stage[chain_stage_of(p, t)].kblocks, k);
+        }
+      }
     } else if constexpr (EPI_ROLE) {
       ptx::setmaxnreg_inc<kEpiRoleRegs>();
     }
     EpiParams e_regs;
-    if constexpr (!EPI_ROLE) e_regs = epi_s;
-    const EpiParams& e = EPI_ROLE ? epi_s : e_regs;
-    const bool vec_ok = ((e.N & 3) == 0);
+    if constexpr (!EPI_ROLE) e_regs = epi_s[0];
     float* tile = reinterpret_cast<float*>(epi_smem) + ew * kEpiTileFloats;
     const int tr = lane >> 3, tc = (lane & 7) * 4;
     int tcount = 0;
     uint32_t res_phase = 0;
     if constexpr (EPI == 4) {
       static_assert(BLOCK_N == 96 && PASSES == 3 && KIND == kKindF16, "skinning epilogue: 32 vertices x 3 per tile, fp16 pairs");
+      const EpiParams& e = e_regs;
       constexpr int kSkinRegBones = 4;
       const int i = ew * 32 + lane;
       float4 sk[kSkinRegBones][3];
@@ -418,7 +553,7 @@
         int nbone = 0, nnb = 0;
         if (has_next) fetch_tables(next % tiles_n, nw0, nw1, nbone, nnb);
 
-        mma_tile(tile_idx, tcount);
+        mma_tile(item_iters(tile_idx), tcount);
         float o[48];
 #pragma unroll
         for (int j = 0; j < 48; ++j) o[j] = 0.0f;
@@ -510,11 +645,57 @@
         }
       }
     }
-    for (int wi = blockIdx.x; EPI != 4 && epi_warp && wi < num_work; wi += gridDim.x, ++tcount) {
-      const int tile_idx = wi / S;
-      const int split_rows = (wi - tile_idx * S) * (!LEAN ? p.split_row_stride : 0);
-      const int m0 = (tile_idx / tiles_n) * kGemmBlockM;
-      const int n0 = (tile_idx % tiles_n) * BLOCK_N;
+    for (int k = 0; EPI != 4 && epi_warp; ++k, ++tcount) {
+      int wi, stage = 0, tile_idx, tiles_n_s = tiles_n, split_rows = 0, epi_k = EPI;
+      if constexpr (EPI_ROLE) {
+        wi = pop_item(k);
+        if (wi >= num_work) break;
+        stage = chain_stage_of(p, wi);
+        const ChainStage& cs = p.stage[stage];
+        tile_idx = wi - cs.first_item;
+        tiles_n_s = cs.tiles_n;
+        epi_k = cs.kind;
+      } else {
+        wi = static_cast<int>(blockIdx.x) + k * static_cast<int>(gridDim.x);
+        if (wi >= num_work) break;
+        tile_idx = wi / S;
+        if constexpr (!LEAN) split_rows = (wi - tile_idx * S) * p.split_row_stride;
+      }
+      auto map_out = [&]() -> const CUtensorMap* {
+        if constexpr (EPI_ROLE) return &p.stage[stage].st_hi;
+        else return &p.st_out;
+      };
+      auto map_hi = [&]() -> const CUtensorMap* {
+        if constexpr (EPI_ROLE) return &p.stage[stage].st_hi;
+        else return &p.st_hi;
+      };
+      auto map_lo = [&]() -> const CUtensorMap* {
+        if constexpr (EPI_ROLE) return &p.stage[stage].st_lo;
+        else return &p.st_lo;
+      };
+      const EpiParams& e = EPI_ROLE ? epi_s[stage] : e_regs;
+      const bool vec_ok = ((e.N & 3) == 0);
+      const int m0 = (tile_idx / tiles_n_s) * kGemmBlockM;
+      const int n0 = (tile_idx % tiles_n_s) * BLOCK_N;
+      if constexpr (EPI_ROLE) {
+        if (stage > 0) {
+          chain_wait(p.words + 1 + (stage - 1) * p.tiles_m + m0 / kGemmBlockM,
+                     static_cast<unsigned int>(p.stage[stage - 1].tiles_n), p.status);
+          ptx::fence_proxy_async_global();
+        }
+      }
+      auto publish = [&]() {
+        if constexpr (EPI_ROLE) {
+          if (stage + 1 < p.num_stages) {
+            if (lane == 0) ptx::bulk_wait_all();
+            asm volatile("bar.sync 4, %0;" ::"n"(kEpiWarps * 32));
+            if (ew == 0 && lane == 0) {
+              ptx::fence_proxy_async_global();
+              ptx::red_release_gpu_add(p.words + 1 + stage * p.tiles_m + m0 / kGemmBlockM, 1u);
+            }
+          }
+        }
+      };
       const int m = m0 + q * 32 + lane;
       const bool row_ok = m < e.M;
       bool row_real = true;
@@ -529,14 +710,14 @@
         if (i < BLOCK_N) {
           const bool col_ok = n0 + i < e.N;
           bias_s[i] = (e.bias != nullptr && !e.bias_per_row && col_ok) ? __ldg(e.bias + n0 + i) : 0.0f;
-          if (EPI == 3) {
+          if (kLnEpi && epi_k == 3) {
             corr_s[i] = e.res_stats != nullptr ? __ldg(e.res_gamma + n0 + i) : 1.0f;
             beta_s[i] = e.res_stats != nullptr ? __ldg(e.res_beta + n0 + i) : 0.0f;
           } else {
             corr_s[i] = (e.a_stats != nullptr && col_ok) ? __ldg(e.a_corr + n0 + i) : 0.0f;
           }
         }
-        if (e.residual != nullptr && row_ok) {
+        if (kResidual && e.residual != nullptr && row_ok) {
           const float* r = e.residual + orow * e.ldr + n0 + half * 32;
 #pragma unroll
           for (int c = 0; c < (EPI_ROLE ? BLOCK_N : (BLOCK_N > 64 ? 128 : 64)); c += kChunkStep)
@@ -545,11 +726,11 @@
         asm volatile("bar.sync 1, %0;" ::"n"(kEpiWarps * 32));
       }
       float a_mean = 0.0f, a_rstd = 1.0f;
-      if (EPI != 3 && LEAN && e.a_stats != nullptr && row_ok) {
+      if (epi_k != 3 && LEAN && e.a_stats != nullptr && row_ok) {
         const float2 mr = combine_row_stats(e.a_stats + static_cast<int64_t>(m) * 8, e.ln_eps);
         a_mean = mr.x, a_rstd = mr.y;
       }
-      float lnv[EPI == 3 ? 2 : 1][EPI == 3 ? 32 : 1];
+      float lnv[kLnEpi ? 2 : 1][kLnEpi ? 32 : 1];
       float r_mean = 0.0f, r_rstd = 1.0f;
       auto load_residual = [&](int g) {
         uint8_t* tb = reinterpret_cast<uint8_t*>(tile);
@@ -560,8 +741,8 @@
           if (lane == 0) {
             ptx::bulk_wait_read_all();
             ptx::mbar_expect_tx(rb, 4096);
-            ptx::tma_load_2d(tb, &p.st_hi, rb, n0 + c0, m0 + q * 32);
-            ptx::tma_load_2d(tb + 2048, &p.st_lo, rb, n0 + c0, m0 + q * 32);
+            ptx::tma_load_2d(tb, map_hi(), rb, n0 + c0, m0 + q * 32);
+            ptx::tma_load_2d(tb + 2048, map_lo(), rb, n0 + c0, m0 + q * 32);
           }
           ptx::mbar_wait(rb, res_phase);
           res_phase ^= 1;
@@ -585,23 +766,23 @@
           __syncwarp();
         }
       };
-      if constexpr (EPI == 3) {
-        if (e.res_stats != nullptr && row_ok) {
-          const float2 mr = combine_row_stats(e.res_stats + static_cast<int64_t>(m) * 8, e.ln_eps);
-          r_mean = mr.x, r_rstd = mr.y;
-        }
-        load_residual(0);
+      if constexpr (kLnEpi) {
+        if (epi_k == 3) {
+          if (e.res_stats != nullptr && row_ok) {
+            const float2 mr = combine_row_stats(e.res_stats + static_cast<int64_t>(m) * 8, e.ln_eps);
+            r_mean = mr.x, r_rstd = mr.y;
+          }
+          load_residual(0);
+        }
       }
       if constexpr (EPI_ROLE) {
         ptx::mbar_wait(&acc_full, static_cast<uint32_t>(tcount & 1));
       } else {
-        mma_tile(wi, tcount);
-      }
-
-      if constexpr (EPI == 3) {
-        static_assert(BLOCK_N == 128 && PASSES == 3 && KIND == kKindF16, "LayerNorm-folding producer: fp16 pairs, 128-wide tiles");
-        static_assert(EPI_ROLE, "one thread per row: both 64-column statistics groups");
-        const int tile_n = tile_idx % tiles_n;
+        mma_tile(item_iters(wi), tcount);
+      }
+
+      if constexpr (kLnEpi) if (epi_k == 3) {
+        const int tile_n = tile_idx % tiles_n_s;
         float (&v)[2][32] = lnv;
         uint8_t* tb = reinterpret_cast<uint8_t*>(tile);
         const bool group_full = (m0 + q * 32 + 32 <= e.M);
@@ -629,7 +810,7 @@
           auto store_chunk = [&](int h2) {
             const int nb = n0 + g * 32 + 64 * h2;
             if (group_full) {
-              stage_pair_chunk(v[h2], tb, lane, &p.st_hi, &p.st_lo, nb, m0 + q * 32);
+              stage_pair_chunk(v[h2], tb, lane, map_hi(), map_lo(), nb, m0 + q * 32);
             } else if (row_ok) {
               __half* oh = static_cast<__half*>(e.out_hi) + static_cast<int64_t>(m) * e.lds + nb;
               __half* ol = static_cast<__half*>(e.out_lo) + static_cast<int64_t>(m) * e.lds + nb;
@@ -651,6 +832,7 @@
           if (row_ok) e.stats_out[static_cast<int64_t>(m) * 8 + tile_n * 2 + g] = make_float2(mean_i, m2_i);
           store_chunk(1);
         }
+        publish();
         continue;
       }
 
@@ -684,7 +866,7 @@
               for (int j = 0; j < 32; ++j) v[j] += bias_row;
             }
           }
-          if (EPI == 1) {
+          if (LEAN && epi_k == 1) {
 #pragma unroll
             for (int j = 0; j < 32; ++j) v[j] = gelu_erf(v[j]);
           }
@@ -727,17 +909,17 @@
           __syncwarp();
           if (lane == 0) {
             if (e.out != nullptr) {
-              ptx::tma_store_2d(&p.st_out, tb, nb, m0 + q * 32 + split_rows);
+              ptx::tma_store_2d(map_out(), tb, nb, m0 + q * 32 + split_rows);
             } else {
-              ptx::tma_store_2d(&p.st_hi, tb, nb, m0 + q * 32 + split_rows);
-              ptx::tma_store_2d(&p.st_lo, tb + 2048, nb, m0 + q * 32 + split_rows);
+              ptx::tma_store_2d(map_hi(), tb, nb, m0 + q * 32 + split_rows);
+              ptx::tma_store_2d(map_lo(), tb + 2048, nb, m0 + q * 32 + split_rows);
             }
             ptx::bulk_commit();
           }
           continue;
         }
         float4 res[8];
-        const bool use_res = e.residual != nullptr && full;
+        const bool use_res = kResidual && e.residual != nullptr && full;
         if (use_res) {
 #pragma unroll
           for (int rr = 0; rr < 8; ++rr) {
@@ -769,18 +951,18 @@
               for (int j = 0; j < 32; ++j) v[j] += bias_row;
             }
           }
-          if (EPI == 0) {
-          } else if (EPI == 1 || e.act == kActGelu) {
+          if (LEAN && epi_k == 0) {
+          } else if (epi_k == 1 || e.act == kActGelu) {
 #pragma unroll
             for (int j = 0; j < 32; ++j) v[j] = gelu_erf(v[j]);
-          } else if (e.act == kActSilu) {
+          } else if (!LEAN && e.act == kActSilu) {
 #pragma unroll
             for (int j = 0; j < 32; ++j) v[j] = v[j] / (1.0f + expf(-v[j]));
-          } else if (e.act == kActMish) {
+          } else if (!LEAN && e.act == kActMish) {
 #pragma unroll
             for (int j = 0; j < 32; ++j) v[j] = apply_act(v[j], kActMish);
           }
-          if (e.residual != nullptr && !full) {
+          if (kResidual && e.residual != nullptr && !full) {
             const float* r = e.residual + orow * e.ldr + nb;
 #pragma unroll
             for (int j = 0; j < 32; ++j)
@@ -863,6 +1045,7 @@
         __syncwarp();
         if (lane == 0) ptx::mbar_arrive(&acc_empty);
       }
+      publish();
     }
     if (lane == 0) ptx::bulk_wait_read_all();
   }
@@ -915,95 +1098,32 @@
 
 template <int BLOCK_N, int PASSES, int KIND>
 static cudaError_t set_attr() {
-  constexpr int kRoleSmem = TileCfg<BLOCK_N, PASSES, true>::kSmemBytes;
-  cudaError_t e = cudaFuncSetAttribute(gemm_tile_kernel<BLOCK_N, PASSES, 0, KIND>,
-                                       cudaFuncAttributeMaxDynamicSharedMemorySize, kRoleSmem);
+  cudaError_t e = cudaFuncSetAttribute(gemm_tile_kernel<BLOCK_N, PASSES, 0, KIND>, cudaFuncAttributeMaxDynamicSharedMemorySize,
+                                       TileCfg<BLOCK_N, PASSES, true>::kSmemBytes);
   if (e != cudaSuccess) return e;
-  e = cudaFuncSetAttribute(gemm_tile_kernel<BLOCK_N, PASSES, 1, KIND>, cudaFuncAttributeMaxDynamicSharedMemorySize, kRoleSmem);
+  e = cudaFuncSetAttribute(gemm_tile_kernel<BLOCK_N, PASSES, 1, KIND>, cudaFuncAttributeMaxDynamicSharedMemorySize,
+                           TileCfg<BLOCK_N, PASSES, true>::kSmemBytes);
   if (e != cudaSuccess) return e;
   e = cudaFuncSetAttribute(gemm_tile_kernel<BLOCK_N, PASSES, 2, KIND>, cudaFuncAttributeMaxDynamicSharedMemorySize,
                            TileCfg<BLOCK_N, PASSES, false>::kSmemBytes);
   if (e != cudaSuccess) return e;
-  e = cudaFuncSetAttribute(gemm_tile_kernel<BLOCK_N, PASSES, 5, KIND>, cudaFuncAttributeMaxDynamicSharedMemorySize,
-                           TileCfg<BLOCK_N, PASSES, false>::kSmemBytes);
-  if (e != cudaSuccess) return e;
-  if constexpr (BLOCK_N == 128 && PASSES == 3 && KIND == kKindF16)
-    e = cudaFuncSetAttribute(gemm_tile_kernel<BLOCK_N, PASSES, 3, KIND>, cudaFuncAttributeMaxDynamicSharedMemorySize, kRoleSmem);
-  return e;
-}
-
-template <int BLOCK_N, int PASSES, int KIND>
-cudaError_t launch_cfg(const GemmParams& p, int m_rows, int n_cols, cudaStream_t stream, bool pdl) {
-  using Cfg = TileCfg<BLOCK_N, PASSES, false>;
-  const bool plain = p.clip_rows == 0;
-  const int epi = (plain && p.act == kActNone) ? 0 : (plain && p.act == kActGelu) ? 1 : p.row_mask != nullptr ? 5 : 2;
-  auto kern = epi == 0   ? gemm_tile_kernel<BLOCK_N, PASSES, 0, KIND>
-              : epi == 1 ? gemm_tile_kernel<BLOCK_N, PASSES, 1, KIND>
-              : epi == 2 ? gemm_tile_kernel<BLOCK_N, PASSES, 2, KIND>
-                         : gemm_tile_kernel<BLOCK_N, PASSES, 5, KIND>;
-  int threads = kernel_threads(epi);
-  int smem_bytes = epi_role(epi) ? TileCfg<BLOCK_N, PASSES, true>::kSmemBytes : Cfg::kSmemBytes;
-  if (p.a_stats != nullptr && (!plain || p.a_corr == nullptr)) return cudaErrorInvalidValue;
-  if (p.row_mask != nullptr && plain) return cudaErrorInvalidValue;
-  if (p.stats_out != nullptr) {
-    if constexpr (BLOCK_N == 128 && PASSES == 3 && KIND == kKindF16) {
-      if (!plain || p.act != kActNone || n_cols != 4 * BLOCK_N || p.N != n_cols || !p.tma_store || p.out != nullptr ||
-          p.out_hi == nullptr || p.a_stats != nullptr || (p.res_stats != nullptr && (p.res_gamma == nullptr || p.res_beta == nullptr)))
-        return cudaErrorInvalidValue;
-      kern = gemm_tile_kernel<BLOCK_N, PASSES, 3, KIND>;
-      threads = kernel_threads(3);
-      smem_bytes = TileCfg<BLOCK_N, PASSES, true>::kSmemBytes;
-    } else {
-      return cudaErrorInvalidValue;
-    }
-  }
-  if (p.skin_A != nullptr) {
-    if constexpr (BLOCK_N == 96 && PASSES == 3 && KIND == kKindF16) {
-      if (!plain || p.act != kActNone || p.out == nullptr || p.skin_nb == nullptr || p.skin_bone == nullptr || p.skin_w == nullptr ||
-          p.bias != nullptr || p.residual != nullptr || p.a_stats != nullptr || p.stats_out != nullptr)
-        return cudaErrorInvalidValue;
-      kern = gemm_tile_kernel<BLOCK_N, PASSES, 4, KIND>;
-      threads = kernel_threads(4);
-      smem_bytes = Cfg::kStages * Cfg::kStageBytes + 1024 + Cfg::kAccBytes + kSkinStageBytes;
-      static bool skin_attr_set = false;
-      if (!skin_attr_set) {
-        cudaError_t e = cudaFuncSetAttribute(kern, cudaFuncAttributeMaxDynamicSharedMemorySize, smem_bytes);
-        if (e != cudaSuccess) return e;
-        skin_attr_set = true;
-      }
-    } else {
-      return cudaErrorInvalidValue;
-    }
-  }
-  static bool attr_set = false;
-  if (!attr_set) {
-    cudaError_t e = set_attr<BLOCK_N, PASSES, KIND>();
-    if (e != cudaSuccess) return e;
-    attr_set = true;
-  }
+  return cudaFuncSetAttribute(gemm_tile_kernel<BLOCK_N, PASSES, 5, KIND>, cudaFuncAttributeMaxDynamicSharedMemorySize,
+                              TileCfg<BLOCK_N, PASSES, false>::kSmemBytes);
+}
+
+static int sm_count() {
   static int num_sms = 0;
   if (num_sms == 0) {
     int dev = 0;
     cudaGetDevice(&dev);
     if (cudaDeviceGetAttribute(&num_sms, cudaDevAttrMultiProcessorCount, dev) != cudaSuccess || num_sms <= 0) num_sms = 132;
   }
-  GemmParams q = p;
-  q.grid_m_rows = m_rows;
-  q.grid_n_cols = n_cols;
-  int tiles = ((n_cols + BLOCK_N - 1) / BLOCK_N) * ((m_rows + kGemmBlockM - 1) / kGemmBlockM);
-  if (q.k_splits > 1) {
-    int iters = 0;
-    for (int s = 0; s < q.num_segs; ++s) iters += q.seg_kblocks[s];
-    const int per = (iters + q.k_splits - 1) / q.k_splits;
-    if (plain || q.out == nullptr || q.out_hi != nullptr || q.bias != nullptr || q.residual != nullptr ||
-        q.act != kActNone || q.out_row_mul != 1 || q.out_row_add != 0 || (q.k_splits - 1) * per >= iters ||
-        q.split_row_stride < m_rows)
-      return cudaErrorInvalidValue;
-    tiles *= q.k_splits;
-  }
+  return num_sms;
+}
+
+static cudaError_t launch_kernel(const void* kern, void** args, int grid, int threads, int smem_bytes, cudaStream_t stream,
+                                 bool pdl) {
   cudaLaunchConfig_t cfg{};
-  int grid = tiles < num_sms ? tiles : num_sms;
-  if (p.stats_out != nullptr) grid -= grid % 4;
   cfg.gridDim = dim3(grid, 1, 1);
   cfg.blockDim = dim3(threads, 1, 1);
   cfg.dynamicSmemBytes = smem_bytes;
@@ -1017,7 +1137,118 @@
   }
   cfg.attrs = attr;
   cfg.numAttrs = na;
-  return cudaLaunchKernelEx(&cfg, kern, q);
+  return cudaLaunchKernelExC(&cfg, kern, args);
+}
+
+template <int BLOCK_N, int PASSES, int KIND>
+cudaError_t fill_stage(const GemmParams& p, int n_cols, ChainStage* s) {
+  if (p.clip_rows != 0 || p.row_mask != nullptr || p.skin_A != nullptr || p.k_splits > 1 || p.num_segs != 1 ||
+      (p.act != kActNone && p.act != kActGelu) || (p.a_stats != nullptr && p.a_corr == nullptr))
+    return cudaErrorInvalidValue;
+  s->kind = p.act == kActGelu ? 1 : 0;
+  if (p.stats_out != nullptr) {
+    if constexpr (BLOCK_N == 128 && PASSES == 3 && KIND == kKindF16) {
+      if (p.act != kActNone || p.residual != nullptr || n_cols != 4 * BLOCK_N || p.N != n_cols || !p.tma_store || p.out != nullptr ||
+          p.out_hi == nullptr || p.a_stats != nullptr || (p.res_stats != nullptr && (p.res_gamma == nullptr || p.res_beta == nullptr)))
+        return cudaErrorInvalidValue;
+      s->kind = 3;
+    } else {
+      return cudaErrorInvalidValue;
+    }
+  }
+  s->a_hi = p.a_hi[0], s->a_lo = p.a_lo[0], s->b_hi = p.b_hi, s->b_lo = p.b_lo;
+  s->st_hi = p.out != nullptr ? p.st_out : p.st_hi;
+  s->st_lo = p.st_lo;
+  EpiParams& e = s->epi;
+  e = EpiParams{};
+  e.bias = p.bias, e.residual = p.residual, e.ldr = p.ldr, e.out = p.out, e.ldo = p.ldo;
+  e.out_hi = p.out_hi, e.out_lo = p.out_lo, e.lds = p.lds, e.act = p.act, e.M = p.M, e.N = p.N;
+  e.out_row_mul = p.out_row_mul, e.out_row_add = p.out_row_add, e.clip_rows = 0, e.clip_valid = 0;
+  e.acc_scale = p.acc_scale == 0.0f ? 1.0f : p.acc_scale;
+  e.tma_store = p.tma_store;
+  e.bias_per_row = p.bias_per_row;
+  e.a_stats = p.a_stats, e.a_corr = p.a_corr, e.res_stats = p.res_stats, e.res_gamma = p.res_gamma;
+  e.res_beta = p.res_beta, e.stats_out = p.stats_out, e.ln_eps = p.ln_eps;
+  s->kblocks = p.seg_kblocks[0], s->row_shift = p.seg_row_shift[0], s->row_mul = p.seg_row_mul[0];
+  s->tiles_n = (n_cols + BLOCK_N - 1) / BLOCK_N;
+  return cudaSuccess;
+}
+
+template <int BLOCK_N, int PASSES, int KIND>
+cudaError_t launch_lean(GemmChainParams& c, int grid, cudaStream_t stream, bool pdl) {
+  static bool attr_set = false;
+  if (!attr_set) {
+    cudaError_t e = set_attr<BLOCK_N, PASSES, KIND>();
+    if (e != cudaSuccess) return e;
+    attr_set = true;
+  }
+  void* args[] = {&c};
+  const void* kern = c.stage[0].epi.residual != nullptr ? reinterpret_cast<const void*>(gemm_tile_kernel<BLOCK_N, PASSES, 1, KIND>)
+                                                        : reinterpret_cast<const void*>(gemm_tile_kernel<BLOCK_N, PASSES, 0, KIND>);
+  return launch_kernel(kern, args, grid, kernel_threads(0),
+                       TileCfg<BLOCK_N, PASSES, true>::kSmemBytes, stream, pdl);
+}
+
+template <int BLOCK_N, int PASSES, int KIND>
+cudaError_t launch_cfg(const GemmParams& p, int m_rows, int n_cols, cudaStream_t stream, bool pdl) {
+  using Cfg = TileCfg<BLOCK_N, PASSES, false>;
+  const bool plain = p.clip_rows == 0;
+  const int tiles_m = (m_rows + kGemmBlockM - 1) / kGemmBlockM;
+  if (p.a_stats != nullptr && (!plain || p.a_corr == nullptr)) return cudaErrorInvalidValue;
+  if (p.row_mask != nullptr && plain) return cudaErrorInvalidValue;
+  if (plain && p.skin_A == nullptr && (p.act == kActNone || p.act == kActGelu)) {
+    GemmChainParams c{};
+    cudaError_t e = fill_stage<BLOCK_N, PASSES, KIND>(p, n_cols, &c.stage[0]);
+    if (e != cudaSuccess) return e;
+    c.num_stages = 1, c.tiles_m = tiles_m, c.num_items = tiles_m * c.stage[0].tiles_n;
+    int grid = c.num_items < sm_count() ? c.num_items : sm_count();
+    if (c.stage[0].kind == 3) grid -= grid % 4;
+    return launch_lean<BLOCK_N, PASSES, KIND>(c, grid, stream, pdl);
+  }
+  if (p.stats_out != nullptr) return cudaErrorInvalidValue;
+  const int epi = p.skin_A != nullptr ? 4 : p.row_mask != nullptr ? 5 : 2;
+  auto kern = epi == 2 ? gemm_tile_kernel<BLOCK_N, PASSES, 2, KIND> : gemm_tile_kernel<BLOCK_N, PASSES, 5, KIND>;
+  int smem_bytes = Cfg::kSmemBytes;
+  if (epi == 4) {
+    if constexpr (BLOCK_N == 96 && PASSES == 3 && KIND == kKindF16) {
+      if (!plain || p.act != kActNone || p.out == nullptr || p.skin_nb == nullptr || p.skin_bone == nullptr || p.skin_w == nullptr ||
+          p.bias != nullptr || p.residual != nullptr || p.a_stats != nullptr)
+        return cudaErrorInvalidValue;
+      kern = gemm_tile_kernel<BLOCK_N, PASSES, 4, KIND>;
+      smem_bytes = Cfg::kStages * Cfg::kStageBytes + 1024 + Cfg::kAccBytes + kSkinStageBytes;
+      static bool skin_attr_set = false;
+      if (!skin_attr_set) {
+        cudaError_t e = cudaFuncSetAttribute(kern, cudaFuncAttributeMaxDynamicSharedMemorySize, smem_bytes);
+        if (e != cudaSuccess) return e;
+        skin_attr_set = true;
+      }
+    } else {
+      return cudaErrorInvalidValue;
+    }
+  }
+  static bool attr_set = false;
+  if (!attr_set) {
+    cudaError_t e = set_attr<BLOCK_N, PASSES, KIND>();
+    if (e != cudaSuccess) return e;
+    attr_set = true;
+  }
+  GemmParams q = p;
+  q.grid_m_rows = m_rows;
+  q.grid_n_cols = n_cols;
+  int tiles = ((n_cols + BLOCK_N - 1) / BLOCK_N) * tiles_m;
+  if (q.k_splits > 1) {
+    int iters = 0;
+    for (int s = 0; s < q.num_segs; ++s) iters += q.seg_kblocks[s];
+    const int per = (iters + q.k_splits - 1) / q.k_splits;
+    if (plain || q.out == nullptr || q.out_hi != nullptr || q.bias != nullptr || q.residual != nullptr ||
+        q.act != kActNone || q.out_row_mul != 1 || q.out_row_add != 0 || (q.k_splits - 1) * per >= iters ||
+        q.split_row_stride < m_rows)
+      return cudaErrorInvalidValue;
+    tiles *= q.k_splits;
+  }
+  const int grid = tiles < sm_count() ? tiles : sm_count();
+  void* args[] = {&q};
+  return launch_kernel(reinterpret_cast<const void*>(kern), args, grid, kernel_threads(epi), smem_bytes, stream, pdl);
 }
 
 }
@@ -1111,6 +1342,29 @@
 #undef ROHM_GEMM_CASE
 }
 
+int gemm_chain_words(int num_stages, int m_rows) { return 1 + num_stages * ((m_rows + kGemmBlockM - 1) / kGemmBlockM); }
+
+cudaError_t launch_gemm_chain(const GemmParams* const* stages, const int* n_cols, int num_stages, int m_rows,
+                              const GemmChainSync& sync, cudaStream_t stream, bool pdl) {
+  if (num_stages < 1 || num_stages > kMaxChainStages || m_rows <= 0) return cudaErrorInvalidValue;
+  if (num_stages > 1 && (sync.words == nullptr || sync.status == nullptr)) return cudaErrorInvalidValue;
+  GemmChainParams c{};
+  c.num_stages = num_stages;
+  c.tiles_m = (m_rows + kGemmBlockM - 1) / kGemmBlockM;
+  c.words = sync.words;
+  c.status = sync.status;
+  for (int s = 0; s < num_stages; ++s) {
+    if (stages[s] == nullptr || (num_stages > 1 && stages[s]->residual != nullptr)) return cudaErrorInvalidValue;
+    const cudaError_t e = fill_stage<128, 3, kKindF16>(*stages[s], n_cols[s], &c.stage[s]);
+    if (e != cudaSuccess) return e;
+    c.stage[s].first_item = c.num_items;
+    c.num_items += c.tiles_m * c.stage[s].tiles_n;
+  }
+  int grid = c.num_items < sm_count() ? c.num_items : sm_count();
+  if (sync.max_ctas > 0 && sync.max_ctas < grid) grid = sync.max_ctas;
+  return launch_lean<128, 3, kKindF16>(c, grid, stream, pdl);
+}
+
 cudaError_t gemm_init_attributes() {
   cudaError_t e;
   if ((e = set_attr<32, 1, kKindTf32>()) != cudaSuccess) return e;
diff --git a/rohm_b200/csrc/gemm.cuh b/rohm_b200/csrc/gemm.cuh
--- a/rohm_b200/csrc/gemm.cuh
+++ b/rohm_b200/csrc/gemm.cuh
@@ -77,6 +77,18 @@
 cudaError_t launch_gemm(const GemmParams& p, int m_rows, int n_cols, int block_n, int passes, cudaStream_t stream,
                         bool pdl = false, int kind = kKindTf32);
 
+constexpr int kMaxChainStages = 4;
+constexpr int kChainOk = 0;
+constexpr int kChainErrWaitExpired = 1;
+struct GemmChainSync {
+  unsigned int* words;
+  int* status;
+  int max_ctas;
+};
+int gemm_chain_words(int num_stages, int m_rows);
+cudaError_t launch_gemm_chain(const GemmParams* const* stages, const int* n_cols, int num_stages, int m_rows,
+                              const GemmChainSync& sync, cudaStream_t stream, bool pdl);
+
 cudaError_t gemm_init_attributes();
 
 cudaError_t launch_split_tf32(const float* x, float* hi, float* lo, int64_t n, cudaStream_t stream);
diff --git a/rohm_b200/csrc/posenet.cu b/rohm_b200/csrc/posenet.cu
--- a/rohm_b200/csrc/posenet.cu
+++ b/rohm_b200/csrc/posenet.cu
@@ -256,6 +256,9 @@
   std::vector<int> prof_cat;
   GemmParams g_in{}, g_cond{}, g_out{};
   std::vector<GemmParams> g_qkv, g_proj, g_ff1, g_ff2;
+  bool use_chains = true;
+  unsigned int* chain_words = nullptr;
+  int* chain_status = nullptr;
 };
 
 enum ProfCat { kCatGemm = 0, kCatAttention = 1, kCatLayerNorm = 2, kCatOther = 3, kNumCats = 4 };
@@ -401,6 +404,25 @@
   g.M = rows;
   prof_begin(pn, kCatGemm, st);
   ROHM_CUDA(pn->ctx, launch_gemm(g, rows, w.N, w.block_n, pn->passes, st, pn->use_pdl && !pn->profiling, w.kind));
+  prof_end(pn, st);
+  pn->launches++;
+  return ROHM_OK;
+}
+
+static bool chains_on(const rohm_posenet* pn) { return pn->fused_ln && pn->use_chains && pn->chain_words != nullptr; }
+
+static int run_layer_chain(rohm_posenet* pn, int l, int rows, cudaStream_t st) {
+  PoseNetLayerDev& d = pn->layers[l];
+  const bool next = l + 1 < pn->L;
+  GemmParams* g[kMaxChainStages] = {&pn->g_proj[l], &pn->g_ff1[l], &pn->g_ff2[l], next ? &pn->g_qkv[l + 1] : nullptr};
+  const int n_cols[kMaxChainStages] = {d.proj.N, d.ff1.N, d.ff2.N, next ? pn->layers[l + 1].qkv.N : 0};
+  const int n = next ? 4 : 3;
+  for (int s = 0; s < n; ++s) g[s]->M = rows;
+  GemmChainSync sync{};
+  sync.words = pn->chain_words + static_cast<int64_t>(l) * gemm_chain_words(kMaxChainStages, rows);
+  sync.status = pn->chain_status;
+  prof_begin(pn, kCatGemm, st);
+  ROHM_CUDA(pn->ctx, launch_gemm_chain(g, n_cols, n, rows, sync, st, pn->use_pdl && !pn->profiling));
   prof_end(pn, st);
   pn->launches++;
   return ROHM_OK;
@@ -676,6 +698,16 @@
       }
     }
   }
+  if (pn->fused_ln && pn->L > 0) {
+    const int64_t words = static_cast<int64_t>(pn->L) * gemm_chain_words(kMaxChainStages, static_cast<int>(R));
+    pn->chain_words = static_cast<unsigned int*>(pn->pool.bytes(words * static_cast<int64_t>(sizeof(unsigned int))));
+    pn->chain_status = static_cast<int*>(pn->pool.bytes(sizeof(int)));
+    if (pn->chain_words == nullptr || pn->chain_status == nullptr || cudaMemset(pn->chain_status, 0, sizeof(int)) != cudaSuccess) {
+      const int rc__ = fail(ctx, ROHM_ERR_CUDA, "chain counter buffers: %s", cudaGetErrorString(pn->pool.last_error()));
+      delete pn;
+      return rc__;
+    }
+  }
   if (gemm_enable_tma_store(&pn->g_out, R, pn->kind) != 0) {
     const int rc__ = fail(ctx, ROHM_ERR_CUDA, "cuTensorMapEncodeTiled (store map) failed");
     delete pn;
@@ -817,6 +849,9 @@
   const int rows = packed ? pn->packed_rows : B * S;
   pn->launches = 0;
   int rc;
+  if (chains_on(pn))
+    ROHM_CUDA(ctx, cudaMemsetAsync(pn->chain_words, 0,
+                                   static_cast<size_t>(pn->L) * gemm_chain_words(kMaxChainStages, rows) * sizeof(unsigned int), st));
 
   dim3 grid((T + 31) / 32, (pn->C + 31) / 32, B);
   prof_begin(pn, kCatOther, st);
@@ -836,6 +871,12 @@
 
   for (int l = 0; l < pn->L; ++l) {
     PoseNetLayerDev& d = pn->layers[l];
+    if (chains_on(pn)) {
+      if (l == 0 && (rc = run_gemm(pn, pn->g_qkv[0], d.qkv, rows, st)) != ROHM_OK) return rc;
+      if ((rc = run_attention(pn, B, S, st)) != ROHM_OK) return rc;
+      if ((rc = run_layer_chain(pn, l, rows, st)) != ROHM_OK) return rc;
+      continue;
+    }
     if ((rc = run_gemm(pn, pn->g_qkv[l], d.qkv, rows, st)) != ROHM_OK) return rc;
     if ((rc = run_attention(pn, B, S, st)) != ROHM_OK) return rc;
     if ((rc = run_gemm(pn, pn->g_proj[l], d.proj, rows, st)) != ROHM_OK) return rc;
@@ -939,5 +980,19 @@
     pn->use_pdl = value != 0;
     return ROHM_OK;
   }
+  if (option == 2) {
+    if (pn->use_chains != (value != 0)) pn->graphs.clear();
+    pn->use_chains = value != 0;
+    return ROHM_OK;
+  }
   return fail(pn->ctx, ROHM_ERR_INVALID, "rohm_posenet_set_option: unknown option %d", option);
 }
+
+extern "C" int rohm_posenet_chain_status(const rohm_posenet* pn, int* status) {
+  if (pn == nullptr || status == nullptr) return ROHM_ERR_INVALID;
+  *status = 0;
+  if (pn->chain_status == nullptr) return ROHM_OK;
+  rohm::DeviceGuard device_guard__(pn->ctx);
+  ROHM_CUDA(pn->ctx, cudaMemcpy(status, pn->chain_status, sizeof(int), cudaMemcpyDeviceToHost));
+  return ROHM_OK;
+}
diff --git a/rohm_b200/csrc/ptx.cuh b/rohm_b200/csrc/ptx.cuh
--- a/rohm_b200/csrc/ptx.cuh
+++ b/rohm_b200/csrc/ptx.cuh
@@ -91,6 +91,16 @@
 __device__ __forceinline__ void bulk_commit() { asm volatile("cp.async.bulk.commit_group;" ::: "memory"); }
 __device__ __forceinline__ void bulk_wait_read_all() { asm volatile("cp.async.bulk.wait_group.read 0;" ::: "memory"); }
 __device__ __forceinline__ void bulk_wait_all() { asm volatile("cp.async.bulk.wait_group 0;" ::: "memory"); }
+
+__device__ __forceinline__ void fence_proxy_async_global() { asm volatile("fence.proxy.async.global;" ::: "memory"); }
+__device__ __forceinline__ unsigned int ld_acquire_gpu(const unsigned int* p) {
+  unsigned int v;
+  asm volatile("ld.acquire.gpu.global.u32 %0, [%1];" : "=r"(v) : "l"(p) : "memory");
+  return v;
+}
+__device__ __forceinline__ void red_release_gpu_add(unsigned int* p, unsigned int v) {
+  asm volatile("red.release.gpu.global.add.u32 [%0], %1;" ::"l"(p), "r"(v) : "memory");
+}
 
 __device__ __forceinline__ void wgmma_fence() { asm volatile("wgmma.fence.sync.aligned;" ::: "memory"); }
 __device__ __forceinline__ void wgmma_commit() { asm volatile("wgmma.commit_group.sync.aligned;" ::: "memory"); }
```

New measurement: 21.16 (median of 6 runs). 1.06x the previous value.
